# Shamir-Lab/Faucet

Hardware: AMD Instinct MI355X
Metric: canonical k-mers/s (load+scan) at k=31, 100bp reads; % HBM roofline (higher is better)
Workload: dtype u64

## Files before the change

### faucet_amd/csrc/api.hip

```cpp
#include <cstdio>
#include <algorithm>
#include <string>

#include <chrono>
#include <thread>

#include "fgpu_ctx.h"

int fgpu_scan_export_impl(fgpu_ctx* ctx, void* dev_entries, uint64_t cap_entries, uint64_t* d_stamps, uint64_t* n_entries);
int fgpu_scan_import_impl(fgpu_ctx* ctx, const void* dev_entries, uint64_t n);
int fgpu_scan_download_impl(fgpu_ctx* ctx, uint64_t* keys_host, fgpu_junction* recs_host, uint64_t cap, uint64_t* n_out);

static thread_local std::string g_create_error;

int g_fgpu_trace = getenv("FGPU_TRACE") && getenv("FGPU_TRACE")[0] == '1';

int fgpu_ensure(fgpu_ctx* ctx, DevBuf* b, uint64_t bytes) {
    if (b->bytes >= bytes && b->p) return FGPU_OK;
    if (b->p) {
        FGPU_HIP(fgpu_sync_stream(ctx, ctx->stream));
        FGPU_HIP(hipFree(b->p));
        b->p = nullptr;
        b->bytes = 0;
    } else {
// ... 228 lines not shown
    if (std::string(prop.gcnArchName).rfind("gfx950", 0) != 0) {
        g_create_error = std::string("device is ") + prop.gcnArchName + ", this library is built for gfx950 only";
        return FGPU_ERR_HIP;
    }
    if ((e = hipSetDevice(p->device)) != hipSuccess) { g_create_error = hipGetErrorString(e); return FGPU_ERR_HIP; }
    lap("device properties, hipSetDevice");

    fgpu_ctx* ctx = new fgpu_ctx();
    ctx->prm = *p;
    const int device = p->device;
    std::thread warm([device, ctx] {
        if (hipSetDevice(device) != hipSuccess) return;
        fgpu_touch_text();
        fgpu_touch_pack();
        fgpu_touch_load();
        fgpu_touch_load_slices();
        (void)fgpu_text_streams(ctx);
        (void)hipGetLastError();
    });
    struct Joiner { std::thread& t; ~Joiner() { if (t.joinable()) t.join(); } } joiner{warm};
    if (!ctx->prm.junction_capacity) {
        uint64_t c = p->tai / 32;
        if (c < (1ULL << 22)) c = 1ULL << 22;
        if (c > (1ULL << 28)) c = 1ULL << 28;
        ctx->prm.junction_capacity = c;
    }
    if (!ctx->prm.max_batch_bases) ctx->prm.max_batch_bases = 1ULL << 30;
    ctx->resident_budget = (p->flags & FGPU_FLAG_NO_RESIDENT) ? 0 : prop.totalGlobalMem / 8;
    ctx->journal_budget = prop.totalGlobalMem / 8;
    if (const char* e = getenv("FGPU_JOURNAL_MB")) ctx->journal_budget = (uint64_t)atoll(e) << 20;
    ctx->fd.k = p->k;
    ctx->fd.j = p->j;
    ctx->fd.n_hash = p->n_hash;
    ctx->fd.max_spacer = p->max_spacer_dist;
    ctx->fd.kmask = (1ULL << (2 * p->k)) - 1;
    ctx->fd.tai_mask = p->tai - 1;
    ctx->profile = (p->flags & FGPU_FLAG_PROFILE) != 0;
    ctx->record_stops = (p->flags & FGPU_FLAG_RECORD_STOPS) != 0;
    { const char* e = getenv("FGPU_PROFILE_WALK"); ctx->prof_walk_detail = e && e[0] == '1'; }
    ctx->bloom_bytes = p->tai / 8;
    ctx->max_span = std::min<uint64_t>(std::max<uint64_t>(p->tai >> 4, FGPU_MAX_SPAN), 1ULL << 28);
    if (const char* e = getenv("FGPU_MAX_SPAN_LOG2")) {
        int l = atoi(e);
        if (l >= 12 && l <= 28) ctx->max_span = 1ULL << l;
    }
    memset(&ctx->load_stats, 0, sizeof(ctx->load_stats));
    memset(&ctx->scan_stats, 0, sizeof(ctx->scan_stats));
    int rc = FGPU_OK;
    auto fail = [&](const char* what, hipError_t he) {
        g_create_error = std::string(what) + ": " + hipGetErrorString(he);
        rc = FGPU_ERR_HIP;
    };
    if (p->stream) {
        ctx->stream = (hipStream_t)p->stream;
    } else {
        if ((e = hipStreamCreateWithFlags(&ctx->stream, hipStreamNonBlocking)) != hipSuccess) fail("hipStreamCreate", e);
        ctx->own_stream = true;
    }
    ctx->launch_stream = ctx->stream;
    if (!rc) {
        ctx->bg = new std::thread([device, ctx] {
            auto bad = [ctx](const char* what, hipError_t he) {
                ctx->bg_err = std::string(what) + ": " + hipGetErrorString(he);
                ctx->bg_rc = FGPU_ERR_HIP;
            };
            hipError_t he;
            if ((he = hipSetDevice(device)) != hipSuccess) return bad("hipSetDevice", he);
            int lo = 0, hi = 0;
            hipDeviceGetStreamPriorityRange(&lo, &hi);
            if ((he = hipStreamCreateWithPriority(&ctx->wstream, hipStreamNonBlocking, hi)) != hipSuccess) return bad("hipStreamCreate (walk)", he);
            if ((he = hipStreamCreateWithPriority(&ctx->cstream, hipStreamNonBlocking, hi)) != hipSuccess) return bad("hipStreamCreate (clean)", he);
            if ((he = hipStreamCreateWithPriority(&ctx->ostream, hipStreamNonBlocking, hi)) != hipSuccess) return bad("hipStreamCreate (optimistic walk)", he);
            if ((he = hipEventCreateWithFlags(&ctx->ev_walked, hipEventDisableTiming)) != hipSuccess) return bad("hipEventCreate", he);
            if ((he = hipEventCreateWithFlags(&ctx->ev_listed, hipEventDisableTiming)) != hipSuccess) return bad("hipEventCreate", he);
            if ((he = hipEventCreateWithFlags(&ctx->ev_settled, hipEventDisableTiming)) != hipSuccess) return bad("hipEventCreate", he);
            for (int q = 0; q < 2; q++)
                if ((he = hipEventCreateWithFlags(&ctx->ev_uf_reset[q], hipEventDisableTiming)) != hipSuccess) return bad("hipEventCreate", he);
            fgpu_touch_scan_pure();
            fgpu_touch_scan_walk();
            fgpu_touch_scan_table();
            fgpu_touch_scan_harvest();
            (void)hipGetLastError();
        });
    }
    lap("main stream");
    if (!rc && getenv("FGPU_DEBUG_ALLOC_FIRST") && hipMalloc(&ctx->first, p->tai * 4) != hipSuccess) { (void)hipGetLastError(); ctx->first = nullptr; }
    if (!rc && (e = hipMalloc(&ctx->bloo1, ctx->bloom_bytes)) != hipSuccess) fail("hipMalloc bloo1", e);
    if (!rc && (e = hipMalloc(&ctx->bloo2, ctx->bloom_bytes)) != hipSuccess) fail("hipMalloc bloo2", e);
    if (!rc && (e = hipMalloc(&ctx->counters, sizeof(DevCounters))) != hipSuccess) fail("hipMalloc counters", e);
    if (!rc && (e = hipHostMalloc(&ctx->counters_host, sizeof(DevCounters))) != hipSuccess) fail("hipHostMalloc", e);
    if (!rc && (e = hipHostMalloc(&ctx->fb_host, 64)) != hipSuccess) fail("hipHostMalloc", e);
    if (!rc) {
        memset(ctx->counters_host, 0, sizeof(DevCounters));
        hipMemsetAsync(ctx->bloo1, 0, ctx->bloom_bytes, ctx->stream);
        hipMemsetAsync(ctx->bloo2, 0, ctx->bloom_bytes, ctx->stream);
        hipMemsetAsync(ctx->counters, 0, sizeof(DevCounters), ctx->stream);
        if ((e = hipStreamSynchronize(ctx->stream)) != hipSuccess) fail("initial memset", e);
    }
    lap("filters allocated and cleared");
    warm.join();
    lap("pass-1 code objects, text stream");
    if (rc) {
        fgpu_destroy(ctx);
        return rc;
    }
    *out = ctx;
    return FGPU_OK;
}

void fgpu_destroy(fgpu_ctx* ctx) {
    if (!ctx) return;
    (void)hipSetDevice(ctx->prm.device);
    (void)fgpu_bg_join(ctx);
    if (ctx->ostream) hipStreamSynchronize(ctx->ostream);
    if (ctx->cstream) hipStreamSynchronize(ctx->cstream);
    if (ctx->copy_stream) { hipStreamSynchronize(ctx->copy_stream); hipStreamDestroy(ctx->copy_stream); hipEventDestroy(ctx->copy_after); }
    if (ctx->tstream) {
        hipStreamSynchronize(ctx->tstream);
        hipStreamDestroy(ctx->tstream);
    }
    for (int i = 0; i < FGPU_TEXT_SETS; i++) if (ctx->ev_text_mark[i]) hipEventDestroy(ctx->ev_text_mark[i]);
    for (int i = 0; i < 2; i++) if (ctx->ev_stage_free[i]) hipEventDestroy(ctx->ev_stage_free[i]);
    if (ctx->ev_text_done) hipEventDestroy(ctx->ev_text_done);
    if (ctx->wstream) hipStreamSynchronize(ctx->wstream);
    if (ctx->stream) hipStreamSynchronize(ctx->stream);
    for (PendingEvent& pe : ctx->pending_events) { hipEventDestroy(pe.a); hipEventDestroy(pe.b); }
    for (DevBuf* b : ctx->owned) if (b->p) hipFree(b->p);
    if (ctx->lp.flips_host) hipHostFree(ctx->lp.flips_host);
    if (ctx->lp.ev_open) hipEventDestroy(ctx->lp.ev_open);
    void* ptrs[] = {ctx->lp.bits, ctx->lp.first, ctx->short_pf, ctx->bloo1, ctx->bloo2, ctx->first, ctx->pair, ctx->rec, ctx->slice_first, ctx->slice_pair, ctx->jkeys, ctx->jrecs, ctx->jstamps, ctx->jfilter, ctx->wkeys,
                    ctx->wbits, ctx->uf_parent, ctx->cl_count, ctx->cl_offset, ctx->cl_fill, ctx->cl_fail, ctx->ko_hk, ctx->ko_occ, ctx->ko_piece, ctx->cl_members, ctx->cl_roots, ctx->counters,
                    ctx->wdesc};
    for (void* p : ptrs) if (p) hipFree(p);
    stop_queue_recycle(ctx);
    for (StopBatch& f : ctx->stop_pool) hipHostFree(f.data);
    ctx->stop_pool.clear();
    if (ctx->counters_host) hipHostFree(ctx->counters_host);
    if (ctx->fb_host) hipHostFree(ctx->fb_host);
    if (ctx->wstream) { hipStreamSynchronize(ctx->wstream); hipStreamDestroy(ctx->wstream); }
    if (ctx->cstream) { hipStreamSynchronize(ctx->cstream); hipStreamDestroy(ctx->cstream); }
    if (ctx->ostream) { hipStreamSynchronize(ctx->ostream); hipStreamDestroy(ctx->ostream); }
    if (ctx->ev_walked) hipEventDestroy(ctx->ev_walked);
    if (ctx->ev_listed) hipEventDestroy(ctx->ev_listed);
    if (ctx->ev_settled) hipEventDestroy(ctx->ev_settled);
    for (int q = 0; q < 2; q++) if (ctx->ev_uf_reset[q]) hipEventDestroy(ctx->ev_uf_reset[q]);
    if (ctx->own_stream && ctx->stream) hipStreamDestroy(ctx->stream);
    for (ResidentBatch* r : ctx->resident) delete r;
    for (PackedBlock* b : ctx->packed) delete b;
    for (JournalBatch* j : ctx->journal) delete j;
    for (JournalBatch* j : ctx->journal_pool) delete j;
    for (BatchBufs* b : ctx->all_batches) {
        if (b->pure_done) hipEventDestroy(b->pure_done);
        if (b->walk_done) hipEventDestroy(b->walk_done);
        delete b;
    }
    delete ctx;
}

int fgpu_synchronize(fgpu_ctx* ctx) {
    if (!ctx) return FGPU_ERR_ARG;
    return sync_all(ctx);
}

int fgpu_load_begin(fgpu_ctx* ctx, int keep_carry) {
    if (!ctx) return FGPU_ERR_ARG;
    if (ctx->phase != 0) { ctx->err = "load_begin while another pass is open"; return FGPU_ERR_STATE; }
    FGPU_HIP(hipSetDevice(ctx->prm.device));
    if (int rc = fgpu_bloom_download_wait(ctx)) return rc;
    static const char* layout_env = getenv("FGPU_LOAD_LAYOUT");
    bool want_rec = layout_env && layout_env[0] == 'r';
    if (want_rec && !ctx->rec) {
        if (hipMalloc(&ctx->rec, ctx->prm.tai / 32 * 256) != hipSuccess) {
            (void)hipGetLastError();
            ctx->rec = nullptr;
            want_rec = false;
        }
    }
    ctx->rec_layout = want_rec;
    if (!ctx->rec_layout && !ctx->first) {
        hipError_t e = hipMalloc(&ctx->first, ctx->prm.tai * 4);
        if (e != hipSuccess) {
            ctx->err = std::string("hipMalloc of the first-set-time array (4 bytes per Bloom bit) failed: ") + hipGetErrorString(e);
            ctx->first = nullptr;
            return FGPU_ERR_NOMEM;
        }
    }
    if (!ctx->rec_layout && !ctx->pair) {
        hipError_t e = hipMalloc(&ctx->pair, ctx->bloom_bytes * 2);
        if (e != hipSuccess) {
            ctx->err = std::string("hipMalloc of the interleaved filter pair failed: ") + hipGetErrorString(e);
            ctx->pair = nullptr;
            return FGPU_ERR_NOMEM;
        }
        if (int rc = fgpu_place_pair(ctx)) return rc;
    }
    ctx->shard_times = (keep_carry & FGPU_LOAD_SHARD_TIMES) != 0;
    ctx->shard_planes = (keep_carry & FGPU_LOAD_SHARD_PLANES) != 0 && !ctx->shard_times && ctx->prm.n_hash <= 4;
    ctx->fixup_ready = false;
    ctx->scan_resident_base = 0;
    ctx->pass_positions = ctx->pass_batches = 0;
    ctx->pass_empty_carry = !(keep_carry & FGPU_LOAD_KEEP_CARRY);
    keep_carry &= FGPU_LOAD_KEEP_CARRY;
    fgpu_load_pass_policy(ctx);
    if (!ctx->rec_layout) FGPU_HIP(hipMemsetAsync(ctx->first, 0xFF, ctx->prm.tai * 4, ctx->stream));
    fgpu_resident_reset(ctx, true);
    if (!keep_carry) FGPU_HIP(hipMemsetAsync(ctx->bloo1, 0, ctx->bloom_bytes, ctx->stream));
    FGPU_HIP(hipMemsetAsync(ctx->bloo2, 0, ctx->bloom_bytes, ctx->stream));
    int rc = fgpu_load_pair_begin(ctx);
    if (rc) return rc;
    if ((rc = fgpu_load_pass_counters(ctx))) return rc;
    ctx->phase = 1;
    return FGPU_OK;
}

int fgpu_load_batch(fgpu_ctx* ctx, const fgpu_reads* reads) {
    if (!ctx) return FGPU_ERR_ARG;
    if (ctx->phase != 1) { ctx->err = "load_batch outside load_begin/load_end"; return FGPU_ERR_STATE; }
    int rc = fgpu_check_reads(ctx, reads);
    if (rc) return rc;
    FGPU_HIP(hipSetDevice(ctx->prm.device));
    if ((rc = fgpu_stage_pack(ctx, reads))) return rc;
    if ((rc = fgpu_stage_load(ctx))) return rc;
    if (ctx->cur->T) ctx->pass_batches++;
    ctx->load_stats.reads_processed += reads->n_reads;
    return fgpu_host_batch_done(ctx, reads);
}

int fgpu_presence_batch(fgpu_ctx* ctx, const fgpu_reads* reads) {
    if (!ctx) return FGPU_ERR_ARG;
    if (ctx->phase != 0) { ctx->err = "presence_batch while a pass is open"; return FGPU_ERR_STATE; }
    int rc = fgpu_check_reads(ctx, reads);
    if (rc) return rc;
    FGPU_HIP(hipSetDevice(ctx->prm.device));
    if ((rc = fgpu_stage_pack(ctx, reads))) return rc;
    if ((rc = fgpu_stage_presence(ctx))) return rc;
    return fgpu_host_batch_done(ctx, reads);
}

int fgpu_load_end(fgpu_ctx* ctx, fgpu_load_stats* stats) {
    if (!ctx) return FGPU_ERR_ARG;
    if (ctx->phase != 1) { ctx->err = "load_end without load_begin"; return FGPU_ERR_STATE; }
    return fgpu_load_pass_end(ctx, stats);
}

int fgpu_load_fixup_state(fgpu_ctx* ctx, int* ready, uint64_t* resident_budget_bytes) {
    if (!ctx) return FGPU_ERR_ARG;
    if (ready) *ready = ctx->phase == 0 && ctx->fixup_ready ? 1 : 0;
    if (resident_budget_bytes) *resident_budget_bytes = ctx->resident_budget;
    return FGPU_OK;
}

int fgpu_load_fixup(fgpu_ctx* ctx, const void* prefix_dev, fgpu_load_stats* stats) {
    if (!ctx || !prefix_dev) return FGPU_ERR_ARG;
    if (ctx->phase != 0) { ctx->err = "load_fixup while a pass is open"; return FGPU_ERR_STATE; }
    if (!ctx->fixup_ready) {
        ctx->err = "load_fixup needs a finished load pass begun with FGPU_LOAD_SHARD_TIMES and an empty carry (or FGPU_LOAD_SHARD_PLANES and at most 4 hash functions), every batch kept resident, no --mercy";
        return FGPU_ERR_STATE;
    }
    FGPU_HIP(hipSetDevice(ctx->prm.device));
    if (int rc = fgpu_bloom_download_wait(ctx)) return rc;
    int rc = fgpu_stage_fixup(ctx, (const uint32_t*)prefix_dev);
    if (!rc) rc = fgpu_util_or(ctx, ctx->bloo1, prefix_dev, ctx->bloom_bytes);
    if (!rc) rc = fgpu_pull_counters(ctx);
    if (rc) return rc;
    ctx->fixup_ready = false;
    ctx->load_stats.to_bloo2 = ctx->counters_host->to_bloo2;
    if (stats) *stats = ctx->load_stats;
    return FGPU_OK;
}

static uint32_t* bloom_ptr(fgpu_ctx* ctx, int which) { return which == FGPU_BLOO1 ? ctx->bloo1 : which == FGPU_BLOO2 ? ctx->bloo2 : nullptr; }

int fgpu_bloom_download(fgpu_ctx* ctx, int which, uint8_t* host_out, uint64_t nbytes) {
    if (!ctx || !host_out || !bloom_ptr(ctx, which) || nbytes != ctx->bloom_bytes) return FGPU_ERR_ARG;
    if (ctx->phase == 1 || ctx->phase == 3) { ctx->err = "bloom_download inside a load pass: the filters are interleaved until load_end"; return FGPU_ERR_STATE; }
    FGPU_HIP(hipMemcpyAsync(host_out, bloom_ptr(ctx, which), nbytes, hipMemcpyDeviceToHost, ctx->stream));
    FGPU_HIP(fgpu_sync_stream(ctx, ctx->stream));
    return FGPU_OK;
}

int fgpu_bloom_download_wait(fgpu_ctx* ctx) {
    if (!ctx) return FGPU_ERR_ARG;
    if (!ctx->copy_pending) return FGPU_OK;
    ctx->copy_pending = false;
    FGPU_HIP(fgpu_sync_stream(ctx, ctx->copy_stream));
    return FGPU_OK;
}

int fgpu_bloom_download_begin(fgpu_ctx* ctx, int which, uint8_t* host_out, uint64_t nbytes) {
    if (!ctx || !host_out || !bloom_ptr(ctx, which) || nbytes != ctx->bloom_bytes) return FGPU_ERR_ARG;
    if (ctx->phase == 1 || ctx->phase == 3) { ctx->err = "bloom_download_begin inside a load pass: the filters are interleaved until load_end"; return FGPU_ERR_STATE; }
    if (int rc = fgpu_bloom_download_wait(ctx)) return rc;
    FGPU_HIP(hipSetDevice(ctx->prm.device));
    if (!ctx->copy_stream) {
        FGPU_HIP(hipStreamCreateWithFlags(&ctx->copy_stream, hipStreamNonBlocking));
        FGPU_HIP(hipEventCreateWithFlags(&ctx->copy_after, hipEventDisableTiming));
    }
    FGPU_HIP(hipEventRecord(ctx->copy_after, ctx->stream));
    FGPU_HIP(hipStreamWaitEvent(ctx->copy_stream, ctx->copy_after, 0));
    FGPU_HIP(hipMemcpyAsync(host_out, bloom_ptr(ctx, which), nbytes, hipMemcpyDeviceToHost, ctx->copy_stream));
    ctx->copy_pending = true;
    return FGPU_OK;
}

int fgpu_bloom_upload(fgpu_ctx* ctx, int which, const uint8_t* host_in, uint64_t nbytes) {
    if (!ctx || !host_in || !bloom_ptr(ctx, which) || nbytes != ctx->bloom_bytes) return FGPU_ERR_ARG;
    if (ctx->phase != 0) { ctx->err = "bloom_upload while a pass is open (a load pass would overwrite it at load_end, a scan is reading bloo2)"; return FGPU_ERR_STATE; }
    if (int rc = fgpu_bloom_download_wait(ctx)) return rc;
    if (which == FGPU_BLOO2) fgpu_resident_reset(ctx, false);
    FGPU_HIP(hipMemcpyAsync(bloom_ptr(ctx, which), host_in, nbytes, hipMemcpyHostToDevice, ctx->stream));
    FGPU_HIP(fgpu_sync_stream(ctx, ctx->stream));
    return FGPU_OK;
}

int fgpu_bloom_weight(fgpu_ctx* ctx, int which, float* weight) {
    if (!ctx || !weight || !bloom_ptr(ctx, which)) return FGPU_ERR_ARG;
    if (ctx->phase == 1 || ctx->phase == 3) { ctx->err = "bloom_weight inside a load pass: the filters are interleaved until load_end"; return FGPU_ERR_STATE; }
    FGPU_HIP(hipMemsetAsync(&ctx->counters->pad, 0, 8, ctx->stream));
    int rc = fgpu_util_popcount(ctx, bloom_ptr(ctx, which), ctx->bloom_bytes, &ctx->counters->pad);
    if (rc) return rc;
    FGPU_HIP(hipMemcpyAsync(&ctx->counters_host->pad, &ctx->counters->pad, 8, hipMemcpyDeviceToHost, ctx->stream));
    FGPU_HIP(fgpu_sync_stream(ctx, ctx->stream));
    *weight = (float)(long)ctx->counters_host->pad / (float)ctx->prm.tai;
    return FGPU_OK;
}

int fgpu_bloom_devptr(fgpu_ctx* ctx, int which, void** dptr, uint64_t* nbytes) {
    if (!ctx || !dptr || !bloom_ptr(ctx, which)) return FGPU_ERR_ARG;
    *dptr = bloom_ptr(ctx, which);
    if (nbytes) *nbytes = ctx->bloom_bytes;
    return FGPU_OK;
}

int fgpu_bitmap_or(fgpu_ctx* ctx, void* dst_dev, const void* src_dev, uint64_t nbytes) {
    if (!ctx || !dst_dev || !src_dev || (nbytes & 15)) return FGPU_ERR_ARG;
    return fgpu_util_or(ctx, dst_dev, src_dev, nbytes);
}

int fgpu_scan_resident_base(fgpu_ctx* ctx, uint64_t first_batch) {
    if (!ctx) return FGPU_ERR_ARG;
    if (ctx->phase != 0) { ctx->err = "scan_resident_base while a pass is open: between the load pass and fgpu_scan_begin"; return FGPU_ERR_STATE; }
    ctx->scan_resident_base = first_batch;
    return FGPU_OK;
}

int fgpu_scan_begin(fgpu_ctx* ctx) {
    if (!ctx) return FGPU_ERR_ARG;
    if (ctx->phase != 0) { ctx->err = "scan_begin while another pass is open"; return FGPU_ERR_STATE; }
    FGPU_HIP(hipSetDevice(ctx->prm.device));
    int rc = fgpu_bg_join(ctx);
    if (rc) return rc;
    if ((rc = fgpu_scan_alloc(ctx))) return rc;
    if ((rc = fgpu_scan_reset(ctx))) return rc;
    ctx->fixup_ready = false;
    FGPU_HIP(hipMemsetAsync(ctx->counters, 0, sizeof(DevCounters), ctx->stream));
    memset(&ctx->scan_stats, 0, sizeof(ctx->scan_stats));
    memset(ctx->counters_host, 0, sizeof(DevCounters));
    ctx->scan_windows = 0;
    ctx->scan_pieces_seen = 0;
    ctx->scan_piece_base = 0;
    ctx->scan_imported = 0;
    ctx->delta_next = 0;
    journal_recycle(ctx);
    ctx->journal_on = !(ctx->prm.flags & FGPU_FLAG_EAGER_FLAGS) && !ctx->eager_runtime;
    ctx->eager_scan = ctx->lazy_failed = ctx->capacity_failed = false;
    ctx->dl_keys_n = 0;
    ctx->late_acc[0] = ctx->late_acc[1] = ctx->late_acc[2] = 0;
    ctx->stops_delivered = 0;
    ctx->lp_applied_seq = 0;
    ctx->host_waits = 0;
    ctx->host_wait_ms = 0;
    ctx->wait_sites.clear();
    if (ctx->short_pf) FGPU_HIP(hipMemsetAsync(ctx->short_pf, 0, ctx->short_pf_tai / 8, ctx->stream));
    if ((rc = fgpu_long_pairs_reset(ctx))) return rc;
    ctx->have_import = false;
    ctx->journal_max_read_len = 0;
    ctx->hint_in_table = false;
    ctx->hint_gen = 0;
    ctx->hint_n = ctx->hint_max_seq = 0;
    ctx->delta_ready = false;
    ctx->delta_keys = ctx->refresh_full = ctx->refresh_delta = ctx->refresh_mismatch = 0;
    ctx->sparse_links = ctx->full_links = 0;
    ctx->dbg_stall_us = getenv("FGPU_DEBUG_WALK_STALL_US") ? std::min(100000, std::max(0, atoi(getenv("FGPU_DEBUG_WALK_STALL_US")))) : 0;
    ctx->dbg_delta_check = getenv("FGPU_DEBUG_DELTA_CHECK") != nullptr;
    ctx->no_sparse_link = getenv("FGPU_NO_SPARSE_LINK") != nullptr;
    const uint64_t start_span = std::max<uint64_t>(1ULL << 18, ctx->settled_span / 4);
    ctx->window_span = ctx->prm.walk_window_span ? std::min<uint64_t>(std::max<uint64_t>(ctx->prm.walk_window_span, 64), ctx->max_span)
                                                 : std::min<uint64_t>(start_span, ctx->max_span);
    ctx->calib_left = 16;
    ctx->calib_f = ctx->calib_p = 0;
    ctx->adapt_followers = 0;
    ctx->adapt_pieces = 0;
    ctx->adapt_overflows = 0;
    ctx->adapt_vote = 0;
    ctx->calib_ovf = 0;
    ctx->span_ceiling = ~0ULL;
    ctx->repeats_seen_before = false;
    ctx->walked_pieces = 0;
    ctx->scan_batch_index = 0;
    ctx->scan_batch_seq = 0;
    for (BatchBufs* b : ctx->to_harvest) b->stops_pending = false;
    ctx->to_harvest.clear();
    stop_queue_recycle(ctx);
    for (BatchBufs* b : ctx->prepared) ctx->pool.push_back(b);
    ctx->prepared.clear();
    ctx->cur = &ctx->bb_default;
    ctx->phase = 2;
    return FGPU_OK;
}

static void adapt_window(fgpu_ctx* ctx) {
    static const bool dbg_span = getenv("FGPU_DEBUG_SPAN") != nullptr;
    const uint64_t f = ctx->counters_host->followers_seen - ctx->adapt_followers;
    const uint64_t p = ctx->counters_host->walked_pieces - ctx->adapt_pieces;
    if (p == 0 || ctx->prm.walk_window_span) return;
    {
        const uint64_t usual = std::min<uint64_t>(std::min<uint64_t>(ctx->max_span, FGPU_USUAL_SPAN), ctx->span_ceiling);
        int want = 0;
        bool clear = false;
        if (f * 2 > p) { want = -1; clear = f * 5 > p * 4; }
        else if (f * 3 < p) { want = 1; clear = f * 20 < p * 3; }
        const bool act = want < 0 || (want > 0 && (clear || ctx->adapt_vote > 0));
        ctx->adapt_vote = act ? 0 : want;
        if (want >= 0) ctx->proven_span = std::max(ctx->proven_span, ctx->window_span);
        if (ctx->counters_host->ko_overflows > ctx->adapt_overflows && ctx->window_span > 4096) {
            ctx->window_span = std::max<uint64_t>(4096, ctx->window_span / 4);
            ctx->proven_span = std::min(ctx->proven_span, ctx->window_span);
            ctx->span_ceiling = std::min(ctx->span_ceiling, ctx->window_span * 2);
            ctx->calib_ovf = ctx->counters_host->ko_overflows;
            ctx->calib_left = 0;
        }
        else if (act && want < 0 && ctx->window_span > 4096) {
            ctx->window_span /= 2;
            if (clear || ctx->window_span > ctx->proven_span) ctx->calib_left = 8;
            ctx->proven_span = std::min(ctx->proven_span, ctx->window_span);
        }
        else if (act && want > 0 && ctx->window_span < usual) {
            ctx->window_span = std::min<uint64_t>(ctx->window_span * 2, usual);
            if (ctx->window_span > ctx->proven_span) ctx->calib_left = std::max(ctx->calib_left, 2);
        }
        else if (f * 16 < p && ctx->window_span < std::min<uint64_t>(ctx->max_span, ctx->span_ceiling)) ctx->window_span *= 2;
    }
    if (dbg_span) fprintf(stderr, "[span] batch: followers %llu of %llu pieces -> span %llu, looks %d, vote %d\n", (unsigned long long)f, (unsigned long long)p,
                          (unsigned long long)ctx->window_span, ctx->calib_left, ctx->adapt_vote);
    ctx->adapt_followers = ctx->counters_host->followers_seen;
    ctx->adapt_pieces = ctx->counters_host->walked_pieces;
    ctx->adapt_overflows = ctx->counters_host->ko_overflows;
}

static BatchBufs* acquire_batch(fgpu_ctx* ctx) {
    BatchBufs* b;
    static const size_t depth = getenv("FGPU_SCAN_BUFFERS") ? (size_t)std::min(FGPU_DELTA_RING, std::max(2, atoi(getenv("FGPU_SCAN_BUFFERS")))) : 2;
    if (ctx->pool.size() >= depth) {
        const size_t at = ctx->pool.size() - depth;
        b = ctx->pool[at];
        ctx->pool.erase(ctx->pool.begin() + at);
    } else {
        b = new BatchBufs();
        ctx->all_batches.push_back(b);
        hipEventCreateWithFlags(&b->pure_done, hipEventDisableTiming);
        hipEventCreateWithFlags(&b->walk_done, hipEventDisableTiming);
    }
    return b;
}

static void note_walked(fgpu_ctx* ctx, BatchBufs* b) {
    if (!ctx->record_stops) return;
    b->stops_pending = true;
    ctx->to_harvest.push_back(b);
}

static int scan_pure_into(fgpu_ctx* ctx, BatchBufs* b, const fgpu_reads* reads) {
    if (b->stops_pending) {
        int hrc = fgpu_scan_harvest(ctx, b);
        if (hrc) return hrc;
    }
    b->seq = ctx->scan_batch_seq++;
    ctx->cur = b;
    const double t_a = fgpu_host_now();
    if (b->walk_pending) {
        FGPU_HIP(fgpu_sync_event(ctx, b->walk_done));
        b->walk_pending = false;
    }
    const double t_b = fgpu_host_now();
    ctx->host_ms[0] += t_b - t_a;
    int rc = fgpu_stage_pack(ctx, reads);
    ctx->host_ms[1] += fgpu_host_now() - t_b;
    if (!rc) rc = journal_add(ctx, b, reads);
    uint64_t n_pieces = 0;
    if (!rc) rc = fgpu_stage_scan_pure(ctx, &n_pieces);
    if (!rc) ctx->journal_max_read_len = std::max<uint64_t>(ctx->journal_max_read_len, ctx->counters_host->max_read_len);
    if (!rc) rc = check_errors(ctx);
    if (!rc) ctx->scan_stats.reads_processed += reads->n_reads;
    if (!rc && b->pure_done) FGPU_HIP(hipEventRecord(b->pure_done, ctx->stream));
    if (!rc) rc = fgpu_host_batch_done(ctx, reads);
    return rc;
}

static void journal_recycle(fgpu_ctx* ctx) {
    for (JournalBatch* j : ctx->journal) ctx->journal_pool.push_back(j);
    ctx->journal.clear();
    ctx->journal_bytes = 0;
}

static int journal_add(fgpu_ctx* ctx, BatchBufs* b, const fgpu_reads* reads) {
    if (!ctx->journal_on || ctx->in_replay) return FGPU_OK;
    const uint64_t cb = 2 * (b->n_words + FGPU_PADW) * 8, bbytes = (b->n_words + FGPU_PADW) * 8, ob = ctx->record_stops ? (b->n_reads + 1) * 8 : 0;
    if (ctx->journal_bytes + cb + bbytes + ob > ctx->journal_budget) {
        int rc = fgpu_pull_counters(ctx);
        if (rc) return rc;
        BatchBufs* const cur = ctx->cur;
        ctx->journal_max_read_len = std::max<uint64_t>(ctx->journal_max_read_len, ctx->counters_host->max_read_len);
        if (ctx->lazy_failed && (rc = scan_replay(ctx))) return rc;
        ctx->cur = cur;
        ctx->journal_on = false;
        ctx->eager_scan = true;
        journal_recycle(ctx);
        return FGPU_OK;
    }
    JournalBatch* j;
    if (!ctx->journal_pool.empty()) { j = ctx->journal_pool.back(); ctx->journal_pool.pop_back(); }
    else j = new JournalBatch();
    int rc;
    if ((rc = fgpu_ensure_b(ctx, &j->codes, cb)) || (rc = fgpu_ensure_b(ctx, &j->bad, bbytes)) || (ob && (rc = fgpu_ensure_b(ctx, &j->offs, ob)))) {
        ctx->journal_pool.push_back(j);
        return rc;
    }
    if (b->T) {
        FGPU_HIP(hipMemcpyAsync(j->codes.p, b->codes.p, cb, hipMemcpyDeviceToDevice, ctx->stream));
        FGPU_HIP(hipMemcpyAsync(j->bad.p, b->bad.p, bbytes, hipMemcpyDeviceToDevice, ctx->stream));
        if (ob) FGPU_HIP(hipMemcpyAsync(j->offs.p, b->d_offs, ob, hipMemcpyDeviceToDevice, ctx->stream));
    }
    j->T = b->T; j->n_words = b->n_words; j->n_reads = b->n_reads; j->seq = b->seq;
    ctx->journal.push_back(j);
    ctx->journal_bytes += cb + bbytes + ob;
    (void)reads;
    return FGPU_OK;
}

static int scan_replay_once(fgpu_ctx* ctx);
static int scan_replay(fgpu_ctx* ctx) {
    for (int attempt = 0;; attempt++) {
        const bool for_room = ctx->capacity_failed;
        ctx->capacity_failed = false;
        if (for_room) {
            int rc = sync_all(ctx);
            if (!rc) rc = fgpu_scan_regrow_empty(ctx, ctx->jcap * 4);
            if (rc) { ctx->lazy_failed = false; return rc; }
            ctx->capacity_replays++;
        }
        int rc = scan_replay_once(ctx);
        if (rc == FGPU_ERR_CAPACITY && (ctx->counters_host->error_flags & 1ULL) && ctx->jcap < (1ULL << 31) && attempt < 6) {
            ctx->capacity_failed = true;
            continue;
        }
        if (!rc && for_room) ctx->journal_on = true;
        return rc;
    }
}

static int scan_replay_once(fgpu_ctx* ctx) {
    ctx->in_replay = true;
    ctx->journal_on = false;
    ctx->eager_scan = true;
    ctx->lazy_failed = false;
    int rc = sync_all(ctx);
    for (BatchBufs* b : ctx->prepared) ctx->pool.push_back(b);
    ctx->prepared.clear();
    for (BatchBufs* b : ctx->to_harvest) b->stops_pending = false;
    ctx->to_harvest.clear();
    stop_queue_recycle(ctx);
    if (!rc) rc = fgpu_scan_reset(ctx);
    if (rc) { ctx->in_replay = false; return rc; }
    {
        unsigned long long ln[3] = {0, 0, 0};
        if (hipMemcpy(ln, ctx->counters->late_n, sizeof(ln), hipMemcpyDeviceToHost) == hipSuccess)
            for (int i = 0; i < 3; i++) ctx->late_acc[i] += ln[i];
    }
    FGPU_HIP(hipMemsetAsync(ctx->counters, 0, sizeof(DevCounters), ctx->stream));
    FGPU_HIP(hipMemcpyAsync(&ctx->counters->max_read_len, &ctx->journal_max_read_len, 8, hipMemcpyHostToDevice, ctx->stream));
    FGPU_HIP(fgpu_sync_stream(ctx, ctx->stream));
    const uint64_t reads_processed = ctx->scan_stats.reads_processed;
    memset(&ctx->scan_stats, 0, sizeof(ctx->scan_stats));
    ctx->scan_stats.reads_processed = reads_processed;
    memset(ctx->counters_host, 0, sizeof(DevCounters));
    ctx->scan_windows = 0;
    ctx->scan_pieces_seen = 0;
    ctx->scan_piece_base = 0;
    ctx->scan_imported = 0;
    ctx->delta_next = 0;
    ctx->hint_in_table = false;
    ctx->delta_ready = false;
    ctx->window_span = ctx->prm.walk_window_span ? std::min<uint64_t>(std::max<uint64_t>(ctx->prm.walk_window_span, 64), ctx->max_span)
                                                 : std::min<uint64_t>(std::max<uint64_t>(1ULL << 18, ctx->settled_span / 4), ctx->max_span);
    ctx->calib_left = 16;
    ctx->calib_f = ctx->calib_p = 0;
    ctx->adapt_followers = ctx->adapt_pieces = ctx->adapt_overflows = 0;
    ctx->adapt_vote = 0;
    ctx->calib_ovf = 0;
    ctx->span_ceiling = ~0ULL;
    ctx->repeats_seen_before = false;
    ctx->walked_pieces = 0;
    ctx->scan_batch_index = 0;
    memset(&ctx->carried, 0, sizeof(ctx->carried));
    if (ctx->have_import) {
        if ((rc = fgpu_scan_reserve(ctx, ctx->import_n)) || (rc = fgpu_scan_import_impl(ctx, ctx->import_copy.p, ctx->import_n))) { ctx->in_replay = false; return rc; }
        FGPU_HIP(fgpu_sync_stream(ctx, ctx->stream));
        ctx->scan_imported = ctx->import_n;
        if (ctx->import_has_carried) {
            ctx->carried = ctx->import_carried;
            ctx->scan_piece_base = ctx->import_carried.reads_no_errors;
        }
    }
    for (size_t i = 0; i < ctx->journal.size() && !rc; i++) {
        JournalBatch* j = ctx->journal[i];
        BatchBufs* b = acquire_batch(ctx);
        if (b->stops_pending && (rc = fgpu_scan_harvest(ctx, b))) {
            ctx->pool.push_back(b);
            break;
        }
        if (b->walk_pending) {
            FGPU_HIP(fgpu_sync_event(ctx, b->walk_done));
            b->walk_pending = false;
        }
        b->seq = j->seq;
        ctx->cur = b;
        b->T = j->T; b->n_words = j->n_words; b->n_reads = j->n_reads;
        b->d_offs = (const uint64_t*)j->offs.p;
        if (b->T) {
            const uint64_t cb = 2 * (b->n_words + FGPU_PADW) * 8, bbytes = (b->n_words + FGPU_PADW) * 8;
            if ((rc = fgpu_ensure_b(ctx, &b->codes, cb)) || (rc = fgpu_ensure_b(ctx, &b->bad, bbytes))) break;
            FGPU_HIP(hipMemcpyAsync(b->codes.p, j->codes.p, cb, hipMemcpyDeviceToDevice, ctx->stream));
            FGPU_HIP(hipMemcpyAsync(b->bad.p, j->bad.p, bbytes, hipMemcpyDeviceToDevice, ctx->stream));
        }
        uint64_t n_pieces = 0;
        rc = fgpu_stage_scan_pure(ctx, &n_pieces);
        if (!rc) rc = check_errors(ctx);
        if (!rc && b->pure_done) FGPU_HIP(hipEventRecord(b->pure_done, ctx->stream));
        if (!rc) rc = fgpu_scan_reserve(ctx, ctx->counters_host->n_junctions + ctx->scan_imported);
        if (!rc) {
            adapt_window(ctx);
            rc = fgpu_stage_scan_walk(ctx, b->n_pieces);
            ctx->walked_pieces += b->n_pieces;
            if (!rc) note_walked(ctx, b);
        }
        ctx->pool.push_back(b);
    }
    ctx->cur = &ctx->bb_default;
    if (!rc) rc = fgpu_pull_counters(ctx);
    ctx->in_replay = false;
    ctx->scan_replays++;
    return rc;
}

int fgpu_scan_batch(fgpu_ctx* ctx, const fgpu_reads* reads) {
    if (!ctx) return FGPU_ERR_ARG;
    if (ctx->phase != 2) { ctx->err = "scan_batch outside scan_begin/scan_end"; return FGPU_ERR_STATE; }
    if (!ctx->prepared.empty()) { ctx->err = "scan_batch while prepared batches are waiting: call fgpu_scan_walk_prepared first"; return FGPU_ERR_STATE; }
    if (ctx->hint_in_table) { ctx->err = "the junction table holds a preview (fgpu_scan_import_hint): import the real table before walking"; return FGPU_ERR_STATE; }
    int rc = fgpu_check_reads(ctx, reads);
    if (rc) return rc;
    FGPU_HIP(hipSetDevice(ctx->prm.device));
    if (ctx->lazy_failed && (rc = scan_replay(ctx))) return rc;
    BatchBufs* b = acquire_batch(ctx);
    rc = scan_pure_into(ctx, b, reads);
    if (rc == FGPU_INTERNAL_REPLAY) {
        ctx->cur = &ctx->bb_default;
        ctx->pool.insert(ctx->pool.begin(), b);
        if ((rc = scan_replay(ctx))) return rc;
        b = acquire_batch(ctx);
        rc = scan_pure_into(ctx, b, reads);
    }
    if (!rc && ctx->lazy_failed) {
        ctx->cur = &ctx->bb_default;
        ctx->pool.push_back(b);
        return scan_replay(ctx);
    }
    if (!rc) rc = fgpu_scan_reserve(ctx, ctx->counters_host->n_junctions + ctx->scan_imported);
    if (!rc) {
        adapt_window(ctx);
        const double t_w = fgpu_host_now();
        rc = fgpu_stage_scan_walk(ctx, b->n_pieces);
        ctx->host_ms[5] += fgpu_host_now() - t_w;
        ctx->walked_pieces += b->n_pieces;
        if (!rc) note_walked(ctx, b);
    }
    ctx->cur = &ctx->bb_default;
    ctx->pool.push_back(b);
    return rc;
}

int fgpu_scan_prepare(fgpu_ctx* ctx, const fgpu_reads* reads) {
    if (!ctx) return FGPU_ERR_ARG;
    if (ctx->phase != 2) { ctx->err = "scan_prepare outside scan_begin/scan_end"; return FGPU_ERR_STATE; }
    int rc = fgpu_check_reads(ctx, reads);
    if (rc) return rc;
    FGPU_HIP(hipSetDevice(ctx->prm.device));
    BatchBufs* b;
    if (!ctx->pool.empty()) { b = ctx->pool.front(); ctx->pool.erase(ctx->pool.begin()); }
    else {
        b = new BatchBufs();
        ctx->all_batches.push_back(b);
        hipEventCreateWithFlags(&b->pure_done, hipEventDisableTiming);
        hipEventCreateWithFlags(&b->walk_done, hipEventDisableTiming);
    }
    rc = scan_pure_into(ctx, b, reads);
    ctx->cur = &ctx->bb_default;
    if (rc == FGPU_INTERNAL_REPLAY) {
        ctx->pool.insert(ctx->pool.begin(), b);
        if ((rc = scan_replay(ctx))) return rc;
        return fgpu_scan_prepare(ctx, reads);
    }
    if (rc) { ctx->pool.push_back(b); return rc; }
    b->planes_gen = ctx->hint_in_table ? ctx->hint_gen : 0;
    b->cand_gen = 0;
    ctx->prepared.push_back(b);
    return FGPU_OK;
}

int fgpu_scan_refresh_prepared(fgpu_ctx* ctx) {
    if (!ctx) return FGPU_ERR_ARG;
    if (ctx->phase != 2) { ctx->err = "scan_refresh_prepared outside scan_begin/scan_end"; return FGPU_ERR_STATE; }
    if (!ctx->hint_in_table) { ctx->err = "scan_refresh_prepared without a preview in the table (fgpu_scan_import_hint)"; return FGPU_ERR_STATE; }
    FGPU_HIP(hipSetDevice(ctx->prm.device));
    const bool no_sparse = ctx->no_sparse_link;
    for (BatchBufs* b : ctx->prepared) {
        if (b->planes_gen != ctx->hint_gen) {
            if (int rc = fgpu_scan_refresh_planes(ctx, b)) return rc;
            b->planes_gen = ctx->hint_gen;
            b->cand_gen = 0;
        }
        if (!no_sparse && b->cand_gen != ctx->hint_gen)
            if (int rc = fgpu_scan_build_cand(ctx, b)) return rc;
    }
    ctx->launch_stream = ctx->stream;
    FGPU_HIP(fgpu_sync_stream(ctx, ctx->stream));
    return FGPU_OK;
}

int fgpu_scan_walk_prepared(fgpu_ctx* ctx) {
    if (!ctx) return FGPU_ERR_ARG;
    if (ctx->phase != 2) { ctx->err = "scan_walk_prepared outside scan_begin/scan_end"; return FGPU_ERR_STATE; }
    if (ctx->hint_in_table) { ctx->err = "the junction table holds a preview (fgpu_scan_import_hint): import the real table before walking"; return FGPU_ERR_STATE; }
    FGPU_HIP(hipSetDevice(ctx->prm.device));
    int rc = FGPU_OK;
    if (ctx->lazy_failed) return scan_replay(ctx);
    static const bool serial_refresh = !(getenv("FGPU_PREPARED_REFRESH") && getenv("FGPU_PREPARED_REFRESH")[0] == 'o');
    if (!serial_refresh && !ctx->prepared.empty()) rc = fgpu_scan_refresh_planes(ctx, ctx->prepared[0]);
    for (size_t i = 0; i < ctx->prepared.size() && !rc; i++) {
        BatchBufs* b = ctx->prepared[i];
        if (i > 0) {
            if ((rc = fgpu_pull_counters(ctx))) break;
            if (ctx->lazy_failed) { ctx->cur = &ctx->bb_default; return scan_replay(ctx); }
            if (!ctx->prm.walk_window_span) adapt_window(ctx);
            if ((rc = fgpu_scan_reserve(ctx, ctx->counters_host->n_junctions + ctx->scan_imported))) break;
        }
        if (!serial_refresh && i + 1 < ctx->prepared.size() && (rc = fgpu_scan_refresh_planes(ctx, ctx->prepared[i + 1]))) break;
        ctx->cur = b;
        ctx->refresh_snapshot = serial_refresh;
        rc = fgpu_stage_scan_walk(ctx, b->n_pieces);
        ctx->refresh_snapshot = false;
        ctx->walked_pieces += b->n_pieces;
        if (!rc) note_walked(ctx, b);
    }
    ctx->cur = &ctx->bb_default;
    for (BatchBufs* b : ctx->prepared) ctx->pool.push_back(b);
    ctx->prepared.clear();
    return rc;
}

int fgpu_scan_set_eager(fgpu_ctx* ctx, int on) {
    if (!ctx) return FGPU_ERR_ARG;
    if (ctx->phase != 0) { ctx->err = "fgpu_scan_set_eager while a pass is open"; return FGPU_ERR_STATE; }
    ctx->eager_runtime = on != 0;
    return FGPU_OK;
}

int fgpu_scan_short_pairs(fgpu_ctx* ctx, uint64_t tai, int32_t n_hash, int32_t lists_to_host) {
    if (!ctx) return FGPU_ERR_ARG;
    if (ctx->phase != 0) { ctx->err = "fgpu_scan_short_pairs while a pass is open"; return FGPU_ERR_STATE; }
    FGPU_HIP(hipSetDevice(ctx->prm.device));
    if (ctx->short_pf) {
        FGPU_HIP(fgpu_sync_stream(ctx, ctx->stream));
        FGPU_HIP(hipFree(ctx->short_pf));
        ctx->short_pf = nullptr;
        ctx->short_pf_tai = 0;
    }
    if (!tai) return FGPU_OK;
    if (!ctx->record_stops) { ctx->err = "fgpu_scan_short_pairs needs FGPU_FLAG_RECORD_STOPS"; return FGPU_ERR_STATE; }
    if (!is_pow2(tai) || tai < 128 || n_hash < 1 || n_hash > 32) { ctx->err = "fgpu_scan_short_pairs: tai must be a power of two >= 128, n_hash 1..32"; return FGPU_ERR_ARG; }
    FGPU_HIP(hipMalloc(&ctx->short_pf, tai / 8));
    FGPU_HIP(hipMemsetAsync(ctx->short_pf, 0, tai / 8, ctx->stream));
    ctx->short_pf_tai = tai;
    ctx->short_pf_hashes = n_hash;
    ctx->short_pf_lists_to_host = lists_to_host != 0;
    return FGPU_OK;
}

int fgpu_scan_short_pairs_download(fgpu_ctx* ctx, uint8_t* out, uint64_t n_bytes) {
    if (!ctx || !out) return FGPU_ERR_ARG;
    if (!ctx->short_pf) { ctx->err = "fgpu_scan_short_pairs_download without fgpu_scan_short_pairs"; return FGPU_ERR_STATE; }
    if (ctx->phase != 0) { ctx->err = "fgpu_scan_short_pairs_download while a pass is open"; return FGPU_ERR_STATE; }
    if (n_bytes != ctx->short_pf_tai / 8) { ctx->err = "fgpu_scan_short_pairs_download: the filter has tai / 8 bytes"; return FGPU_ERR_ARG; }
    FGPU_HIP(hipSetDevice(ctx->prm.device));
    FGPU_HIP(hipMemcpyAsync(out, ctx->short_pf, n_bytes, hipMemcpyDeviceToHost, ctx->stream));
    FGPU_HIP(fgpu_sync_stream(ctx, ctx->stream));
    return FGPU_OK;
}

int fgpu_scan_take_stops(fgpu_ctx* ctx, fgpu_stop* out, uint64_t cap, uint64_t* n_out, int64_t* batch_seq) {
    if (!ctx || !n_out || !batch_seq) return FGPU_ERR_ARG;
    if (!ctx->record_stops) { ctx->err = "fgpu_scan_take_stops needs FGPU_FLAG_RECORD_STOPS"; return FGPU_ERR_STATE; }
    *n_out = 0;
    *batch_seq = -1;
    if (ctx->phase == 2 && ctx->lazy_failed) {
        if (int rc = scan_replay(ctx)) return rc;
    }
    if (ctx->stop_queue.empty() && !ctx->to_harvest.empty()) {
        FGPU_HIP(hipSetDevice(ctx->prm.device));
        int rc = fgpu_scan_harvest(ctx, ctx->to_harvest.front());
        if (rc == FGPU_INTERNAL_REPLAY && ctx->phase == 2) {
            if ((rc = scan_replay(ctx))) return rc;
            if (!ctx->to_harvest.empty()) rc = fgpu_scan_harvest(ctx, ctx->to_harvest.front());
        }
        if (rc) return rc;
    }
    if (ctx->stop_queue.empty()) return FGPU_OK;
    StopBatch& sb = ctx->stop_queue.front();
    *n_out = sb.n;
    *batch_seq = (int64_t)sb.seq;
    if (sb.n > cap || (sb.n && !out)) return FGPU_ERR_CAPACITY;
    if (sb.n) memcpy(out, sb.data, sb.n * sizeof(fgpu_stop));
    ctx->stops_delivered = sb.seq + 1;
    if (sb.data) { StopBatch f; f.data = sb.data; f.cap = sb.cap; ctx->stop_pool.push_back(f); }
    ctx->stop_queue.pop_front();
    return FGPU_OK;
}

int fgpu_scan_end(fgpu_ctx* ctx, fgpu_scan_stats* stats) {
    if (!ctx) return FGPU_ERR_ARG;
    if (ctx->phase != 2) { ctx->err = "scan_end without scan_begin"; return FGPU_ERR_STATE; }
    static const bool dbg_host = getenv("FGPU_DEBUG_HOST") != nullptr;
    static const bool dbg_waits = getenv("FGPU_DEBUG_WAITS") != nullptr;
    struct TellWaits {
        fgpu_ctx* c;
        bool on;
        ~TellWaits() {
            if (!on) return;
            for (const WaitSite& w : c->wait_sites) {
                const char* f = strrchr(w.file, '/');
                fprintf(stderr, "[waits] %-14s:%-5d %6llu times %9.2f ms\n", f ? f + 1 : w.file, w.line, (unsigned long long)w.n, w.ms);
            }
        }
    } tell_waits{ctx, dbg_waits};
    if (dbg_host) {
        fprintf(stderr, "[host] scan: wait for the buffers' last walk %.2f ms, pack issue %.2f, pure stage issue (first half) %.2f, wait for the piece count %.2f, "
                        "pure stage issue (second half) %.2f, walk issue %.2f\n", ctx->host_ms[0], ctx->host_ms[1], ctx->host_ms[2], ctx->host_ms[3], ctx->host_ms[4], ctx->host_ms[5]);
        for (double& v : ctx->host_ms) v = 0;
    }
// ... 310 lines not shown
```

### faucet_amd/csrc/fgpu_ctx.h

```cpp
#pragma once
#include <chrono>
#include <hip/hip_runtime.h>
#include <stdint.h>
#include <stdio.h>
#include <string.h>

#include <string>
#include <thread>
#include <vector>

#include "../../include/faucet_gpu.h"
#include <deque>

#include "fgpu_device.h"

#define FGPU_PADW 8
#define FGPU_USUAL_SPAN (1ULL << 26)
#define FGPU_MAX_SPAN (1ULL << 26)

struct DevBuf {
    void*    p = nullptr;
    uint64_t bytes = 0;
};

struct BatchBufs {
    DevBuf codes, bad;
    DevBuf readflag;
    DevBuf pending;
    DevBuf sure;
    DevBuf fail;
    DevBuf same;
    DevBuf valid, pm, ps, ff, fb, cf0, cf1, cb0, cb1, inF, inB;
    DevBuf lk;
    DevBuf cand;
    uint32_t cand_gen = 0;
    DevBuf nF, nB, need;
    DevBuf kh;
    DevBuf cr;
    DevBuf ps_prefix;
    DevBuf pieces;
    DevBuf sF, sB;
    DevBuf piece_read;
    DevBuf stop_off, stop_out;
    const uint64_t* d_offs = nullptr;
    uint64_t seq = 0;
    bool stops_pending = false;
    uint64_t T = 0;
    uint64_t n_words = 0;
    uint64_t n_reads = 0;
    uint64_t n_pieces = 0;
    uint64_t max_piece_span = 0;
    hipEvent_t pure_done = nullptr;
    hipEvent_t walk_done = nullptr;
    bool walk_pending = false;
    uint32_t planes_gen = 0;
};

struct ResidentBatch {
    DevBuf codes, bad, sure;
    DevBuf fail;
    DevBuf miss;
    uint64_t T = 0, n_words = 0;
    uint32_t tb = 0;
    void *packed_codes = nullptr, *packed_bad = nullptr;
    const void* codes_p() const { return packed_codes ? packed_codes : codes.p; }
    const void* bad_p() const { return packed_bad ? packed_bad : bad.p; }
};

struct PackedBlock {
    DevBuf buf;
    uint64_t T = 0, n_words = 0, n_reads = 0;
    int state = 0;
};
static inline uint64_t fgpu_packed_bytes(uint64_t n_words) { return 3 * (n_words + FGPU_PADW) * 8 + 16; }

struct DeltaList {
    DevBuf list, count;
};
#define FGPU_DELTA_RING 4

struct JournalBatch {
    DevBuf codes, bad, offs;
    uint64_t T = 0, n_words = 0, n_reads = 0, seq = 0;
};
#define FGPU_INTERNAL_REPLAY 1000

struct StopBatch {
    uint64_t seq = 0;
    fgpu_stop* data = nullptr;
    size_t n = 0, cap = 0;
};

struct LongPairs {
    int mode = 0;
    bool sparse = false;
    uint64_t tai = 0;
    int n_hash = 0;
    uint32_t* bits = nullptr;
    uint32_t* first = nullptr;
    DevBuf table;
    uint64_t table_high = 0;
    DevBuf canon, h0, h1, vread, rs, state, dev;
    DevBuf kept_set[2];
    int kept_cur = 0;
    uint32_t* flips_host = nullptr;
    bool pending_first = false;
    uint64_t n_kept = 0;
    uint64_t empty_host = 0;
    uint64_t rounds = 0, max_rounds = 0, batches = 0;
    bool open = false, open_odd = false, open_filter = false;
    uint32_t open_elems = 0, open_vreads = 0;
    hipEvent_t ev_open = nullptr;
};

struct WaitSite {
    const char* file;
    int line;
    uint64_t n;
    double ms;
};

struct KernelStat {
    std::string name;
    uint64_t launches = 0;
    double total_ms = 0;
};

struct PendingEvent {
    int stat;
    hipEvent_t a, b;
};

constexpr unsigned FGPU_LATE_CAP = 256;
struct DevCounters {
    unsigned long long kmers;
    unsigned long long to_bloo2;
    unsigned long long segments;
    unsigned long long pieces;
    unsigned long long nb_jcheck;
    unsigned long long nb_no_juncs;
    unsigned long long nb_processed;
    unsigned long long nb_skipped;
    unsigned long long n_junctions;
    unsigned long long table_slots_used;
    unsigned long long followers;
    unsigned long long max_cluster;
    unsigned long long error_flags;
    unsigned long long max_read_len;
    unsigned long long wt_used;
    unsigned long long pad;
    unsigned long long wt_used_b;
    unsigned long long pad2;
    unsigned long long flag_positions;
    unsigned long long piece_positions;
    unsigned long long valid_reused;
    unsigned long long flags_filled;
    unsigned long long walked_pieces;
    unsigned long long followers_seen;
    unsigned long long mark_hits;
    unsigned long long mark_pending;
    unsigned long long walk_parallel;
    unsigned long long par_probe[4];
    unsigned long long ko_time[8];
    unsigned long long ko_overflows;
    unsigned long long ovw_kept;
    unsigned long long ovw[4];
    unsigned long long ovw_fill;
    unsigned long long late_n[3];
    unsigned long long late[2 * FGPU_LATE_CAP];
    unsigned long long slice_mercy[6];
};

constexpr int FGPU_TEXT_SETS = 3;
struct TextSet { DevBuf buf, nl, rank, tmp, rec; };

static inline double fgpu_host_now() { return std::chrono::duration<double, std::milli>(std::chrono::steady_clock::now().time_since_epoch()).count(); }

struct fgpu_ctx {
    fgpu_params prm;
    FdParams fd;
    hipStream_t stream = nullptr;
    hipStream_t wstream = nullptr;
    hipStream_t cstream = nullptr;
    hipEvent_t ev_walked = nullptr, ev_uf_reset[2] = {nullptr, nullptr};
    hipStream_t ostream = nullptr;
    hipEvent_t ev_listed = nullptr, ev_settled = nullptr;
    hipStream_t launch_stream = nullptr;
    bool own_stream = false;
    std::string err;
    std::thread* bg = nullptr;
    int bg_rc = 0;
    std::string bg_err;

    uint32_t* bloo1 = nullptr;
    uint64_t epoch_positions = 0;
    uint64_t swept_positions = 0;
    bool shard_times = false;
    bool shard_planes = false;
    bool fixup_ready = false;
    uint64_t pass_positions = 0;
    uint32_t cur_tb = 0;
    bool pass_empty_carry = true;
    uint64_t pass_batches = 0;
    uint64_t sweep_min = 0;
    uint32_t sweep_num = 1, sweep_den = 1;
    bool carry_by_set = false;
    uint32_t* bloo2 = nullptr;
    uint32_t* first = nullptr;
    uint2* pair = nullptr;
    uint32_t* rec = nullptr;
    bool rec_layout = false;
    uint64_t bloom_bytes = 0;
    int phase = 0;
    uint64_t slice_lo = 0, slice_n = 0;
    uint32_t* slice_first = nullptr;
    uint2* slice_pair = nullptr;
    uint64_t slice_first_bytes = 0, slice_pair_bytes = 0;
    bool slice_committed = false;
    bool slice_mercy = false;
    bool slice_probe_owed = false;
    uint64_t slice_owed_span = 0;
    uint64_t slice_mercy_diag[6] = {0, 0, 0, 0, 0, 0};
    std::vector<ResidentBatch*> resident;
    uint64_t resident_count = 0;
    uint64_t resident_bytes = 0, resident_budget = 0;
    bool resident_open = false;
    uint64_t scan_batch_index = 0;
    uint64_t scan_resident_base = 0;
    std::vector<PackedBlock*> packed;
    DevBuf packed_digest;

    uint64_t jcap = 0;
    uint64_t* jkeys = nullptr;
    uint8_t* jrecs = nullptr;
    uint64_t* jstamps = nullptr;
    uint32_t* jfilter = nullptr;
    uint64_t wcap = 0;
    uint64_t* wkeys = nullptr;
    uint32_t* wbits = nullptr;
    int wbits_log2 = 24;
    DeltaList delta_ring[FGPU_DELTA_RING];
    bool refresh_snapshot = false;
    uint64_t delta_hist[FGPU_DELTA_RING] = {0, 0, 0, 0};
    uint64_t delta_ring_keys = 0, delta_batch_base = 0;
    uint64_t delta_next = 0;
    uint32_t wt_epoch = 0;
    uint32_t wmax = 0;
    uint32_t* uf_parent = nullptr;
    uint32_t* cl_count = nullptr;
    uint32_t* cl_offset = nullptr;
    uint32_t* cl_fill = nullptr;
    uint32_t* ko_hk = nullptr;
    uint32_t* ko_occ = nullptr;
    uint32_t* ko_piece = nullptr;
    DevBuf ovw_ev, ovw_filt, ovw_log, ovw_res, ovw_list, ovw_state, ovw_longp, ovw_marks;
    uint32_t ovw_epoch = 0;
    int ovw_ev_log2 = 23;
    int ovw_ev_log2_alloc = 0;
    int ovw_rounds = 12;
    uint32_t ko_hk_cap = 0, ko_occ_cap = 0;
    uint32_t walk_ko = 64;
    uint32_t walk_ko_weight = 0;
    bool walk_ko_always = false;
    uint32_t* cl_fail = nullptr;
    uint32_t walk_heavy = 0;
    uint32_t* cl_members = nullptr;
    uint32_t* cl_roots = nullptr;
    void* wdesc = nullptr;
    uint64_t window_span = 1ULL << 17;
    uint64_t max_span = FGPU_MAX_SPAN;
    uint64_t settled_span = 0;
    uint64_t scan_piece_base = 0;
    uint64_t scan_imported = 0;
    bool hint_in_table = false;
    uint32_t hint_gen = 0;
    uint64_t hint_n = 0, hint_max_seq = 0;
    uint64_t hint_digest[2] = {0, 0};
    DevBuf delta_filter;
    uint64_t delta_filter_bits = 0;
    bool delta_ready = false;
    uint64_t delta_keys = 0;
    uint64_t refresh_full = 0, refresh_delta = 0, refresh_mismatch = 0;
    DevBuf cand_filter;
    uint64_t sparse_links = 0, full_links = 0;
    int dbg_stall_us = 0;
    bool dbg_delta_check = false;
    bool no_sparse_link = false;
    DevBuf import_probe;
    uint64_t scan_grown = 0;

    DevCounters* counters = nullptr;
    DevCounters* counters_host = nullptr;

    fgpu_load_stats load_stats;
    uint64_t load_mark_hits = 0, load_mark_pending = 0;
    fgpu_scan_stats scan_stats;
    uint64_t scan_windows = 0;
    uint64_t scan_pieces_seen = 0;

    uint64_t adapt_followers = 0, adapt_pieces = 0;
    double host_ms[8] = {0, 0, 0, 0, 0, 0, 0, 0};
    bool repeats_seen_before = false;
    uint64_t calib_ovf = 0;
    uint64_t span_ceiling = ~0ULL;
    int adapt_vote = 0;
    uint64_t proven_span = 0;
    uint64_t adapt_overflows = 0;
    int calib_left = 0;
    uint64_t calib_f = 0, calib_p = 0;
    unsigned long long* fb_host = nullptr;
    fgpu_scan_stats carried = {};

    BatchBufs bb_default;
    BatchBufs* cur = &bb_default;
    std::vector<BatchBufs*> prepared;
    std::vector<BatchBufs*> pool;
    std::vector<BatchBufs*> all_batches;
    std::vector<JournalBatch*> journal, journal_pool;
    uint64_t journal_bytes = 0, journal_budget = 0;
    bool journal_on = false;
    bool eager_scan = false;
    bool lazy_failed = false;
    bool in_replay = false;
    bool capacity_failed = false;
    uint64_t capacity_replays = 0;
    uint32_t* short_pf = nullptr;
    uint64_t short_pf_tai = 0;
    int short_pf_hashes = 0;
    bool short_pf_lists_to_host = true;
    LongPairs lp;
    uint64_t stops_delivered = 0;
    uint64_t lp_applied_seq = 0;
    uint64_t scan_replays = 0;
    uint64_t host_waits = 0;
    double host_wait_ms = 0;
    std::vector<WaitSite> wait_sites;
    uint64_t late_acc[3] = {0, 0, 0};
    uint64_t journal_max_read_len = 0;
    DevBuf import_copy;
    uint64_t import_n = 0;
    fgpu_scan_stats import_carried = {};
    bool have_import = false, import_has_carried = false;
    bool record_stops = false;
    bool eager_runtime = false;
    std::vector<BatchBufs*> to_harvest;
    std::deque<StopBatch> stop_queue;
    std::vector<StopBatch> stop_pool;
    uint64_t scan_batch_seq = 0;
    uint64_t walked_pieces = 0;
    DevBuf probe_buf, export_stamps;
    DevBuf ko_trace;
    DevBuf s3_keys, s3_dist, s3_in;
    uint64_t s3_mask = 0, s3_count = 0;
    bool s3_ready = false;
    DevBuf dl_entries, dl_stamps, dl_stamps_sorted, dl_idx, dl_idx_sorted, dl_keys, dl_recs, dl_tmp;
    uint64_t dl_keys_n = 0;
    hipStream_t copy_stream = nullptr;
    hipEvent_t copy_after = nullptr;
    bool copy_pending = false;
    TextSet text[FGPU_TEXT_SETS];
    uint64_t text_calls = 0;
    uint64_t text_reserve = 0;
    uint64_t text_last_bytes = 0;
    double ensure_scale = 1.0;
    hipStream_t tstream = nullptr;
    hipEvent_t ev_text_mark[FGPU_TEXT_SETS] = {nullptr, nullptr, nullptr};
    hipEvent_t ev_text_done = nullptr;
    DevBuf host_stage[4];
    hipEvent_t ev_stage_free[2] = {nullptr, nullptr};
    bool host_stage_used[2] = {false, false};
    uint64_t host_turn = 0;
    int host_set = -1;
    const uint64_t* split_offsets = nullptr;
    uint64_t split_n = 0, split_total = 0;
    std::vector<DevBuf*> owned;

    bool profile = false;
    bool prof_suppress = false;
    bool prof_walk_detail = false;
    std::vector<KernelStat> kstats;
    std::vector<PendingEvent> pending_events;
};

#define FGPU_HIP(call)                                                                               \
    do {                                                                                             \
        hipError_t e__ = (call);                                                                     \
        if (e__ != hipSuccess) {                                                                     \
            char b__[512];                                                                           \
            snprintf(b__, sizeof(b__), "%s failed: %s (%s:%d)", #call, hipGetErrorString(e__), __FILE__, __LINE__); \
            ctx->err = b__;                                                                          \
            return FGPU_ERR_HIP;                                                                     \
        }                                                                                            \
    } while (0)

static inline void fgpu_note_wait(fgpu_ctx* ctx, double ms, const char* file, int line) {
    ctx->host_waits++;
    ctx->host_wait_ms += ms;
    for (WaitSite& w : ctx->wait_sites)
        if (w.line == line && w.file == file) { w.n++; w.ms += ms; return; }
    ctx->wait_sites.push_back(WaitSite{file, line, 1, ms});
}
static inline hipError_t fgpu_sync_stream_at(fgpu_ctx* ctx, hipStream_t st, const char* file, int line) {
    const double t0 = fgpu_host_now();
    const hipError_t e = hipStreamSynchronize(st);
    fgpu_note_wait(ctx, fgpu_host_now() - t0, file, line);
    return e;
}
static inline hipError_t fgpu_sync_event_at(fgpu_ctx* ctx, hipEvent_t ev, const char* file, int line) {
    const double t0 = fgpu_host_now();
    const hipError_t e = hipEventSynchronize(ev);
    fgpu_note_wait(ctx, fgpu_host_now() - t0, file, line);
    return e;
}
#define fgpu_sync_stream(ctx, st) fgpu_sync_stream_at(ctx, st, __FILE__, __LINE__)
#define fgpu_sync_event(ctx, ev) fgpu_sync_event_at(ctx, ev, __FILE__, __LINE__)

int fgpu_ensure(fgpu_ctx* ctx, DevBuf* b, uint64_t bytes);
int fgpu_ensure_b(fgpu_ctx* ctx, DevBuf* b, uint64_t bytes);
int fgpu_bg_join(fgpu_ctx* ctx);
int fgpu_prof_begin(fgpu_ctx* ctx, const char* name);
void fgpu_prof_end(fgpu_ctx* ctx, int token);
int fgpu_prof_collect(fgpu_ctx* ctx);

extern int g_fgpu_trace;
#define FGPU_LAUNCH(name, kernel, grid, block, ...)                                        \
    do {                                                                                   \
        int tok__ = fgpu_prof_begin(ctx, name);                                            \
        if (g_fgpu_trace) { fprintf(stderr, "[fgpu] %s grid %u x %u ...", name, (unsigned)(grid), (unsigned)(block)); fflush(stderr); } \
        hipLaunchKernelGGL(kernel, dim3(grid), dim3(block), 0, ctx->launch_stream, __VA_ARGS__);  \
        fgpu_prof_end(ctx, tok__);                                                         \
        FGPU_HIP(hipGetLastError());                                                       \
        if (g_fgpu_trace) { FGPU_HIP(hipStreamSynchronize(ctx->launch_stream)); fprintf(stderr, " done\n"); fflush(stderr); } \
    } while (0)

static inline unsigned fgpu_blocks(uint64_t n, unsigned per_block) { return (unsigned)((n + per_block - 1) / per_block); }
#define FGPU_GRID_BLOCKS 4096u
static inline unsigned fgpu_grid(uint64_t n, unsigned per_block) {
    uint64_t b = (n + per_block - 1) / per_block;
    return (unsigned)(b < FGPU_GRID_BLOCKS ? (b ? b : 1) : FGPU_GRID_BLOCKS);
}

static inline bool fgpu_overflow_absorbable(const fgpu_ctx* ctx) {
    return ctx->journal_on && ctx->phase == 2 && !ctx->in_replay && ctx->jcap < (1ULL << 31);
}
#define FGPU_TABLE_FULL_MSG "junction table full: raise fgpu_params.junction_capacity"

int fgpu_text_streams(fgpu_ctx* ctx);
void fgpu_touch_load();
void fgpu_touch_load_slices();
void fgpu_touch_pack();
void fgpu_touch_text();
void fgpu_touch_scan_pure();
void fgpu_touch_scan_walk();
void fgpu_touch_scan_table();
void fgpu_touch_scan_harvest();
int fgpu_stage_pack(fgpu_ctx* ctx, const fgpu_reads* reads);
int fgpu_stage_pack_block(fgpu_ctx* ctx, const fgpu_reads* reads, PackedBlock** out);
int fgpu_packed_acquire(fgpu_ctx* ctx, uint64_t T, uint64_t n_reads, int state, const char* who, PackedBlock** out);
int fgpu_packed_digest(fgpu_ctx* ctx, const PackedBlock* b, bool verify);
int fgpu_host_batch_done(fgpu_ctx* ctx, const fgpu_reads* reads);
int fgpu_stage_load(fgpu_ctx* ctx);
int fgpu_load_sweep(fgpu_ctx* ctx);
int fgpu_stage_fixup(fgpu_ctx* ctx, const uint32_t* prefix);
int fgpu_stage_presence(fgpu_ctx* ctx);
int fgpu_epoch_before_batch(fgpu_ctx* ctx, uint64_t span);
int fgpu_epoch_after_batch(fgpu_ctx* ctx, uint64_t span);
enum { FGPU_TAKE_OK = 0, FGPU_TAKE_NO_BUDGET, FGPU_TAKE_NO_MEMORY };
int fgpu_resident_take(fgpu_ctx* ctx, const uint64_t (&parts)[5], bool budgeted, ResidentBatch** out, uint64_t* total);
int fgpu_pull_counters(fgpu_ctx* ctx);
int fgpu_check_reads(fgpu_ctx* ctx, const fgpu_reads* r);
void fgpu_load_pass_policy(fgpu_ctx* ctx);
int fgpu_load_pass_counters(fgpu_ctx* ctx);
int fgpu_load_pass_end(fgpu_ctx* ctx, fgpu_load_stats* stats);
int fgpu_load_pair_begin(fgpu_ctx* ctx);
int fgpu_load_pair_end(fgpu_ctx* ctx);
void fgpu_resident_reset(fgpu_ctx* ctx, bool keep_going);
int fgpu_stage_scan_pure(fgpu_ctx* ctx, uint64_t* n_pieces);
int fgpu_stage_scan_walk(fgpu_ctx* ctx, uint64_t n_pieces);
int fgpu_stage_scan_need(fgpu_ctx* ctx);
int fgpu_scan_refresh_planes(fgpu_ctx* ctx, BatchBufs* b);
int fgpu_scan_build_cand(fgpu_ctx* ctx, BatchBufs* b);
int fgpu_scan_import_probe(fgpu_ctx* ctx, const void* dev_entries, uint64_t n, uint64_t after_seq, uint32_t* dfilter, uint64_t dfilter_bits,
                           uint64_t* max_seq, uint64_t* n_newer, uint64_t digest[2]);
int fgpu_stage_scan_debug_drop(fgpu_ctx* ctx);
int fgpu_util_count_segments(fgpu_ctx* ctx, const void* bad, uint64_t n_words, int minlen);
int fgpu_util_popcount(fgpu_ctx* ctx, const void* dev, uint64_t nbytes, unsigned long long* dev_out);
int fgpu_util_or(fgpu_ctx* ctx, void* dst, const void* src, uint64_t nbytes);
int fgpu_util_probe_hash(fgpu_ctx* ctx, const uint64_t* d_kmers, uint64_t n, uint64_t* d_canon, uint64_t* d_hA, uint64_t* d_hB);
int fgpu_util_probe_contains(fgpu_ctx* ctx, const uint32_t* bloom, const uint64_t* d_canon, uint64_t n, unsigned char* d_out);
int fgpu_util_probe_stage3(fgpu_ctx* ctx, const uint64_t* d_kmers, uint64_t n, int mode, signed char* d_out);
int fgpu_scan_alloc(fgpu_ctx* ctx);
int fgpu_scan_harvest(fgpu_ctx* ctx, BatchBufs* b);
int fgpu_long_pairs_batch(fgpu_ctx* ctx, const fgpu_stop* d_stops, uint64_t n_stops, uint64_t n_reads);
int fgpu_long_pairs_reset(fgpu_ctx* ctx);
int fgpu_long_pairs_close(fgpu_ctx* ctx);
int fgpu_place_pair(fgpu_ctx* ctx);
int fgpu_scan_reset(fgpu_ctx* ctx);
int fgpu_scan_grow(fgpu_ctx* ctx, uint64_t new_cap);
int fgpu_scan_reserve(fgpu_ctx* ctx, uint64_t records);
int fgpu_scan_clear_table(fgpu_ctx* ctx);
int fgpu_scan_dump_order_impl(fgpu_ctx* ctx, const uint64_t* d_keys, const uint64_t* counts, const uint64_t* buckets, uint64_t n_phases, uint64_t n, uint32_t* order_host);
int fgpu_scan_regrow_empty(fgpu_ctx* ctx, uint64_t new_cap);
```

### faucet_amd/csrc/scan_pure.hip

```cpp
#include <algorithm>

#include "fgpu_ctx.h"
#include "fgpu_flags.h"

namespace {

__global__ void __launch_bounds__(256) k_scan_same(const uint64_t* __restrict__ codes, const uint64_t* __restrict__ kept_codes, uint64_t n_code_words,
                                                   const uint64_t* __restrict__ bad, const uint64_t* __restrict__ kept_bad, uint64_t n_words,
                                                   uint32_t* same) {
    bool differ = false;
    for (uint64_t i = (uint64_t)blockIdx.x * blockDim.x + threadIdx.x; i < n_code_words; i += (uint64_t)gridDim.x * blockDim.x) {
        differ |= codes[i] != kept_codes[i];
        if (i < n_words) differ |= bad[i] != kept_bad[i];
    }
    if (__ballot(differ) && fd_lane() == 0) *same = 0;
}

__global__ void __launch_bounds__(256) k_scan_valid(const uint64_t* __restrict__ codes, const uint64_t* __restrict__ bad,
                                                    uint64_t T, uint64_t n_words, FdParams fp, const uint32_t* __restrict__ bloom,
                                                    const uint64_t* __restrict__ sure, const uint32_t* __restrict__ same,
                                                    uint64_t* __restrict__ valid, DevCounters* cnt) {
    unsigned long long n_ok = 0, n_reused = 0;
    const uint64_t total = n_words * 64;
    const bool reuse = sure && *same != 0;
    for (uint64_t p = (uint64_t)blockIdx.x * blockDim.x + threadIdx.x; p < total; p += (uint64_t)gridDim.x * blockDim.x) {
        bool ok = p < T && fd_window_ok(bad, p, fp.k);
        bool v = false;
        if (ok) {
            n_ok++;
            if (reuse && ((sure[p >> 6] >> (p & 63)) & 1ULL)) {
                v = true;
                n_reused++;
            } else {
                v = fd_bloom_contains_canon(bloom, fd_canon(fd_kmer_at(codes, p, fp.k), fp.k), fp.tai_mask, fp.n_hash);
            }
        }
        uint64_t vm = __ballot(v);
        if (fd_lane() == 0) valid[p >> 6] = vm;
    }
    block_add(&cnt->kmers, n_ok);
    block_add(&cnt->valid_reused, n_reused);
}

__global__ void __launch_bounds__(256) k_scan_pieces(const uint64_t* __restrict__ valid, const uint64_t* __restrict__ bad,
                                                     uint64_t n_words, FdParams fp, int check_segment,
                                                     unsigned long long* pm, uint64_t* __restrict__ ps, DevCounters* cnt) {
    unsigned long long n_pieces = 0;
    for (uint64_t w = (uint64_t)blockIdx.x * blockDim.x + threadIdx.x; w < n_words; w += (uint64_t)gridDim.x * blockDim.x) {
        uint64_t vw = valid[w];
        uint64_t prev = w ? valid[w - 1] >> 63 : 0;
        uint64_t starts = vw & ~((vw << 1) | prev);
        uint64_t psw = 0;
        while (starts) {
            const int sbit = __builtin_ctzll(starts);
            starts &= starts - 1;
            const uint64_t p = w * 64 + sbit;
            uint64_t q = p, len = 0;
            for (;;) {
                uint64_t bits = ~fd_bits_at(valid, q);
                if (bits) { len += __builtin_ctzll(bits); break; }
                len += 64;
                q += 64;
            }
            bool piece = len >= (uint64_t)fp.k;
            if (piece && check_segment) {
                uint64_t b = p;
                while (b > 0 && !((bad[(b - 1) >> 6] >> ((b - 1) & 63)) & 1ULL)) b--;
                uint64_t e = p;
                for (;;) {
                    uint64_t bits = fd_bits_at(bad, e);
                    if (bits) { e += __builtin_ctzll(bits); break; }
                    e += 64;
                }
                piece = (e - b) >= (uint64_t)(fp.k + 2 * fp.j + 1);
            }
            if (piece) {
                psw |= 1ULL << sbit;
                n_pieces++;
                uint64_t a = p, z = p + len;
                while (a < z) {
                    uint64_t wi = a >> 6;
                    uint64_t hi = (wi + 1) << 6;
                    uint64_t upto = z < hi ? z : hi;
                    int lo_b = (int)(a & 63), n_b = (int)(upto - a);
                    unsigned long long m = (n_b == 64 ? ~0ULL : ((1ULL << n_b) - 1)) << lo_b;
                    atomicOr(&pm[wi], m);
                    a = upto;
                }
            }
        }
        ps[w] = psw;
    }
    block_add(&cnt->pieces, n_pieces);
}

constexpr int SCAN_BLOCK = 1024;
__global__ void __launch_bounds__(SCAN_BLOCK) k_prefix_block(const uint64_t* __restrict__ ps, uint64_t n_words,
                                                             uint32_t* __restrict__ prefix, uint32_t* __restrict__ block_sums) {
    __shared__ uint32_t sh[SCAN_BLOCK];
    uint64_t w = (uint64_t)blockIdx.x * SCAN_BLOCK + threadIdx.x;
    uint32_t c = w < n_words ? (uint32_t)__popcll(ps[w]) : 0;
    sh[threadIdx.x] = c;
    __syncthreads();
    for (int o = 1; o < SCAN_BLOCK; o <<= 1) {
        uint32_t t = threadIdx.x >= (unsigned)o ? sh[threadIdx.x - o] : 0;
        __syncthreads();
        sh[threadIdx.x] += t;
        __syncthreads();
    }
    if (w < n_words) prefix[w] = sh[threadIdx.x] - c;
    if (threadIdx.x == SCAN_BLOCK - 1) block_sums[blockIdx.x] = sh[threadIdx.x];
}

__global__ void __launch_bounds__(SCAN_BLOCK) k_prefix_sums(uint32_t* block_sums, uint32_t n_blocks) {
    __shared__ uint32_t sh[SCAN_BLOCK];
    __shared__ uint32_t carry;
    if (threadIdx.x == 0) carry = 0;
    __syncthreads();
    for (uint32_t base = 0; base < n_blocks; base += SCAN_BLOCK) {
        uint32_t i = base + threadIdx.x;
        uint32_t c = i < n_blocks ? block_sums[i] : 0;
        sh[threadIdx.x] = c;
        __syncthreads();
        for (int o = 1; o < SCAN_BLOCK; o <<= 1) {
            uint32_t t = threadIdx.x >= (unsigned)o ? sh[threadIdx.x - o] : 0;
            __syncthreads();
            sh[threadIdx.x] += t;
            __syncthreads();
        }
        if (i < n_blocks) block_sums[i] = carry + sh[threadIdx.x] - c;
        __syncthreads();
        if (threadIdx.x == SCAN_BLOCK - 1) carry += sh[threadIdx.x];
        __syncthreads();
    }
}

__global__ void __launch_bounds__(256) k_prefix_apply(uint32_t* __restrict__ prefix, const uint32_t* __restrict__ block_sums,
                                                      uint64_t n_words) {
    uint64_t w = (uint64_t)blockIdx.x * blockDim.x + threadIdx.x;
    if (w < n_words) prefix[w] += block_sums[w / SCAN_BLOCK];
}

__global__ void __launch_bounds__(256) k_scan_piece_list(const uint64_t* __restrict__ ps, const uint64_t* __restrict__ pm,
                                                         const uint32_t* __restrict__ prefix, uint64_t n_words, uint2* __restrict__ pieces) {
    for (uint64_t w = (uint64_t)blockIdx.x * blockDim.x + threadIdx.x; w < n_words; w += (uint64_t)gridDim.x * blockDim.x) {
        uint64_t word = ps[w];
        uint32_t rank = prefix[w];
        while (word) {
            const int sbit = __builtin_ctzll(word);
            word &= word - 1;
            const uint64_t p = w * 64 + sbit;
            uint64_t q = p, len = 0;
            for (;;) {
                uint64_t bits = ~fd_bits_at(pm, q);
                if (bits) { len += __builtin_ctzll(bits); break; }
                len += 64;
                q += 64;
            }
            pieces[rank++] = make_uint2((uint32_t)p, (uint32_t)len);
        }
    }
}

__global__ void __launch_bounds__(256) k_scan_piece_read(const uint2* __restrict__ pieces, uint64_t n_pieces, const uint64_t* __restrict__ offs,
                                                         uint64_t n_reads, uint32_t* __restrict__ piece_read) {
    const uint64_t i = (uint64_t)blockIdx.x * blockDim.x + threadIdx.x;
    if (i >= n_pieces) return;
    const uint64_t off0 = offs[0], s0 = pieces[i].x;
    uint64_t lo = 0, hi = n_reads - 1;
    while (lo < hi) {
        const uint64_t mid = (lo + hi + 1) >> 1;
        if ((offs[mid] - off0) + mid <= s0) lo = mid; else hi = mid - 1;
    }
    piece_read[i] = (uint32_t)lo;
}

__global__ void __launch_bounds__(256) k_scan_flags(const uint64_t* __restrict__ codes, const uint64_t* __restrict__ pm,
                                                    const uint64_t* __restrict__ need, uint64_t T, uint64_t n_words, FdParams fp, const uint32_t* __restrict__ bloom,
                                                    unsigned long long* ff, unsigned long long* fb, unsigned long long* cf0,
                                                    unsigned long long* cf1, unsigned long long* cb0, unsigned long long* cb1,
                                                    DevCounters* cnt) {
    const int lane = fd_lane();
    const uint64_t n_waves = ((uint64_t)gridDim.x * blockDim.x) >> 6;
    const uint64_t n_chunks = (n_words + 3) / 4;
    unsigned long long n_eval = 0, n_piece = 0;
    for (uint64_t chunk = ((uint64_t)blockIdx.x * blockDim.x + threadIdx.x) >> 6; chunk < n_chunks; chunk += n_waves) {
        uint64_t mine = 0;
        if (lane < 8) {
            const uint64_t w = chunk * 4 + (lane & 3);
            if (w < n_words) {
                const uint64_t tmask = (w + 1) * 64 <= T ? ~0ULL : (T > w * 64 ? (1ULL << (T - w * 64)) - 1 : 0ULL);
                const uint64_t pmw = pm[w] & tmask, nd = need[w] & tmask;
                if (lane < 4) {
                    mine = nd & pmw & ((pmw >> 1) | (pm[w + 1] << 63));
                    n_eval += __popcll(nd);
                    n_piece += __popcll(pmw);
                } else {
                    mine = nd & pmw & ((pmw << 1) | (w ? pm[w - 1] >> 63 : 0ULL));
                }
            }
        }
        uint64_t m[8];
        int cum[9];
        cum[0] = 0;
#pragma unroll
        for (int q = 0; q < 8; q++) {
            m[q] = __shfl(mine, q, 64);
            cum[q + 1] = cum[q] + __popcll(m[q]);
        }
        for (int t = lane; t < cum[8]; t += 64) {
            int q = 0;
            uint64_t mq = m[0];
            int before = 0;
#pragma unroll
            for (int c = 1; c < 8; c++)
                if (t >= cum[c]) { q = c; mq = m[c]; before = cum[c]; }
            const int bit = select_bit(mq, t - before);
            const uint64_t w = chunk * 4 + (q & 3);
            const uint64_t pos = w * 64 + bit;
            const uint64_t km = fd_kmer_at(codes, pos, fp.k);
            bool flag;
            int njc;
            const unsigned long long bm = 1ULL << bit;
            if (q < 4) {
                test_for_junction(km, fd_base_at(codes, pos + fp.k), fp, bloom, flag, njc);
                if (flag) atomicOr(&ff[w], bm);
                if (njc & 1) atomicOr(&cf0[w], bm);
                if (njc & 2) atomicOr(&cf1[w], bm);
            } else {
                test_for_junction(fd_revcomp(km, fp.k), fd_base_at(codes, pos - 1) ^ 2, fp, bloom, flag, njc);
                if (flag) atomicOr(&fb[w], bm);
                if (njc & 1) atomicOr(&cb0[w], bm);
                if (njc & 2) atomicOr(&cb1[w], bm);
            }
        }
    }
    block_add(&cnt->flag_positions, n_eval);
    block_add(&cnt->piece_positions, n_piece);
}

struct FlagPool {
    unsigned long long mf[64], mb[64];
    int excl[64];
};

struct FlagChain {
    uint64_t key;
    uint64_t hA, hB;
    uint32_t w;
    uint32_t st;
};
#define FC_ACTIVE 1u
#define FC_FRESH 2u
#define FC_BACKWARD 4u
#define FC_GET(st, sh, bits) (((st) >> (sh)) & ((1u << (bits)) - 1))
#define FC_SET(st, sh, bits, v) ((st) = ((st) & ~(((1u << (bits)) - 1) << (sh))) | ((uint32_t)(v) << (sh)))

template <int S>
__global__ void __launch_bounds__(256) k_scan_flags_sm(const uint64_t* __restrict__ codes, const uint64_t* __restrict__ pm,
                                                       const uint64_t* __restrict__ need, uint64_t T, uint64_t n_words, FdParams fp,
                                                       const uint32_t* __restrict__ bloom, unsigned long long* ff, unsigned long long* fb,
                                                       unsigned long long* cf0, unsigned long long* cf1, unsigned long long* cb0,
                                                       unsigned long long* cb1, DevCounters* cnt) {
    __shared__ FlagPool pools[4];
    const int wid = (int)(threadIdx.x >> 6);
    const int lane = fd_lane();
    const uint64_t lt_mask = (1ULL << lane) - 1;
    const uint64_t n_waves = ((uint64_t)gridDim.x * blockDim.x) >> 6;
    const uint64_t wv = ((uint64_t)blockIdx.x * blockDim.x + threadIdx.x) >> 6;
    const uint64_t n_groups = (n_words + 63) / 64;
    uint64_t grp = wv * n_groups / n_waves;
    const uint64_t grp_end = (wv + 1) * n_groups / n_waves;
    unsigned long long n_eval = 0, n_piece = 0;
    int next = 0, total = 0;
    uint64_t pool_word0 = 0;
    FlagChain ch[S];
#pragma unroll
    for (int q = 0; q < S; q++) ch[q].st = 0;

    for (;;) {
        uint64_t idle[S];
        uint64_t any_idle = 0;
#pragma unroll
        for (int q = 0; q < S; q++) { idle[q] = __ballot(!(ch[q].st & FC_ACTIVE)); any_idle |= idle[q]; }
        while (any_idle && (next < total || grp < grp_end)) {
            if (next == total) {
                const uint64_t w = grp * 64 + lane;
                uint64_t f = 0, b = 0;
                if (w < n_words) {
                    const uint64_t tmask = (w + 1) * 64 <= T ? ~0ULL : (T > w * 64 ? (1ULL << (T - w * 64)) - 1 : 0ULL);
                    const uint64_t pmw = pm[w] & tmask, nd = need[w] & tmask;
                    f = nd & pmw & ((pmw >> 1) | (pm[w + 1] << 63));
                    b = nd & pmw & ((pmw << 1) | (w ? pm[w - 1] >> 63 : 0ULL));
                    n_eval += __popcll(nd);
                    n_piece += __popcll(pmw);
                }
                const int c = __popcll(f) + __popcll(b);
                int incl = c;
#pragma unroll
                for (int d = 1; d < 64; d <<= 1) {
                    const int o = __shfl_up(incl, d, 64);
                    if (lane >= d) incl += o;
                }
                pools[wid].mf[lane] = f;
                pools[wid].mb[lane] = b;
                pools[wid].excl[lane] = incl - c;
                total = __builtin_amdgcn_readlane(incl, 63);
                next = 0;
                pool_word0 = grp * 64;
                grp++;
                __builtin_amdgcn_fence(__ATOMIC_RELEASE, "wavefront");
                __builtin_amdgcn_wave_barrier();
                __builtin_amdgcn_fence(__ATOMIC_ACQUIRE, "wavefront");
                continue;
            }
#pragma unroll
            for (int q = 0; q < S; q++) {
                const int r = __popcll(idle[q] & lt_mask);
                const int avail = total - next;
                if (!(ch[q].st & FC_ACTIVE) && r < avail) {
                    const int t = next + r;
                    int sl = 0;
#pragma unroll
                    for (int step = 32; step > 0; step >>= 1)
                        if (pools[wid].excl[sl + step] <= t) sl += step;
                    const uint64_t f = pools[wid].mf[sl], b = pools[wid].mb[sl];
                    const int within = t - pools[wid].excl[sl], cf = __popcll(f);
                    const bool backward = within >= cf;
                    const int bit = backward ? select_bit(b, within - cf) : select_bit(f, within);
                    const uint64_t iw = pool_word0 + sl;
                    const uint64_t pos = iw * 64 + bit;
                    const uint64_t km = fd_kmer_at(codes, pos, fp.k);
                    int real;
                    if (!backward) {
                        ch[q].key = km;
                        real = fd_base_at(codes, pos + fp.k);
                    } else {
                        ch[q].key = fd_revcomp(km, fp.k);
                        real = fd_base_at(codes, pos - 1) ^ 2;
                    }
                    ch[q].w = (uint32_t)iw;
                    uint32_t st = FC_ACTIVE | FC_FRESH | (backward ? FC_BACKWARD : 0u);
                    FC_SET(st, 3, 2, real);
                    FC_SET(st, 5, 3, real == 0 ? 1 : 0);
                    FC_SET(st, 17, 6, bit);
                    ch[q].st = st;
                }
                next += min(__popcll(idle[q]), avail > 0 ? avail : 0);
            }
            any_idle = 0;
#pragma unroll
            for (int q = 0; q < S; q++) { idle[q] = __ballot(!(ch[q].st & FC_ACTIVE)); any_idle |= idle[q]; }
        }
        bool mine = false;
#pragma unroll
        for (int q = 0; q < S; q++) mine |= (ch[q].st & FC_ACTIVE) != 0;
        if (!__ballot(mine)) break;
        uint32_t word[S];
        uint32_t sh[S];
#pragma unroll
        for (int q = 0; q < S; q++) {
            word[q] = 0;
            sh[q] = 0;
            if (ch[q].st & FC_ACTIVE) {
                if (ch[q].st & FC_FRESH) {
                    const uint32_t jn = FC_GET(ch[q].st, 8, 3);
                    const uint64_t alt = ((ch[q].key << 2) | (uint64_t)FC_GET(ch[q].st, 5, 3)) & fp.kmask;
                    const uint64_t e = jn == 0 ? alt : ((alt << 2) | (uint64_t)(jn - 1)) & fp.kmask;
                    fd_hash_pair(fd_canon(e, fp.k), fp.tai_mask, ch[q].hA, ch[q].hB);
                    FC_SET(ch[q].st, 11, 4, 0);
                    ch[q].st &= ~FC_FRESH;
                }
                const uint64_t p = (ch[q].hA + (uint64_t)FC_GET(ch[q].st, 11, 4) * ch[q].hB) & fp.tai_mask;
                word[q] = bloom[p >> 5];
                sh[q] = (uint32_t)(p & 31);
            }
        }
#pragma unroll
        for (int q = 0; q < S; q++) {
            uint32_t st = ch[q].st;
            if (st & FC_ACTIVE) {
            const bool bit = (word[q] >> sh[q]) & 1u;
            const uint32_t real = FC_GET(st, 3, 2);
            uint32_t jn = FC_GET(st, 8, 3), h = FC_GET(st, 11, 4), njc = FC_GET(st, 15, 2), nt = FC_GET(st, 5, 3);
            bool done = false, flag = false;
            if (bit && h + 1 < (uint32_t)fp.n_hash) {
                h++;
            } else if (bit) {
                if (jn == 0) {
                    njc++;
                    if (fp.j == 0) { done = true; flag = true; }
                    else { jn = 1; st |= FC_FRESH; }
                } else {
                    done = true;
                    flag = true;
                }
            } else {
                if (jn >= 1 && jn < 4) {
                    jn++;
                    st |= FC_FRESH;
                } else {
                    nt++;
                    if (nt == real) nt++;
                    if (nt > 3) done = true;
                    else { jn = 0; st |= FC_FRESH; }
                }
            }
            FC_SET(st, 8, 3, jn);
            FC_SET(st, 11, 4, h);
            FC_SET(st, 15, 2, njc);
            FC_SET(st, 5, 3, nt & 7);
            if (done) {
                const unsigned long long bm = 1ULL << FC_GET(st, 17, 6);
                const uint32_t iw = ch[q].w;
                if (!(st & FC_BACKWARD)) {
                    if (flag) atomicOr(&ff[iw], bm);
                    if (njc & 1) atomicOr(&cf0[iw], bm);
                    if (njc & 2) atomicOr(&cf1[iw], bm);
                } else {
                    if (flag) atomicOr(&fb[iw], bm);
                    if (njc & 1) atomicOr(&cb0[iw], bm);
                    if (njc & 2) atomicOr(&cb1[iw], bm);
                }
                st &= ~FC_ACTIVE;
            }
            ch[q].st = st;
            }
        }
    }
    block_add(&cnt->flag_positions, n_eval);
    block_add(&cnt->piece_positions, n_piece);
}

__global__ void __launch_bounds__(256) k_probe_stage3(const uint64_t* __restrict__ kmers, uint64_t n, int mode, FdParams fp,
                                                      const uint32_t* __restrict__ bloom, signed char* __restrict__ out) {
    const uint64_t i = (uint64_t)blockIdx.x * blockDim.x + threadIdx.x;
    if (i >= n) return;
    const uint64_t km = kmers[i] & fp.kmask;
    int r;
    if (mode == 0) {
        r = jcheck_dfs(km, fp, bloom) ? 1 : 0;
    } else if (mode == 1) {
        r = -1;
        for (int nt = 0; nt < 4; nt++) {
            const uint64_t e = ((km << 2) | (uint64_t)nt) & fp.kmask;
            if (fd_bloom_contains_canon(bloom, fd_canon(e, fp.k), fp.tai_mask, fp.n_hash) && jcheck_dfs(e, fp, bloom)) {
                if (r != -1) { r = -2; break; }
                r = nt;
            }
        }
    } else {
        int paths = 0;
        for (int nt = 0; nt < 4; nt++) paths += jcheck_dfs(((km << 2) | (uint64_t)nt) & fp.kmask, fp, bloom) ? 1 : 0;
        r = paths > 1 ? 1 : 0;
    }
    out[i] = (signed char)r;
}

}

void fgpu_touch_scan_pure() {
    hipFuncAttributes attr;
    (void)hipFuncGetAttributes(&attr, (const void*)k_scan_same);
}

int fgpu_util_probe_stage3(fgpu_ctx* ctx, const uint64_t* d_kmers, uint64_t n, int mode, signed char* d_out) {
    FGPU_LAUNCH("probe_stage3", k_probe_stage3, fgpu_blocks(n, 256), 256, d_kmers, n, mode, ctx->fd, (const uint32_t*)ctx->bloo2, d_out);
    return FGPU_OK;
}

int fgpu_stage_scan_pure(fgpu_ctx* ctx, uint64_t* n_pieces) {
    BatchBufs& bb = *ctx->cur;
    *n_pieces = 0;
    bb.n_pieces = 0;
    if (bb.T == 0) return FGPU_OK;
    const uint64_t wb = (bb.n_words + FGPU_PADW) * 8;
    int rc;
    DevBuf* planes[] = {&bb.valid, &bb.pm, &bb.ps, &bb.ff, &bb.fb, &bb.cf0, &bb.cf1, &bb.cb0, &bb.cb1, &bb.inF, &bb.inB, &bb.lk, &bb.nF, &bb.nB, &bb.need};
    for (DevBuf* b : planes)
        if ((rc = fgpu_ensure_b(ctx, b, wb))) return rc;
    if ((rc = fgpu_ensure_b(ctx, &bb.ps_prefix, (bb.n_words + FGPU_PADW + bb.n_words / SCAN_BLOCK + 2) * 4))) return rc;
    const double t_a = fgpu_host_now();
    FGPU_HIP(hipMemsetAsync(bb.valid.p, 0, wb, ctx->stream));
    FGPU_HIP(hipMemsetAsync(bb.pm.p, 0, wb, ctx->stream));
    FGPU_HIP(hipMemsetAsync(bb.ps.p, 0, wb, ctx->stream));

    const unsigned grid = fgpu_grid(bb.n_words * 64, 256);
    const unsigned wgrid = fgpu_grid(bb.n_words, 256);
    if ((rc = fgpu_util_count_segments(ctx, ctx->cur->bad.p, ctx->cur->n_words, ctx->fd.k + 2 * ctx->fd.j + 1))) return rc;
    const uint64_t kept_index = ctx->scan_resident_base + ctx->scan_batch_index;
    const ResidentBatch* kept = kept_index < ctx->resident_count ? ctx->resident[kept_index] : nullptr;
    ctx->scan_batch_index++;
    if (kept && (kept->T != bb.T || kept->n_words != bb.n_words)) kept = nullptr;
    if (kept) {
        if ((rc = fgpu_ensure_b(ctx, &bb.same, 64))) return rc;
        FGPU_HIP(hipMemsetAsync(bb.same.p, 0x01, 4, ctx->stream));
        const uint64_t ncw = 2 * bb.n_words;
        FGPU_LAUNCH("scan_same", k_scan_same, fgpu_grid(ncw, 256), 256, (const uint64_t*)bb.codes.p, (const uint64_t*)kept->codes_p(), ncw,
                    (const uint64_t*)bb.bad.p, (const uint64_t*)kept->bad_p(), bb.n_words, (uint32_t*)bb.same.p);
    }
    FGPU_LAUNCH("scan_valid", k_scan_valid, grid, 256, (const uint64_t*)bb.codes.p, (const uint64_t*)bb.bad.p, bb.T, bb.n_words, ctx->fd,
                (const uint32_t*)ctx->bloo2, kept ? (const uint64_t*)kept->sure.p : (const uint64_t*)nullptr,
                kept ? (const uint32_t*)bb.same.p : (const uint32_t*)nullptr, (uint64_t*)bb.valid.p, ctx->counters);
    const int check_segment = ctx->fd.k < 2 * ctx->fd.j + 2;
    FGPU_LAUNCH("scan_pieces", k_scan_pieces, wgrid, 256, (const uint64_t*)bb.valid.p, (const uint64_t*)bb.bad.p, bb.n_words, ctx->fd,
                check_segment, (unsigned long long*)bb.pm.p, (uint64_t*)bb.ps.p, ctx->counters);
    uint32_t* prefix = (uint32_t*)bb.ps_prefix.p;
    uint32_t* block_sums = prefix + bb.n_words + FGPU_PADW;
    const uint32_t nblk = fgpu_blocks(bb.n_words + 1, SCAN_BLOCK);
    const uint64_t nw1 = bb.n_words + 1;
    FGPU_LAUNCH("prefix_block", k_prefix_block, nblk, SCAN_BLOCK, (const uint64_t*)bb.ps.p, nw1, prefix, block_sums);
    FGPU_LAUNCH("prefix_sums", k_prefix_sums, 1, SCAN_BLOCK, block_sums, nblk);
    FGPU_LAUNCH("prefix_apply", k_prefix_apply, fgpu_blocks(nw1, 256), 256, prefix, (const uint32_t*)block_sums, nw1);
    FGPU_HIP(hipMemcpyAsync(ctx->counters_host, ctx->counters, sizeof(DevCounters), hipMemcpyDeviceToHost, ctx->stream));
    const double t_b = fgpu_host_now();
    FGPU_HIP(fgpu_sync_stream(ctx, ctx->stream));
    const double t_c = fgpu_host_now();
    ctx->host_ms[2] += t_b - t_a;
    ctx->host_ms[3] += t_c - t_b;
    bb.max_piece_span = ctx->counters_host->max_read_len + 64;
    const uint64_t np = ctx->counters_host->pieces - ctx->scan_pieces_seen;
    ctx->scan_pieces_seen = ctx->counters_host->pieces;
    *n_pieces = np;
    bb.n_pieces = np;
    if ((rc = fgpu_ensure_b(ctx, &bb.pieces, (np + 1) * sizeof(uint2)))) return rc;
    if (np) {
        FGPU_LAUNCH("piece_list", k_scan_piece_list, wgrid, 256, (const uint64_t*)bb.ps.p, (const uint64_t*)bb.pm.p,
                    (const uint32_t*)prefix, bb.n_words, (uint2*)bb.pieces.p);
        if (ctx->record_stops) {
            if ((rc = fgpu_ensure_b(ctx, &bb.piece_read, np * 4))) return rc;
            FGPU_LAUNCH("piece_read", k_scan_piece_read, fgpu_blocks(np, 256), 256, (const uint2*)bb.pieces.p, np, bb.d_offs, bb.n_reads,
                        (uint32_t*)bb.piece_read.p);
        }
        if ((rc = fgpu_stage_scan_need(ctx))) return rc;
        DevBuf* outs[] = {&bb.ff, &bb.fb, &bb.cf0, &bb.cf1, &bb.cb0, &bb.cb1};
        for (DevBuf* o : outs) FGPU_HIP(hipMemsetAsync(o->p, 0, wb, ctx->stream));
        const unsigned flags_grid = (unsigned)std::min<uint64_t>(std::max<uint64_t>(bb.n_words / 16, 1), 2 * FGPU_GRID_BLOCKS);
        static const int sm_blocks = getenv("FGPU_FLAGS_SM_BLOCKS") ? atoi(getenv("FGPU_FLAGS_SM_BLOCKS")) : 4096;
        if (ctx->fd.j <= 1 && sm_blocks > 0) {
            const unsigned sm_grid = (unsigned)std::min<uint64_t>(std::max<uint64_t>((bb.n_words + 255) / 256, 1), (uint64_t)sm_blocks);
            static const int sm_slots = getenv("FGPU_FLAGS_SM_SLOTS") ? atoi(getenv("FGPU_FLAGS_SM_SLOTS")) : 1;
#define FGPU_FLAGS_SM(SLOTS)                                                                                                        \
    FGPU_LAUNCH("scan_flags", k_scan_flags_sm<SLOTS>, sm_grid, 256, (const uint64_t*)bb.codes.p, (const uint64_t*)bb.pm.p,           \
                (const uint64_t*)bb.need.p, bb.T, bb.n_words, ctx->fd, (const uint32_t*)ctx->bloo2, (unsigned long long*)bb.ff.p,    \
                (unsigned long long*)bb.fb.p, (unsigned long long*)bb.cf0.p, (unsigned long long*)bb.cf1.p,                         \
                (unsigned long long*)bb.cb0.p, (unsigned long long*)bb.cb1.p, ctx->counters)
            if (sm_slots <= 1) FGPU_FLAGS_SM(1);
            else if (sm_slots == 2) FGPU_FLAGS_SM(2);
            else if (sm_slots == 3) FGPU_FLAGS_SM(3);
            else FGPU_FLAGS_SM(4);
#undef FGPU_FLAGS_SM
        } else
        FGPU_LAUNCH("scan_flags", k_scan_flags, flags_grid, 256, (const uint64_t*)bb.codes.p, (const uint64_t*)bb.pm.p,
                    (const uint64_t*)bb.need.p, bb.T, bb.n_words, ctx->fd, (const uint32_t*)ctx->bloo2, (unsigned long long*)bb.ff.p,
                    (unsigned long long*)bb.fb.p, (unsigned long long*)bb.cf0.p, (unsigned long long*)bb.cf1.p,
                    (unsigned long long*)bb.cb0.p, (unsigned long long*)bb.cb1.p, ctx->counters);
        if ((rc = fgpu_stage_scan_debug_drop(ctx))) return rc;
    }
    ctx->host_ms[4] += fgpu_host_now() - t_c;
    return FGPU_OK;
}
```

### faucet_amd/csrc/scan_walk.hip

```cpp
#include <cstring>
#include <algorithm>

#include "fgpu_flags.h"
#include "walk_tables.h"

namespace {

__device__ __forceinline__ uint32_t uf_find(uint32_t* parent, uint32_t x) {
    uint32_t p = ld_agent(&parent[x]);
    while (p != x) {
        uint32_t gp = ld_agent(&parent[p]);
        if (gp != p) atomicMin(&parent[x], gp);
        x = p;
        p = gp;
    }
    return x;
}

__device__ __forceinline__ void uf_union(uint32_t* parent, uint32_t a, uint32_t b) {
    for (;;) {
        a = uf_find(parent, a);
        b = uf_find(parent, b);
        if (a == b) return;
        if (a < b) { uint32_t t = a; a = b; b = t; }
// ... 1881 lines not shown
        for (int o = 32; o > 0; o >>= 1) { n0 += __shfl_down(n0, o, 64); n1 += __shfl_down(n1, o, 64); }
        if (fd_lane() == 0) {
            if (n0) atomicAdd(&ot.state[6], n0);
            if (n1) atomicAdd(&ot.state[7], n1);
            __threadfence();
            if (atomicAdd(&ot.state[5], 1u) + 1u == gridDim.x * (blockDim.x / 64)) {
                const unsigned a = atomicAdd(&ot.state[6], 0u), b = atomicAdd(&ot.state[7], 0u);
                atomicMax(&cnt->ovw_fill, (unsigned long long)(a > b ? a : b));
            }
        }
    }
    const int settled = ovw_settled_round(ot.state, rounds);
    unsigned long long v[8] = {0, 0, 0, 0, 0, 0, 0, 0};
    if (settled >= 0) {
        const uint4* log = ot.log;
        const uint32_t* res_all = ot.res;
        const uint32_t n = ot.state[0] < ot.list_cap ? ot.state[0] : ot.list_cap;
        if (blockIdx.x == 0 && threadIdx.x == 0 && n) v[7] = (unsigned long long)settled + 1;
        const WinDesc wd = *wdp;
        for (uint32_t idx = blockIdx.x * blockDim.x + threadIdx.x; idx < n; idx += gridDim.x * blockDim.x) {
            const uint32_t li = ot.list[idx];
            const uint32_t r = root[li];
            if (!ot.longp[r] && !kt.bad[r]) {
                if (r == li) {
                    if (count_followers) atomicAdd(&cnt->followers, (unsigned long long)count[r]);
                    atomicMax(&cnt->max_cluster, (unsigned long long)count[r] + 1);
                }
                const uint2 pc = pl.pieces[wd.first_piece + li];
                const uint32_t* res = res_all + 8 * idx;
                const uint4* lg = log + 2ULL * kt.piece_base[li];
                const uint64_t seq = piece_seq_base + wd.first_piece + li;
                for (uint32_t i = 0; i < res[0]; i++) {
                    const uint4 e = lg[i];
                    const uint32_t tn = e.y & 0xFFFF, flags = (e.y >> 16) & 0xFF;
                    const uint64_t pos = pc.x + (tn >> 1);
                    if (flags & OVW_F_CREATED) {
                        const uint64_t slot = e.x >> 1;
                        jt.stamps[e.x] = (seq << STAMP_SHIFT) | ((flags & OVW_F_FAKE) ? STAMP_FAKE : (uint64_t)tn);
                        atomicOr((unsigned long long*)&jt.keys[slot], 1ULL << (62 + (e.x & 1)));
                        const uint64_t hb = jt_filter_bit(jt, ld_agent(&jt.keys[slot]) & J_KEYMASK);
                        atomicOr(&jt.filter[hb >> 5], 1u << (hb & 31));
                        atomicOr(&pl.cr[pos >> 6], 1ULL << (pos & 63));
                        v[4]++;
                    }
                    if (pl.sF && !(flags & OVW_F_FAKE)) atomicOr(&((tn & 1) ? pl.sF : pl.sB)[pos >> 6], 1ULL << (pos & 63));
                    ovw_apply((uint64_t*)(jt.recs + (uint64_t)e.x * 16), tn, flags, e.y >> 24, e.z & 0xFF);
                }
                v[0] += res[1]; v[1] += res[2]; v[2] += res[3]; v[3] += res[4]; v[5] += res[5]; v[6] += 1;
                if (res[6]) atomicOr(&cnt->error_flags, 4ULL);
            }
        }
    }
    walk_counters_flush(cnt, v[0], v[1], v[2], v[3]);
    wave_add(&cnt->n_junctions, v[4]);
    wave_add(&cnt->flags_filled, v[5]);
    v[6] = wave_sum(v[6]);
    v[7] = wave_sum(v[7]);
    if (fd_lane() == 0) {
        if (v[6]) { atomicAdd(&cnt->walk_parallel, v[6]); atomicAdd(&cnt->ovw[0], v[6]); }
        if (v[7]) { atomicAdd(&cnt->ovw[1], v[7]); atomicAdd(&cnt->ovw[2], 1ULL); }
        if (blockIdx.x == 0 && settled < 0 && kt.state[3]) atomicAdd(&cnt->ovw[3], 1ULL);
        if (blockIdx.x == 0 && settled < 0 && kt.state[3] && ot.state[1]) atomicAdd(&cnt->ko_overflows, 1ULL);
    }
}

__global__ void __launch_bounds__(256) k_delta_collect(unsigned long long* __restrict__ cr, const uint32_t* __restrict__ kh, uint64_t w_first, uint64_t n_words,
                                                       uint32_t* __restrict__ list, unsigned long long* __restrict__ count, Planes pl,
                                                       const WinDesc* __restrict__ wdp, DevCounters* cnt, uint32_t win_seq) {
    __shared__ unsigned s_wave[4];
    __shared__ unsigned long long s_base;
    __shared__ uint32_t s_late_h[FGPU_LATE_CAP];
    __shared__ uint64_t s_late_p[FGPU_LATE_CAP];
    __shared__ uint32_t s_late_n;
    if (threadIdx.x == 0) s_late_n = 0;
    if (blockIdx.x == 0 && threadIdx.x == 0) { cnt->walked_pieces += wdp->n; cnt->followers_seen = ld_agent((const uint64_t*)&cnt->followers); }
    __syncthreads();
    const unsigned long long n_noted = cnt->late_n[0] < FGPU_LATE_CAP ? cnt->late_n[0] : FGPU_LATE_CAP;
    if (n_noted) {
        if (threadIdx.x < n_noted && cnt->late[2 * threadIdx.x + 1] == win_seq) {
            const uint32_t at = atomicAdd(&s_late_n, 1u);
            s_late_p[at] = cnt->late[2 * threadIdx.x];
            s_late_h[at] = kh[cnt->late[2 * threadIdx.x]];
        }
        __syncthreads();
    }
    const uint32_t n_late = s_late_n;
    const int wave = (int)(threadIdx.x >> 6);
    for (uint64_t w0 = w_first + (uint64_t)blockIdx.x * 256; w0 < n_words; w0 += (uint64_t)gridDim.x * 256) {
        const uint64_t w = w0 + threadIdx.x;
        if (n_late && w < n_words) {
            const WinDesc wd = *wdp;
            uint64_t inside = pl.pm[w];
            while (inside) {
                const uint64_t pos = w * 64 + (uint64_t)__builtin_ctzll(inside);
                inside &= inside - 1;
                const uint32_t h = kh[pos];
                for (uint32_t e = 0; e < n_late; e++) {
                    uint32_t li;
                    uint2 pc;
                    if (h == s_late_h[e] && piece_in_window(pl, wd, pos, li, pc)) {
                        if (pos == s_late_p[e]) {
                            atomicAdd(&cnt->late_n[2], 1ULL);
                        } else {
                            atomicOr(&cnt->error_flags, 4ULL);
                            atomicAdd(&cnt->late_n[1], 1ULL);
                        }
                    }
                }
            }
        }
        unsigned long long m = w < n_words ? cr[w] : 0ULL;
        if (m) cr[w] = 0;
        unsigned mine = (unsigned)__popcll(m), incl = mine;
        for (int o = 1; o < 64; o <<= 1) { const unsigned t = __shfl_up(incl, o, 64); if (fd_lane() >= o) incl += t; }
        if (fd_lane() == 63) s_wave[wave] = incl;
        __syncthreads();
        if (threadIdx.x == 0) {
            const unsigned total = s_wave[0] + s_wave[1] + s_wave[2] + s_wave[3];
            s_base = total ? atomicAdd(count, (unsigned long long)total) : 0ULL;
        }
        __syncthreads();
        unsigned long long at = s_base + (incl - mine);
        for (int q = 0; q < wave; q++) at += s_wave[q];
        while (m) {
            const int b = __builtin_ctzll(m);
            m &= m - 1;
            list[at++] = kh[w * 64 + (uint64_t)b];
        }
        __syncthreads();
    }
}

__global__ void __launch_bounds__(256) k_walk_reset_uf(uint32_t* parent, uint32_t* count, uint32_t* head, uint32_t* par_fail, uint32_t n, uint4* wbits,
                                                       uint32_t wbits_vec) {
    for (uint32_t a = blockIdx.x * blockDim.x + threadIdx.x; a < n; a += gridDim.x * blockDim.x) {
        parent[a] = a;
        count[a] = 0;
        head[a] = U_INF;
        par_fail[a] = 0;
    }
    for (uint32_t a = blockIdx.x * blockDim.x + threadIdx.x; a < wbits_vec; a += gridDim.x * blockDim.x) wbits[a] = make_uint4(0, 0, 0, 0);
}

__global__ void __launch_bounds__(256) k_fill_u64(uint64_t* p, uint64_t n, uint64_t v) {
    uint64_t i = (uint64_t)blockIdx.x * blockDim.x + threadIdx.x;
    uint64_t stride = (uint64_t)gridDim.x * blockDim.x;
    for (; i < n; i += stride) p[i] = v;
}
__global__ void k_debug_stall(unsigned long long ticks) {
    const unsigned long long t0 = wall_clock64();
    while (wall_clock64() - t0 < ticks) __builtin_amdgcn_s_sleep(32);
}

__global__ void __launch_bounds__(256) k_debug_need_drop(uint64_t n_words, uint64_t* __restrict__ ff, uint64_t* __restrict__ fb,
                                                         uint64_t* need, uint64_t* cf0, uint64_t* cf1, uint64_t* cb0, uint64_t* cb1, int mode,
                                                         const uint64_t* __restrict__ pm, const uint32_t* __restrict__ kh) {
    for (uint64_t w = (uint64_t)blockIdx.x * blockDim.x + threadIdx.x; w < n_words; w += (uint64_t)gridDim.x * blockDim.x) {
        uint64_t drop = need[w] & ~(ff[w] | fb[w]) & fd_mix(w * 0x9E3779B97F4A7C15ULL + 12345);
        if (mode == 2) {
            drop = 0;
            for (uint64_t m = need[w] & pm[w]; m; m &= m - 1) {
                const int b = __builtin_ctzll(m);
                if ((fd_mix((uint64_t)kh[w * 64 + (uint64_t)b] + 0x1234567ULL) & 15) == 0) drop |= 1ULL << b;
            }
        }
        need[w] &= ~drop;
        cf0[w] &= ~drop; cf1[w] &= ~drop; cb0[w] &= ~drop; cb1[w] &= ~drop;
        if (mode == 2) { ff[w] &= ~drop; fb[w] &= ~drop; }
    }
}

__global__ void __launch_bounds__(256) k_need_lookup(const uint64_t* __restrict__ codes, const uint64_t* __restrict__ pm, uint64_t n_words,
                                                     FdParams fp, JTable jt, uint64_t* __restrict__ nF, uint64_t* __restrict__ nB,
                                                     uint32_t* __restrict__ kh, uint64_t w_first) {
    const uint64_t total = n_words * 64;
    for (uint64_t p = w_first * 64 + (uint64_t)blockIdx.x * blockDim.x + threadIdx.x; p < total; p += (uint64_t)gridDim.x * blockDim.x) {
        bool inF = false, inB = false;
        if ((pm[p >> 6] >> (p & 63)) & 1ULL) {
            uint64_t km = fd_kmer_at(codes, p, fp.k);
            uint64_t rc = fd_revcomp(km, fp.k);
            uint64_t canon = km < rc ? km : rc;
            const uint32_t h32 = jt_h32(canon);
            kh[p] = h32;
            const uint64_t hb = jt_filter_bit_h(jt, h32);
            if ((jt.filter[hb >> 5] >> (hb & 31)) & 1u) {
                uint32_t present = jt_present_snapshot(jt, canon);
                inF = (present >> (km == canon ? 0 : 1)) & 1u;
                inB = (present >> (rc == canon ? 0 : 1)) & 1u;
            }
        }
        uint64_t mF = __ballot(inF), mB = __ballot(inB);
        if (fd_lane() == 0) { nF[p >> 6] = mF; nB[p >> 6] = mB; }
    }
}

__global__ void __launch_bounds__(256) k_refresh_lookup(const uint64_t* __restrict__ codes, const uint64_t* __restrict__ pm, uint64_t n_words,
                                                        FdParams fp, JTable jt, const uint32_t* __restrict__ filter, uint64_t filter_mask,
                                                        uint64_t* __restrict__ nF, uint64_t* __restrict__ nB, const uint32_t* __restrict__ kh, int merge,
                                                        uint64_t* __restrict__ cand) {
    const uint64_t total = n_words * 64;
    for (uint64_t p = (uint64_t)blockIdx.x * blockDim.x + threadIdx.x; p < total; p += (uint64_t)gridDim.x * blockDim.x) {
        bool inF = false, inB = false, hitC = false;
        if ((pm[p >> 6] >> (p & 63)) & 1ULL) {
            const uint32_t h32 = kh[p];
            const uint64_t hb = ((((uint64_t)(h32 * 0x9E3779B1u) << 16) ^ (uint64_t)(h32 >> 7)) & filter_mask);
            const bool maybe = merge ? (filter[hb >> 5] & delta_bits(h32)) == delta_bits(h32) : (((filter[hb >> 5] >> (hb & 31)) & 1u) != 0);
            if (maybe) {
                hitC = true;
                const uint64_t km = fd_kmer_at(codes, p, fp.k);
                const uint64_t rc = fd_revcomp(km, fp.k);
                const uint64_t canon = km < rc ? km : rc;
                const uint32_t present = jt_present_snapshot(jt, canon);
                inF = (present >> (km == canon ? 0 : 1)) & 1u;
                inB = (present >> (rc == canon ? 0 : 1)) & 1u;
            }
        }
        const uint64_t mF = __ballot(inF), mB = __ballot(inB);
        if (cand) {
            const uint64_t mC = __ballot(hitC);
            if (fd_lane() == 0 && mC) cand[p >> 6] |= mC;
        }
        if (fd_lane() == 0) {
            if (merge) { if (mF) nF[p >> 6] |= mF; if (mB) nB[p >> 6] |= mB; }
            else { nF[p >> 6] = mF; nB[p >> 6] = mB; }
        }
    }
}

__global__ void k_dbg_diff(const uint64_t* a, const uint64_t* b, uint64_t n, unsigned long long* out, int slot) {
    unsigned long long d = 0;
    for (uint64_t i = (uint64_t)blockIdx.x * blockDim.x + threadIdx.x; i < n; i += (uint64_t)gridDim.x * blockDim.x) d += a[i] != b[i];
    if (d) atomicAdd(&out[slot], d);
}
__device__ __forceinline__ void need_mark(unsigned long long* need, uint64_t a, uint64_t z) {
    while (a < z) {
        uint64_t wi = a >> 6;
        uint64_t hi = (wi + 1) << 6;
        uint64_t upto = z < hi ? z : hi;
        int lo_b = (int)(a & 63), n_b = (int)(upto - a);
        unsigned long long m = (n_b == 64 ? ~0ULL : ((1ULL << n_b) - 1)) << lo_b;
        atomicOr(&need[wi], m);
        a = upto;
    }
}

__global__ void __launch_bounds__(256) k_need_prewalk(const uint64_t* __restrict__ codes, const uint2* __restrict__ pieces, uint64_t n_pieces,
                                                      FdParams fp, JTable jt, const uint64_t* __restrict__ nF, const uint64_t* __restrict__ nB,
                                                      unsigned long long* need, int tight) {
    for (uint64_t i = (uint64_t)blockIdx.x * blockDim.x + threadIdx.x; i < n_pieces; i += (uint64_t)gridDim.x * blockDim.x) {
        const uint2 pc = pieces[i];
        const uint64_t p0 = pc.x;
        const uint32_t nwin = pc.y;
        const int k = fp.k, j = fp.j;
        const int tmax = 2 * (int)nwin - 2 - 2 * j;
        int t = 2 * j + 1;
        while (t <= tmax) {
            int t_ev = 0x7fffffff;
            const uint32_t q0 = (uint32_t)(t >> 1);
            for (uint32_t qc = q0; qc < nwin && 2 * (int)qc <= tmax; qc += 64) {
                uint64_t eF = fd_bits_at(nF, p0 + qc), eB = fd_bits_at(nB, p0 + qc);
                if (qc == q0 && (t & 1)) eB &= ~1ULL;
                const uint32_t rem = nwin - qc;
                if (rem < 64) { const uint64_t m = (1ULL << rem) - 1; eF &= m; eB &= m; }
                const int tb = eB ? 2 * (int)(qc + __builtin_ctzll(eB)) : 0x7fffffff;
                const int tf = eF ? 2 * (int)(qc + __builtin_ctzll(eF)) + 1 : 0x7fffffff;
                const int te = tb < tf ? tb : tf;
                if (te != 0x7fffffff) { t_ev = te; break; }
            }
            if (t_ev > tmax) {
                need_mark(need, p0 + (uint64_t)(t >> 1), p0 + (uint64_t)(tmax >> 1) + 1);
                break;
            }
            if (tight >= 1) { if (t < t_ev) need_mark(need, p0 + (uint64_t)(t >> 1), p0 + (uint64_t)((t_ev - 1) >> 1) + 1); }
            else need_mark(need, p0 + (uint64_t)(t >> 1), p0 + (uint64_t)(t_ev >> 1) + 1);
            const uint32_t q = (uint32_t)(t_ev >> 1);
            const bool fwd = t_ev & 1;
            const uint64_t km = fd_kmer_at(codes, p0 + q, k);
            const uint64_t rc = fd_revcomp(km, k);
            const uint64_t key = fwd ? km : rc;
            const uint64_t canon = km < rc ? km : rc;
            const int orient = key == canon ? 0 : 1;
            const int ext_fwd = fwd ? fd_base_at(codes, p0 + q + k) : 4;
            uint64_t s = fd_mix(canon) & jt.mask;
            int d = 1;
            for (uint64_t n = 0; n <= jt.mask; n++) {
                const uint64_t w = jt.keys[s];
                if (w == J_EMPTY) break;
                if ((w & J_KEYMASK) == canon) {
                    const uint8_t dv = jt.recs[(s * 2 + orient) * 16 + ext_fwd];
                    d = dv < 1 ? 1 : dv;
                    break;
                }
                s = (s + 1) & jt.mask;
            }
            const int land = t_ev + d;
            if (land > tmax) break;
            const uint32_t lq = (uint32_t)(land >> 1);
            const uint64_t lbits = (land & 1) ? fd_bits_at(nF, p0 + lq) : fd_bits_at(nB, p0 + lq);
            if (!(lbits & 1ULL) && tight < 2) {
                need_mark(need, p0 + lq, p0 + (uint64_t)(tmax >> 1) + 1);
                break;
            }
            t = land;
        }
    }
}

__global__ void __launch_bounds__(256) k_delta_filter_add(const uint32_t* __restrict__ list, const unsigned long long* __restrict__ count, uint32_t* dfilter,
                                                          uint64_t dmask) {
    const uint64_t n = *count;
    for (uint64_t i = (uint64_t)blockIdx.x * blockDim.x + threadIdx.x; i < n; i += (uint64_t)gridDim.x * blockDim.x) {
        const uint32_t h32 = list[i];
        atomicOr(&dfilter[delta_word(h32, dmask)], delta_bits(h32));
    }
}

}

void fgpu_touch_scan_walk() {
    hipFuncAttributes attr;
    (void)hipFuncGetAttributes(&attr, (const void*)k_iota_u32);
}

int fgpu_scan_alloc(fgpu_ctx* ctx) {
    if (ctx->jkeys) return FGPU_OK;
    ctx->jcap = ctx->prm.junction_capacity;
    if (const char* e = getenv("FGPU_WBITS_LOG2")) ctx->wbits_log2 = std::min(28, std::max(16, atoi(e)));
    if (const char* e = getenv("FGPU_WALK_KO")) ctx->walk_ko = (uint32_t)std::max(0, atoi(e));
    ctx->walk_ko_always = getenv("FGPU_WALK_KO_ALWAYS") != nullptr || (ctx->prm.flags & FGPU_FLAG_KEY_ORDER_FROM_START) != 0;
    if ((ctx->prm.flags & FGPU_FLAG_KEY_ORDER_FROM_START) && !getenv("FGPU_WALK_KO")) ctx->walk_ko = 32;
    ctx->walk_ko_weight = (ctx->prm.flags & FGPU_FLAG_KEY_ORDER_FROM_START) ? 128u : 0u;
    if (const char* e = getenv("FGPU_WALK_KO_WEIGHT")) ctx->walk_ko_weight = (uint32_t)std::max(0, atoi(e));
    if (const char* e = getenv("FGPU_OVW_EV_LOG2")) ctx->ovw_ev_log2 = std::min(27, std::max(8, atoi(e)));
    if (const char* e = getenv("FGPU_OVW_ROUNDS")) ctx->ovw_rounds = std::max(0, atoi(e));
    ctx->ko_hk_cap = 1u << 22;
    ctx->ko_occ_cap = 1u << 24;
    if (const char* e = getenv("FGPU_WALK_HEAVY")) ctx->walk_heavy = (uint32_t)std::max(0, atoi(e));
    {
        size_t free_b = 0, total_b = 0;
        if (hipMemGetInfo(&free_b, &total_b) == hipSuccess)
            while (ctx->max_span > FGPU_MAX_SPAN && 40ULL * ctx->max_span > free_b / 4) ctx->max_span >>= 1;
        (void)hipGetLastError();
    }
    for (;;) {
        while (ctx->max_span / (uint64_t)(ctx->fd.k + 1) + 2 >= W_OWNER_MASK) ctx->max_span >>= 1;
        ctx->wcap = 4 * ctx->max_span;
        ctx->wmax = (uint32_t)(ctx->max_span / (uint64_t)(ctx->fd.k + 1) + 2);
        struct { void** p; uint64_t bytes; } want[] = {
            {(void**)&ctx->jkeys, ctx->jcap * 8}, {(void**)&ctx->jrecs, ctx->jcap * 32}, {(void**)&ctx->jstamps, ctx->jcap * 16}, {(void**)&ctx->jfilter, ctx->jcap * 2 / 8},
            {(void**)&ctx->wdesc, 64}, {(void**)&ctx->wkeys, ctx->wcap * 8},
            {(void**)&ctx->wbits, 2 * (1ULL << ctx->wbits_log2) / 8},
            {(void**)&ctx->uf_parent, 2ULL * ctx->wmax * 4},
            {(void**)&ctx->cl_count, 2ULL * ctx->wmax * 4}, {(void**)&ctx->cl_offset, 2ULL * ctx->wmax * 4}, {(void**)&ctx->cl_fill, (uint64_t)ctx->wmax * 4},
            {(void**)&ctx->cl_fail, 2ULL * ctx->wmax * 4}, {(void**)&ctx->ko_hk, (uint64_t)ctx->ko_hk_cap * 4 * 3},
            {(void**)&ctx->ko_occ, (uint64_t)ctx->ko_occ_cap * (4 * 3 + 8)}, {(void**)&ctx->ko_piece, (uint64_t)ctx->wmax * 4 * 2 + 64},
            {(void**)&ctx->cl_members, (uint64_t)ctx->wmax * 4 * 2}, {(void**)&ctx->cl_roots, (uint64_t)ctx->wmax * 4 + 64}};
        hipError_t err = hipSuccess;
        uint64_t failed_bytes = 0;
        for (auto& w : want) {
            *w.p = nullptr;
            if ((err = hipMalloc(w.p, w.bytes)) != hipSuccess) { *w.p = nullptr; failed_bytes = w.bytes; break; }
        }
        if (err == hipSuccess) return FGPU_OK;
        (void)hipGetLastError();
        for (auto& w : want) { if (*w.p) hipFree(*w.p); *w.p = nullptr; }
        if (ctx->max_span <= FGPU_MAX_SPAN) {
            ctx->err = std::string("the scan's tables do not fit the device (hipMalloc of ") + std::to_string(failed_bytes) + " bytes: " + hipGetErrorString(err) + ")";
            return FGPU_ERR_NOMEM;
        }
        ctx->max_span >>= 1;
    }
}

int fgpu_scan_reset(fgpu_ctx* ctx) {
    if (int rc = fgpu_scan_clear_table(ctx)) return rc;
    if (!ctx->wt_epoch) FGPU_HIP(hipMemsetAsync(ctx->wkeys, 0, ctx->wcap * 8, ctx->stream));
    FGPU_HIP(hipMemsetAsync(ctx->wbits, 0, 2 * (1ULL << ctx->wbits_log2) / 8, ctx->stream));
    FGPU_LAUNCH("iota", k_iota_u32, 64, 256, ctx->uf_parent, (uint64_t)ctx->wmax);
    FGPU_LAUNCH("iota", k_iota_u32, 64, 256, ctx->uf_parent + ctx->wmax, (uint64_t)ctx->wmax);
    FGPU_HIP(hipMemsetAsync(ctx->cl_count, 0, 2 * ctx->wmax * 4, ctx->stream));
    FGPU_HIP(hipMemsetAsync(ctx->cl_offset, 0xFF, 2 * ctx->wmax * 4, ctx->stream));
    FGPU_HIP(hipMemsetAsync(ctx->cl_fail, 0, 2 * ctx->wmax * 4, ctx->stream));
    FGPU_HIP(hipMemsetAsync(ctx->ko_hk, 0xFF, (size_t)ctx->ko_hk_cap * 4 * 2, ctx->stream));
    FGPU_HIP(hipMemsetAsync(ctx->ko_hk + 2 * (size_t)ctx->ko_hk_cap, 0, (size_t)ctx->ko_hk_cap * 4, ctx->stream));
    FGPU_HIP(hipMemsetAsync(ctx->ko_piece, 0, (size_t)ctx->wmax * 4 * 2 + 64, ctx->stream));
    return FGPU_OK;
}

int fgpu_stage_scan_need(fgpu_ctx* ctx) {
    BatchBufs& bb = *ctx->cur;
    const uint64_t wb = (bb.n_words + FGPU_PADW) * 8;
    const bool eager = (ctx->prm.flags & FGPU_FLAG_EAGER_FLAGS) || ctx->eager_runtime || ctx->eager_scan;
    FGPU_HIP(hipMemsetAsync(bb.need.p, eager ? 0xFF : 0, wb, ctx->stream));
    if (!bb.n_pieces) return FGPU_OK;
    if (int rc = fgpu_ensure_b(ctx, &bb.kh, (bb.n_words + FGPU_PADW) * 64 * 4)) return rc;

    static const int need_tight = getenv("FGPU_NEED_TIGHT") ? atoi(getenv("FGPU_NEED_TIGHT")) : 2;
    JTable jt = make_jt(ctx);
    FGPU_LAUNCH("need_lookup", k_need_lookup, fgpu_grid(bb.n_words * 64, 256), 256, (const uint64_t*)bb.codes.p, (const uint64_t*)bb.pm.p,
                bb.n_words, ctx->fd, jt, (uint64_t*)bb.nF.p, (uint64_t*)bb.nB.p, (uint32_t*)bb.kh.p, (uint64_t)0);
    if (eager) return FGPU_OK;
    FGPU_LAUNCH("need_prewalk", k_need_prewalk, fgpu_grid(bb.n_pieces, 256), 256, (const uint64_t*)bb.codes.p, (const uint2*)bb.pieces.p,
                bb.n_pieces, ctx->fd, jt, (const uint64_t*)bb.nF.p, (const uint64_t*)bb.nB.p, (unsigned long long*)bb.need.p, need_tight);
    return FGPU_OK;
}

int fgpu_scan_refresh_planes(fgpu_ctx* ctx, BatchBufs* b) {
    if (!b->n_pieces || !b->T) return FGPU_OK;
    JTable jt = make_jt(ctx);
    ctx->launch_stream = ctx->stream;
    FGPU_LAUNCH("need_lookup", k_refresh_lookup, fgpu_grid(b->n_words * 64, 256), 256, (const uint64_t*)b->codes.p, (const uint64_t*)b->pm.p, b->n_words,
                ctx->fd, jt, (const uint32_t*)jt.filter, jt.filter_mask, (uint64_t*)b->nF.p, (uint64_t*)b->nB.p, (const uint32_t*)b->kh.p, 0, (uint64_t*)nullptr);
    if (b->pure_done) FGPU_HIP(hipEventRecord(b->pure_done, ctx->stream));
    return FGPU_OK;
}

int fgpu_scan_build_cand(fgpu_ctx* ctx, BatchBufs* b) {
    b->cand_gen = 0;
    if (!b->n_pieces || !b->T) return FGPU_OK;
    int rc;
    const uint64_t wb = (b->n_words + FGPU_PADW) * 8;
    if ((rc = fgpu_ensure_b(ctx, &b->cand, wb)) || (rc = fgpu_ensure(ctx, &ctx->cand_filter, (1ULL << CAND_FILTER_LOG2) / 8))) return rc;
    ctx->launch_stream = ctx->stream;
    FGPU_HIP(hipMemsetAsync(ctx->cand_filter.p, 0, (1ULL << CAND_FILTER_LOG2) / 8, ctx->stream));
    FGPU_HIP(hipMemsetAsync(b->cand.p, 0, wb, ctx->stream));
    const unsigned word_blocks = std::min(fgpu_blocks(b->n_words, 256), 2048u), piece_blocks = std::min(fgpu_blocks(b->n_pieces, 256), 2048u);
    FGPU_LAUNCH("cand_plane", k_cand_mark, word_blocks + piece_blocks, 256, (const uint64_t*)b->pm.p, (const uint64_t*)b->nF.p, (const uint64_t*)b->nB.p,
                (const uint64_t*)b->ff.p, (const uint64_t*)b->fb.p, (const uint32_t*)b->kh.p, b->n_words, (const uint2*)b->pieces.p, b->n_pieces, ctx->fd,
                (uint32_t*)ctx->cand_filter.p, word_blocks);
    FGPU_LAUNCH("cand_plane", k_cand_probe, fgpu_grid(b->n_words * 64, 256), 256, (const uint64_t*)b->pm.p, (const uint32_t*)b->kh.p, b->n_words,
                (const uint32_t*)ctx->cand_filter.p, (uint64_t*)b->cand.p);
    if (b->pure_done) FGPU_HIP(hipEventRecord(b->pure_done, ctx->stream));
    b->cand_gen = ctx->hint_gen;
    return FGPU_OK;
}

int fgpu_stage_scan_debug_drop(fgpu_ctx* ctx) {
    static const int drop = getenv("FGPU_DEBUG_NEED_DROP") ? atoi(getenv("FGPU_DEBUG_NEED_DROP")) : 0;
    BatchBufs& bb = *ctx->cur;
    if (!drop || !bb.n_pieces) return FGPU_OK;
    if (drop == 2 && ((ctx->prm.flags & FGPU_FLAG_EAGER_FLAGS) || ctx->eager_runtime || ctx->eager_scan)) return FGPU_OK;
    FGPU_LAUNCH("debug_need_drop", k_debug_need_drop, fgpu_grid(bb.n_words, 256), 256, bb.n_words, (uint64_t*)bb.ff.p, (uint64_t*)bb.fb.p,
                (uint64_t*)bb.need.p, (uint64_t*)bb.cf0.p, (uint64_t*)bb.cf1.p, (uint64_t*)bb.cb0.p, (uint64_t*)bb.cb1.p, drop,
                (const uint64_t*)bb.pm.p, (const uint32_t*)bb.kh.p);
    return FGPU_OK;
}

static int env_int(const char* name, int absent) { const char* e = getenv(name); return e ? atoi(e) : absent; }
static bool env_is_one(const char* name) { const char* e = getenv(name); return e && e[0] == '1'; }
struct WalkKnobs {
    const int dbg_walk = env_int("FGPU_DEBUG_WALK", 0);
    const bool serial_clean = env_is_one("FGPU_SERIAL_CLEAN");
    const bool no_overlap = env_is_one("FGPU_NO_OVERLAP");
    const bool no_whole_batch = getenv("FGPU_NO_WHOLE_BATCH") != nullptr;
    const unsigned cluster_grid = (unsigned)std::max(1, env_int("FGPU_CLUSTER_GRID", 256));
    const uint64_t refresh_div = (uint64_t)std::max(1, env_int("FGPU_REFRESH_DIV", 4));
    const unsigned delta_per_block = (unsigned)std::max(1, env_int("FGPU_DELTA_PER_BLOCK", 1024));
    const int ko_avg = getenv("FGPU_WALK_KO_AVG") ? std::min(255, std::max(0, env_int("FGPU_WALK_KO_AVG", 0))) : -1;
    const int ko_avg_min = getenv("FGPU_WALK_KO_AVG_MIN") ? std::min(255, std::max(1, env_int("FGPU_WALK_KO_AVG_MIN", 0))) : -1;
    const uint32_t ko_ticket = (uint32_t)std::max(64, env_int("FGPU_KO_TICKET", 64) / 64 * 64);
    const int ovw_followers = env_int("FGPU_OVW_FOLLOWERS", 0);
    const bool ovw_beside = !env_is_one("FGPU_OVW_SERIAL");
    const unsigned walk_dyn_grid = (unsigned)std::max(1, env_int("FGPU_WALK_DYN_GRID", 1024));
    const bool dbg_span = getenv("FGPU_DEBUG_SPAN") != nullptr;
};
static const WalkKnobs& walk_knobs() { static const WalkKnobs knobs; return knobs; }

struct WalkBatch {
    BatchBufs& bb;
    Planes pl;
    JTable jt;
    uint64_t T, ext, seq_base;
    hipStream_t walk_stream, ovw_stream;
    bool cand_ok;
    DeltaList* created;
};

struct WalkWindow {
    uint64_t lo, hi, pos_end;
    int parity;
    uint64_t max_pieces;
    uint32_t *uf_parent, *cl_count, *cl_offset, *cl_fail;
    WTable wt;
    uint32_t *roots_state, *root_list;
};

struct LargeClusterRule {
    uint32_t ko_heavy;
    uint32_t ko_heavy_w;
    uint32_t heavy;
    int ovw_rounds;
    bool ovw_on;
};

constexpr int OVW_MARK_LOG2 = 22;

template <class FullPass>
static int walk_dbg_compare(fgpu_ctx* ctx, hipStream_t st, const uint64_t* plane0, const uint64_t* plane1, uint64_t n_words, FullPass full, const char* what,
                            uint64_t batch, uint64_t lo) {
    uint64_t* scratch = nullptr;
    unsigned long long* out = nullptr;
    FGPU_HIP(hipMalloc(&scratch, 2 * n_words * 8));
    FGPU_HIP(hipMalloc(&out, 32));
    FGPU_HIP(hipMemsetAsync(out, 0, 32, st));
    FGPU_HIP(full(scratch));
    hipLaunchKernelGGL(k_dbg_diff, dim3(64), dim3(256), 0, st, (const uint64_t*)scratch, plane0, n_words, out, 0);
    if (plane1) hipLaunchKernelGGL(k_dbg_diff, dim3(64), dim3(256), 0, st, (const uint64_t*)(scratch + n_words), plane1, n_words, out, 1);
    unsigned long long h[4] = {0, 0, 0, 0};
    FGPU_HIP(hipMemcpyAsync(h, out, 32, hipMemcpyDeviceToHost, st));
    FGPU_HIP(hipStreamSynchronize(st));
    ctx->refresh_mismatch += h[0] + h[1];
    if (h[0] + h[1]) fprintf(stderr, "[fgpu] %s: %llu + %llu words differ, batch %llu window at %llu\n", what, h[0], h[1], (unsigned long long)batch, (unsigned long long)lo);
    (void)hipFree(scratch); (void)hipFree(out);
    return FGPU_OK;
}

static int walk_refresh_prepared(fgpu_ctx* ctx, BatchBufs& bb, const JTable& jt, hipStream_t walk_stream, bool* cand_ok) {
    *cand_ok = false;
    if (!(ctx->delta_ready && bb.planes_gen == ctx->hint_gen)) {
        FGPU_LAUNCH("walk_lookup", k_refresh_lookup, fgpu_grid(bb.n_words * 64, 256), 256, (const uint64_t*)bb.codes.p, (const uint64_t*)bb.pm.p, bb.n_words,
                    ctx->fd, jt, (const uint32_t*)jt.filter, jt.filter_mask, (uint64_t*)bb.nF.p, (uint64_t*)bb.nB.p, (const uint32_t*)bb.kh.p, 0, (uint64_t*)nullptr);
        ctx->refresh_full++;
        return FGPU_OK;
    }
    *cand_ok = !ctx->no_sparse_link && bb.cand.p && bb.cand_gen == ctx->hint_gen;
    if (ctx->delta_keys || ctx->refresh_delta)
        FGPU_LAUNCH("walk_lookup", k_refresh_lookup, fgpu_grid(bb.n_words * 64, 256), 256, (const uint64_t*)bb.codes.p, (const uint64_t*)bb.pm.p, bb.n_words,
                    ctx->fd, jt, (const uint32_t*)ctx->delta_filter.p, ctx->delta_filter_bits - 1, (uint64_t*)bb.nF.p, (uint64_t*)bb.nB.p,
                    (const uint32_t*)bb.kh.p, 1, *cand_ok ? (uint64_t*)bb.cand.p : (uint64_t*)nullptr);
    ctx->refresh_delta++;
    if (!ctx->dbg_delta_check) return FGPU_OK;
    const auto full = [&](uint64_t* scratch) {
        hipLaunchKernelGGL(k_refresh_lookup, dim3(fgpu_grid(bb.n_words * 64, 256)), dim3(256), 0, walk_stream, (const uint64_t*)bb.codes.p, (const uint64_t*)bb.pm.p,
                           bb.n_words, ctx->fd, jt, (const uint32_t*)jt.filter, jt.filter_mask, scratch, scratch + bb.n_words, (const uint32_t*)bb.kh.p, 0,
                           (uint64_t*)nullptr);
        return hipSuccess;
    };
    return walk_dbg_compare(ctx, walk_stream, (const uint64_t*)bb.nF.p, (const uint64_t*)bb.nB.p, bb.n_words, full, "merged in-map planes against planes made again",
                            bb.seq, 0);
}

static int walk_window_begin(fgpu_ctx* ctx, const WalkBatch& wb, uint64_t lo, uint64_t hi, WalkWindow* w) {
    const int parity = (int)(ctx->scan_windows & 1);
    const uint64_t set = parity * (uint64_t)ctx->wmax;
    FGPU_HIP(hipStreamWaitEvent(wb.walk_stream, ctx->ev_uf_reset[parity], 0));
    if (++ctx->wt_epoch > 255) {
        FGPU_HIP(hipMemsetAsync(ctx->wkeys, 0, ctx->wcap * 8, wb.walk_stream));
        ctx->wt_epoch = 1;
    }
    const uint64_t max_pieces = std::min<uint64_t>((hi - lo) / (uint64_t)(ctx->fd.k + 1) + 2, ctx->wmax);
    *w = WalkWindow{lo, hi, std::min<uint64_t>(wb.T, hi + wb.ext), parity, max_pieces, ctx->uf_parent + set, ctx->cl_count + set, ctx->cl_offset + set, ctx->cl_fail + set,
                    make_wt(ctx, ctx->wt_epoch, parity),
                    ctx->cl_roots, ctx->cl_roots + 16};
    return FGPU_OK;
}

static int walk_register(fgpu_ctx* ctx, const WalkKnobs& kn, const WalkBatch& wb, const WalkWindow& w) {
    const BatchBufs& bb = wb.bb;
    DeltaSrc ds;
    memset(&ds, 0, sizeof(ds));
    const uint64_t delta_est = ctx->delta_ring_keys + (uint64_t)(3.0 * (double)bb.n_pieces * (double)w.lo / (double)wb.T);
    const bool refresh_window = !ctx->refresh_snapshot && delta_est > (w.pos_end - w.lo) / kn.refresh_div;
    if (refresh_window) {
        const uint64_t w_first = w.lo >> 6, w_last = std::min<uint64_t>(bb.n_words, (w.pos_end + 63) / 64);
        FGPU_LAUNCH("walk_lookup", k_need_lookup, fgpu_grid((w_last - w_first) * 64, 256), 256, (const uint64_t*)bb.codes.p, (const uint64_t*)bb.pm.p, w_last,
                    ctx->fd, wb.jt, (uint64_t*)bb.nF.p, (uint64_t*)bb.nB.p, (uint32_t*)bb.kh.p, w_first);
    } else {
        if (!ctx->refresh_snapshot)
            for (int r = 1; r < FGPU_DELTA_RING && (uint64_t)r <= ctx->delta_next; r++) {
                const DeltaList& dl = ctx->delta_ring[(ctx->delta_next - r) % FGPU_DELTA_RING];
                ds.list[r - 1] = (const uint32_t*)dl.list.p;
                ds.count[r - 1] = (const unsigned long long*)dl.count.p;
            }
        if (w.lo) {
            ds.list[FGPU_DELTA_RING - 1] = (const uint32_t*)wb.created->list.p;
            ds.count[FGPU_DELTA_RING - 1] = (const unsigned long long*)wb.created->count.p;
        }
    }
    const unsigned word_blocks = fgpu_blocks((w.pos_end - (w.lo & ~63ULL) + 63) / 64, 256);
    const unsigned piece_blocks = fgpu_blocks(w.max_pieces, 256);
    const unsigned delta_blocks = refresh_window ? 64u : (unsigned)std::min<uint64_t>(4096, std::max<uint64_t>(64, delta_est / kn.delta_per_block));
    FGPU_LAUNCH("walk_lookup", k_walk_register, word_blocks + piece_blocks + delta_blocks, 256, wb.pl, ctx->fd, w.wt, w.uf_parent, w.lo, w.hi, w.pos_end, ctx->counters,
                word_blocks, piece_blocks, ds);
    return FGPU_OK;
}

static int walk_link(fgpu_ctx* ctx, const WalkBatch& wb, const WalkWindow& w) {
    const BatchBufs& bb = wb.bb;
    const unsigned full_grid = std::min(fgpu_blocks(w.pos_end - (w.lo & ~63ULL), 1024), 4096u);
    if (!(wb.cand_ok && w.lo == 0)) {
        FGPU_LAUNCH("walk_link", k_walk_link, full_grid, 256, wb.pl, ctx->fd, w.wt, w.uf_parent, w.lo, w.hi, w.pos_end, w.roots_state);
        if (ctx->refresh_snapshot) ctx->full_links++;
        return FGPU_OK;
    }
    const uint64_t link_words = ((w.pos_end + 63) >> 6) - (w.lo >> 6);
    uint64_t* const lk = (uint64_t*)bb.lk.p + (w.lo >> 6);
    FGPU_LAUNCH("walk_link", k_walk_link_sparse, std::min(fgpu_blocks(link_words, 256), 4096u), 256, wb.pl, ctx->fd, w.wt, w.uf_parent, w.lo, w.hi, w.pos_end,
                w.roots_state, (const uint64_t*)bb.cand.p, (uint64_t*)bb.lk.p);
    ctx->sparse_links++;
    if (!ctx->dbg_delta_check) return FGPU_OK;
    const auto full = [&](uint64_t* scratch) {
        const hipError_t e = hipMemcpyAsync(scratch, lk, link_words * 8, hipMemcpyDeviceToDevice, wb.walk_stream);
        hipLaunchKernelGGL(k_walk_link, dim3(full_grid), dim3(256), 0, wb.walk_stream, wb.pl, ctx->fd, w.wt, w.uf_parent, w.lo, w.hi, w.pos_end, (uint32_t*)nullptr);
        return e;
    };
    return walk_dbg_compare(ctx, wb.walk_stream, (const uint64_t*)lk, (const uint64_t*)nullptr, link_words, full, "sparse link pass: lk plane against the full pass's",
                            bb.seq, w.lo);
}

static LargeClusterRule large_cluster_rule(fgpu_ctx* ctx, const WalkKnobs& kn) {
    const DevCounters& seen = *ctx->counters_host;
    LargeClusterRule r;
    r.ko_heavy = (kn.dbg_walk || !ctx->walk_ko || !(ctx->walk_ko_always || seen.max_cluster >= ctx->walk_ko)) ? 0u : ctx->walk_ko;
    const bool repeats_seen = seen.walk_parallel * 50 > seen.walked_pieces ||
                              (ctx->walk_ko_always && seen.walked_pieces < (1ULL << 17) && ctx->delta_next >= 2 && ctx->repeats_seen_before);
    if (repeats_seen) ctx->repeats_seen_before = true;
    const uint32_t ko_total = std::min<uint32_t>(ctx->walk_ko_weight, 0xFFFFu);
    const uint32_t ko_avg = kn.ko_avg >= 0 ? (uint32_t)kn.ko_avg : repeats_seen ? 8u : 12u;
    const uint32_t ko_total_rep = kn.ko_avg_min > 0 ? (uint32_t)kn.ko_avg_min : repeats_seen ? 16u : std::min<uint32_t>(255u, 3 * ko_total / 8);
    r.ko_heavy_w = (r.ko_heavy && ko_total) ? (ko_total | (ko_avg << 16) | (ko_total_rep << 24)) : 0u;
    r.heavy = (kn.dbg_walk || r.ko_heavy) ? 0u : ctx->walk_heavy;
    r.ovw_rounds = !r.ko_heavy ? 0 : std::min(ctx->ovw_rounds, OVW_MAX_ROUNDS);
    const bool ovw_seen_enough = seen.walked_pieces >= (1ULL << 17);
    r.ovw_on = r.ovw_rounds > 0 && ((ctx->walk_ko_always && (ctx->delta_next < 2 || !ovw_seen_enough)) || seen.walk_parallel * 256 > seen.walked_pieces);
    return r;
}

static int walk_large_tables(fgpu_ctx* ctx, const WalkBatch& wb, const LargeClusterRule& rule, KoTables& kt, OvwTables& ot) {
    kt.hk_key = ctx->ko_hk;
    kt.hk_head = ctx->ko_hk + ctx->ko_hk_cap;
    kt.hk_turn = ctx->ko_hk + 2 * (size_t)ctx->ko_hk_cap;
    kt.hk_mask = ctx->ko_hk_cap - 1;
    kt.occ_id = (uint64_t*)ctx->ko_occ;
    kt.occ_entry = (uint32_t*)(kt.occ_id + ctx->ko_occ_cap);
    kt.occ_rank = kt.occ_entry + ctx->ko_occ_cap;
    kt.occ_next = kt.occ_rank + ctx->ko_occ_cap;
    kt.occ_cap = ctx->ko_occ_cap;
    kt.trace = nullptr;
#ifdef FGPU_KO_TRACE
    if (!ctx->ko_trace.p) {
        if (int trc = fgpu_ensure(ctx, &ctx->ko_trace, ((1ULL << 23) + 4096 * 1024) * 8)) return trc;
        FGPU_HIP(hipMemsetAsync(ctx->ko_trace.p, 0, 32, ctx->stream));
    }
    kt.trace = (unsigned long long*)ctx->ko_trace.p;
#endif
    kt.state = ctx->ko_piece;
    kt.piece_base = ctx->ko_piece + 16;
    kt.bad = kt.piece_base + ctx->wmax;
    memset(&ot, 0, sizeof(ot));
    {
        const uint64_t fill = ctx->counters_host->ovw_fill;
        int want = ctx->ovw_ev_log2;
        while (want < 27 && fill * 4 > (1ULL << want)) want++;
        if (want != ctx->ovw_ev_log2) {
            while (want < 27 && fill * 8 > (1ULL << want)) want++;
            if (ctx->ovw_ev.p) {
                FGPU_HIP(fgpu_sync_stream(ctx, wb.walk_stream));
                if (ctx->ostream) FGPU_HIP(fgpu_sync_stream(ctx, ctx->ostream));
            }
            ctx->ovw_ev_log2 = want;
        }
    }
    if (!rule.ovw_on) return FGPU_OK;
    int rc;
    const int ev_log2 = ctx->ovw_ev_log2;
    const uint32_t filt_words = 1u << (ev_log2 + 1 - 5), list_cap = (uint32_t)std::min<uint64_t>(ctx->wmax, 1u << 20);
    const bool fresh = !ctx->ovw_ev.p || ctx->ovw_ev_log2_alloc != ev_log2;
    ctx->ovw_ev_log2_alloc = ev_log2;
    if ((rc = fgpu_ensure(ctx, &ctx->ovw_ev, 4ULL * 8 * (1ULL << ev_log2))) || (rc = fgpu_ensure(ctx, &ctx->ovw_filt, 3ULL * 4 * filt_words)) ||
        (rc = fgpu_ensure(ctx, &ctx->ovw_log, 2ULL * ctx->ko_occ_cap * sizeof(uint4))) || (rc = fgpu_ensure(ctx, &ctx->ovw_res, 32ULL * list_cap)) ||
        (rc = fgpu_ensure(ctx, &ctx->ovw_marks, 3ULL * 4 * (1ULL << OVW_MARK_LOG2))) ||
        (rc = fgpu_ensure(ctx, &ctx->ovw_list, 4ULL * list_cap)) || (rc = fgpu_ensure(ctx, &ctx->ovw_state, 4ULL * (8 + OVW_MAX_ROUNDS) + 64)) ||
        (rc = fgpu_ensure(ctx, &ctx->ovw_longp, 4ULL * ctx->wmax)))
        return rc;
    if (fresh || ctx->ovw_epoch + (uint32_t)rule.ovw_rounds > 255) {
        FGPU_HIP(hipMemsetAsync(ctx->ovw_ev.p, 0, 4ULL * 8 * (1ULL << ev_log2), wb.walk_stream));
        ctx->ovw_epoch = 0;
    }
    ot.list = (uint32_t*)ctx->ovw_list.p;
    ot.list_cap = list_cap;
    ot.state = (uint32_t*)ctx->ovw_state.p;
    ot.longp = (uint32_t*)ctx->ovw_longp.p;
    ot.filt_words = filt_words;
    return FGPU_OK;
}

static int walk_large_first(fgpu_ctx* ctx, const WalkKnobs& kn, const WalkBatch& wb, const WalkWindow& w, const LargeClusterRule& rule, const KoTables& kt,
                            OvwTables& ot) {
    const int ev_log2 = ctx->ovw_ev_log2;
    const uint32_t filt_words = ot.filt_words;
    uint32_t* const ovw_filt = rule.ovw_on ? (uint32_t*)ctx->ovw_filt.p : nullptr;
    if (rule.ko_heavy) {
        FGPU_LAUNCH("walk_ko_prepare", k_ko_reset, 256, 256, kt, (uint32_t)ctx->wmax, (uint32_t)w.parity);
        if (rule.ovw_on) FGPU_LAUNCH("walk_ko_prepare", k_ovw_reset, 64, 256, ot.state, ovw_filt, 3 * filt_words, ot.longp, (uint32_t)w.max_pieces,
                                     (uint32_t*)ctx->ovw_marks.p, 3u << OVW_MARK_LOG2);
        FGPU_LAUNCH("walk_ko_prepare", k_ko_prepare, fgpu_blocks(w.max_pieces, 256), 256, wb.pl, (const uint32_t*)ctx->cl_fill, (const uint32_t*)w.cl_count,
                    (const WinDesc*)ctx->wdesc, kt, rule.ko_heavy, (uint32_t)w.parity, (const uint32_t*)w.cl_fail, rule.ko_heavy_w, ot);
// ... 4 lines not shown
        FGPU_HIP(hipStreamWaitEvent(wb.ovw_stream, ctx->ev_listed, 0));
        ctx->launch_stream = wb.ovw_stream;
    }
    unsigned long long* const evb = (unsigned long long*)ctx->ovw_ev.p;
    uint32_t* const marks = (uint32_t*)ctx->ovw_marks.p;
    ot.log = (uint4*)ctx->ovw_log.p;
    ot.res = (uint32_t*)ctx->ovw_res.p;
    ot.mark_mask = (1u << OVW_MARK_LOG2) - 1;
    const unsigned ovw_grid = (unsigned)std::min<uint64_t>(fgpu_blocks(std::min<uint64_t>(w.max_pieces, ot.list_cap), 64), 2048);
    const auto table = [&](int r, uint64_t epoch) {
        OvwEv ev;
        ev.key = evb + (uint64_t)(r & 1) * 2 * (1ULL << ev_log2);
        ev.val = ev.key + (1ULL << ev_log2);
        ev.bits = ovw_filt + (uint64_t)(r % 3) * filt_words;
        ev.mask = (1ULL << ev_log2) - 1;
        ev.epoch = epoch << 56;
        ev.fshift = 32 - (ev_log2 + 1);
        return ev;
    };
    const uint64_t epoch_first = (uint64_t)ctx->ovw_epoch + 1;
    for (int r = 0; r < rule.ovw_rounds; r++) {
        ctx->ovw_epoch++;
        ot.cur = table(r, ctx->ovw_epoch);
        ot.prev = table(r + 1, ctx->ovw_epoch - 1);
        ot.prev.bits = ovw_filt + (uint64_t)((r + 2) % 3) * filt_words;
        ot.filt_next = ovw_filt + (uint64_t)((r + 1) % 3) * filt_words;
        ot.mark_cur = marks + ((uint64_t)(r % 3) << OVW_MARK_LOG2);
        ot.mark_prev = marks + ((uint64_t)((r + 2) % 3) << OVW_MARK_LOG2);
        ot.mark_next = marks + ((uint64_t)((r + 1) % 3) << OVW_MARK_LOG2);
        FGPU_LAUNCH("walk_ovw", k_ovw_round, ovw_grid, 64, wb.pl, ctx->fd, wb.jt, (const uint32_t*)ctx->cl_fill, (const WinDesc*)ctx->wdesc, kt, ot, (uint32_t)r,
                    (const uint32_t*)ctx->bloo2, ctx->counters);
    }
    FGPU_LAUNCH("walk_ovw", k_ovw_commit, ovw_grid, 64, wb.pl, ctx->fd, wb.jt, (const uint32_t*)ctx->cl_fill, (const uint32_t*)w.cl_count, (const WinDesc*)ctx->wdesc,
                wb.seq_base, kt, ot, rule.ovw_rounds, ctx->counters, kn.ovw_followers, (const unsigned long long*)evb, (uint64_t)1 << ev_log2, epoch_first);
    if (wb.ovw_stream != wb.walk_stream) {
        FGPU_HIP(hipEventRecord(ctx->ev_settled, wb.ovw_stream));
        ctx->launch_stream = wb.walk_stream;
    }
    return FGPU_OK;
}

static int walk_clusters(fgpu_ctx* ctx, const WalkKnobs& kn, const WalkBatch& wb, const WalkWindow& w, const LargeClusterRule& rule, const KoTables& kt,
                         const OvwTables& ot) {
    const unsigned walk_grid_w = fgpu_blocks(w.max_pieces, 64);
#ifdef FGPU_KO_ONE_XCD
    const unsigned ko_grid = 4096;
#else
    const unsigned ko_grid = 512;
#endif
    if (rule.heavy)
        FGPU_LAUNCH("walk_probe", k_walk_par<WALK_PROBE>, walk_grid_w, 64, wb.pl, ctx->fd, wb.jt, (const uint32_t*)ctx->cl_fill, (const uint32_t*)w.cl_count, w.cl_fail,
                    (const WinDesc*)ctx->wdesc, (const uint32_t*)ctx->bloo2, ctx->counters, rule.heavy);
    FGPU_LAUNCH("walk", k_walk_dyn, std::min(walk_grid_w, kn.walk_dyn_grid), 64, wb.pl, ctx->fd, wb.jt, (const uint32_t*)w.root_list, w.roots_state,
                (const uint32_t*)w.cl_count, (const uint32_t*)w.cl_offset, (const uint32_t*)ctx->cl_members, ctx->cl_members + ctx->wmax, (const WinDesc*)ctx->wdesc,
                wb.seq_base, (const uint32_t*)ctx->bloo2, ctx->counters, kn.dbg_walk, (const uint32_t*)w.cl_fail, rule.heavy, (const uint32_t*)kt.bad,
                (const uint32_t*)kt.state, rule.ko_heavy, (uint32_t)ctx->scan_windows, rule.ko_heavy_w);
    if (rule.ovw_on && wb.ovw_stream != wb.walk_stream) FGPU_HIP(hipStreamWaitEvent(wb.walk_stream, ctx->ev_settled, 0));
    if (rule.ko_heavy) {
        FGPU_LAUNCH("walk_ko_prepare", k_ko_rank, 256, 256, kt, (const uint32_t*)ot.state, rule.ovw_rounds);
        FGPU_LAUNCH("walk_ko", k_walk_ko, ko_grid, 64, wb.pl, ctx->fd, wb.jt, (const uint32_t*)ctx->cl_fill, (const uint32_t*)w.cl_count, (const WinDesc*)ctx->wdesc,
                    wb.seq_base, (const uint32_t*)ctx->bloo2, ctx->counters, kt, rule.ko_heavy, kn.ko_ticket, (const uint32_t*)w.cl_fail, rule.ko_heavy_w,
                    (const uint32_t*)ot.state, (const uint32_t*)ot.longp, rule.ovw_rounds);
    }
    if (rule.heavy)
        FGPU_LAUNCH("walk_commit", k_walk_par<WALK_COMMIT>, walk_grid_w, 64, wb.pl, ctx->fd, wb.jt, (const uint32_t*)ctx->cl_fill, (const uint32_t*)w.cl_count, w.cl_fail,
                    (const WinDesc*)ctx->wdesc, (const uint32_t*)ctx->bloo2, ctx->counters, rule.heavy);
    return FGPU_OK;
}

static int walk_collect_and_reset(fgpu_ctx* ctx, const WalkKnobs& kn, const WalkBatch& wb, const WalkWindow& w) {
    const BatchBufs& bb = wb.bb;
    const uint64_t w_first = w.lo >> 6, w_last = std::min<uint64_t>(bb.n_words, (w.pos_end + 63) / 64);
    FGPU_LAUNCH("walk_delta", k_delta_collect, (unsigned)std::min<uint64_t>(fgpu_blocks(w_last - w_first, 256), 256), 256, (unsigned long long*)bb.cr.p,
                (const uint32_t*)bb.kh.p, w_first, w_last, (uint32_t*)wb.created->list.p, (unsigned long long*)wb.created->count.p, wb.pl,
                (const WinDesc*)ctx->wdesc, ctx->counters, (uint32_t)ctx->scan_windows);
    FGPU_HIP(hipEventRecord(ctx->ev_walked, wb.walk_stream));
    FGPU_HIP(hipStreamWaitEvent(ctx->cstream, ctx->ev_walked, 0));
    ctx->launch_stream = ctx->cstream;
    FGPU_LAUNCH("walk_clean", k_walk_reset_uf, std::min(256u, fgpu_blocks(w.max_pieces, 256)), 256, w.uf_parent, w.cl_count, w.cl_offset, w.cl_fail, (uint32_t)w.max_pieces,
                (uint4*)w.wt.bits, (uint32_t)((1u << ctx->wbits_log2) / 128));
    ctx->launch_stream = wb.walk_stream;
    FGPU_HIP(hipEventRecord(ctx->ev_uf_reset[w.parity], ctx->cstream));
    if (kn.serial_clean) FGPU_HIP(hipStreamWaitEvent(wb.walk_stream, ctx->ev_uf_reset[w.parity], 0));
    return FGPU_OK;
}

static int walk_span_look(fgpu_ctx* ctx, const WalkKnobs& kn, hipStream_t walk_stream, uint64_t* span_now) {
    if (ctx->calib_left <= 0 || ctx->prm.walk_window_span) return FGPU_OK;
    FGPU_HIP(hipMemcpyAsync(ctx->fb_host, &ctx->counters->followers, 8, hipMemcpyDeviceToHost, walk_stream));
    FGPU_HIP(hipMemcpyAsync(ctx->fb_host + 1, &ctx->counters->walked_pieces, 8, hipMemcpyDeviceToHost, walk_stream));
    FGPU_HIP(hipMemcpyAsync(ctx->fb_host + 2, &ctx->counters->ko_overflows, 8, hipMemcpyDeviceToHost, walk_stream));
    FGPU_HIP(fgpu_sync_stream(ctx, walk_stream));
    uint64_t span = *span_now;
    const uint64_t f = ctx->fb_host[0] - ctx->calib_f, p = ctx->fb_host[1] - ctx->calib_p;
    if (ctx->fb_host[2] > ctx->calib_ovf && span > 4096) {
        ctx->calib_ovf = ctx->fb_host[2];
        ctx->calib_f = ctx->fb_host[0];
        ctx->calib_p = ctx->fb_host[1];
        span = std::max<uint64_t>(4096, span / 4);
        ctx->proven_span = std::min(ctx->proven_span, span);
        ctx->calib_left = std::max(ctx->calib_left, 4);
        ctx->span_ceiling = std::min(ctx->span_ceiling, span * 2);
        if (kn.dbg_span) fprintf(stderr, "[span] look: the large-cluster walks' tables overflowed -> span %llu, looks left %d\n", (unsigned long long)span, ctx->calib_left);
    } else if (p >= 64) {
        ctx->calib_f = ctx->fb_host[0];
        ctx->calib_p = ctx->fb_host[1];
        bool shrunk = false;
        const uint64_t ceiling = std::min<uint64_t>(ctx->max_span, ctx->span_ceiling), usual = std::min<uint64_t>(ceiling, FGPU_USUAL_SPAN);
        if (f * 2 > p && span > 4096) { span /= 2; shrunk = true; }
        else if (f * 3 < p && span < usual) span = std::min<uint64_t>(span * 4, usual);
        else if (f * 16 < p && span < ceiling) span = std::min<uint64_t>(span * 4, ceiling);
        else ctx->calib_left = 1;
        ctx->calib_left--;
        if (!shrunk && span >= (1ULL << 22)) ctx->calib_left = 0;
        if (kn.dbg_span) fprintf(stderr, "[span] look: followers %llu of %llu pieces -> span %llu, looks left %d\n", (unsigned long long)f, (unsigned long long)p,
                                 (unsigned long long)span, ctx->calib_left);
    }
    *span_now = span;
    return FGPU_OK;
}

int fgpu_stage_scan_walk(fgpu_ctx* ctx, uint64_t n_pieces) {
    if (!n_pieces) return FGPU_OK;
    const WalkKnobs& kn = walk_knobs();
    BatchBufs& bb = *ctx->cur;
    int rc;
    const uint64_t wbytes = (bb.n_words + FGPU_PADW) * 8;
    Planes pl{(const uint64_t*)bb.codes.p, (const uint64_t*)bb.pm.p, (const uint64_t*)bb.ps.p, (const uint32_t*)bb.ps_prefix.p,
              (const uint64_t*)bb.ff.p, (const uint64_t*)bb.fb.p, (const uint64_t*)bb.cf0.p, (const uint64_t*)bb.cf1.p,
              (const uint64_t*)bb.cb0.p, (const uint64_t*)bb.cb1.p, (uint64_t*)bb.nF.p, (uint64_t*)bb.nB.p, (const uint2*)bb.pieces.p,
              (uint64_t*)bb.lk.p, (const uint64_t*)bb.need.p, nullptr, nullptr, (const uint32_t*)bb.kh.p, nullptr};
    if ((rc = fgpu_ensure_b(ctx, &bb.cr, wbytes))) return rc;
    pl.cr = (unsigned long long*)bb.cr.p;
    if (ctx->record_stops) {
        if ((rc = fgpu_ensure_b(ctx, &bb.sF, wbytes)) || (rc = fgpu_ensure_b(ctx, &bb.sB, wbytes))) return rc;
        pl.sF = (unsigned long long*)bb.sF.p;
        pl.sB = (unsigned long long*)bb.sB.p;
    }
    const uint64_t span = ctx->window_span;
    const uint64_t ext = bb.max_piece_span;
    if (ctx->max_span + ext + 64 > ctx->wcap) {
        ctx->err = "a read of " + std::to_string(ext) + " bases is longer than the walk's window tables allow";
        return FGPU_ERR_CAPACITY;
    }
    if (ext >= (1ULL << (STAMP_SHIFT - 1)) - 64) {
        ctx->err = "a read of " + std::to_string(ext) + " bases is longer than the junction creation stamps allow (2^19 windows)";
        return FGPU_ERR_CAPACITY;
    }
    hipStream_t walk_stream = kn.no_overlap ? ctx->stream : ctx->wstream;
    hipStream_t ovw_stream = (kn.ovw_beside && !kn.no_overlap && ctx->ostream) ? ctx->ostream : walk_stream;
    WalkBatch wb{bb, pl, make_jt(ctx), bb.T, ext, ctx->scan_piece_base, walk_stream, ovw_stream, false, &ctx->delta_ring[ctx->delta_next % FGPU_DELTA_RING]};
    const uint64_t T = wb.T;
    ctx->launch_stream = walk_stream;
    if (bb.pure_done) FGPU_HIP(hipStreamWaitEvent(walk_stream, bb.pure_done, 0));
    if (ctx->dbg_stall_us) FGPU_LAUNCH("debug_stall", k_debug_stall, 1, 1, (unsigned long long)ctx->dbg_stall_us * 100ULL);
    if (ctx->refresh_snapshot && (rc = walk_refresh_prepared(ctx, bb, wb.jt, walk_stream, &wb.cand_ok))) return rc;
    if (ctx->record_stops) {
        FGPU_HIP(hipMemsetAsync(bb.sF.p, 0, wbytes, walk_stream));
        FGPU_HIP(hipMemsetAsync(bb.sB.p, 0, wbytes, walk_stream));
    }
    FGPU_HIP(hipMemsetAsync(bb.cr.p, 0, wbytes, walk_stream));
    {
        const uint64_t now = ctx->counters_host->n_junctions;
        ctx->delta_hist[ctx->delta_next % FGPU_DELTA_RING] = now;
        const uint64_t back = ctx->delta_next >= (uint64_t)(FGPU_DELTA_RING - 1) ? ctx->delta_hist[(ctx->delta_next - (FGPU_DELTA_RING - 1)) % FGPU_DELTA_RING] : 0;
        ctx->delta_ring_keys = now > back ? now - back : 0;
        ctx->delta_batch_base = now;
    }
    if ((rc = fgpu_ensure_b(ctx, &wb.created->list, (bb.n_words + FGPU_PADW) * 64 * 4)) || (rc = fgpu_ensure(ctx, &wb.created->count, 64))) return rc;
    FGPU_HIP(hipMemsetAsync(wb.created->count.p, 0, 8, walk_stream));
    const int stage_tok = fgpu_prof_begin(ctx, "walk_stage");
    ctx->prof_suppress = !ctx->prof_walk_detail;
    uint64_t span_now = span;
    const bool whole_batch = wb.cand_ok && !kn.no_whole_batch && !ctx->prm.walk_window_span && ctx->calib_left <= 0 && span * 2 >= T && span < T && T <= ctx->max_span &&
                             bb.n_pieces <= ctx->wmax;
    for (uint64_t lo = 0, step = 0; lo < T; lo += step) {
        step = whole_batch ? T : span_now;
        WalkWindow w;
        KoTables kt;
        OvwTables ot;
        if ((rc = walk_window_begin(ctx, wb, lo, std::min<uint64_t>(T, lo + step), &w))) return rc;
        if ((rc = walk_register(ctx, kn, wb, w)) || (rc = walk_link(ctx, wb, w))) return rc;
        const LargeClusterRule rule = large_cluster_rule(ctx, kn);
        FGPU_LAUNCH("walk_cluster", k_walk_cluster, std::min(kn.cluster_grid, fgpu_blocks(w.max_pieces, 256)), 256, (const uint32_t*)w.uf_parent, w.cl_count, w.cl_offset,
                    ctx->cl_fill, ctx->cl_members, pl, lo, w.hi, (WinDesc*)ctx->wdesc, ctx->counters, w.cl_fail, rule.ko_heavy_w, w.root_list, w.roots_state);
        if ((rc = walk_large_tables(ctx, wb, rule, kt, ot)) || (rc = walk_large_first(ctx, kn, wb, w, rule, kt, ot)) || (rc = walk_clusters(ctx, kn, wb, w, rule, kt, ot)) ||
            (rc = walk_collect_and_reset(ctx, kn, wb, w)))
            return rc;
        ctx->scan_windows++;
        if ((rc = walk_span_look(ctx, kn, walk_stream, &span_now))) return rc;
    }
    if (ctx->delta_ready)
        FGPU_LAUNCH("walk_delta", k_delta_filter_add, 256, 256, (const uint32_t*)wb.created->list.p, (const unsigned long long*)wb.created->count.p,
                    (uint32_t*)ctx->delta_filter.p, ctx->delta_filter_bits - 1);
    ctx->delta_next++;
    ctx->window_span = span_now;
    ctx->prof_suppress = false;
    fgpu_prof_end(ctx, stage_tok);
    if (bb.walk_done) {
        FGPU_HIP(hipEventRecord(bb.walk_done, walk_stream));
        bb.walk_pending = true;
    }
    ctx->launch_stream = ctx->stream;
    ctx->scan_piece_base += n_pieces;
    return FGPU_OK;
}
```

Baseline: 5.942 billion.

## Split pure scan into position ranges so walk starts before whole batch finishes

The pure-scan need lookup, prewalk and flag kernels now run over word ranges, and an event is recorded after each range. The walk stream waits only on the event covering the window it is about to process, instead of waiting for the whole batch's pure_done. This lets the walk of early windows overlap with the scan of later ranges. In exchange there are more, smaller kernel launches and extra event bookkeeping, and a correctness risk if a range's reach does not cover piece extents.

```diff
diff --git a/faucet_amd/csrc/api.hip b/faucet_amd/csrc/api.hip
--- a/faucet_amd/csrc/api.hip
+++ b/faucet_amd/csrc/api.hip
@@ -404,6 +404,7 @@
     for (BatchBufs* b : ctx->all_batches) {
         if (b->pure_done) hipEventDestroy(b->pure_done);
         if (b->walk_done) hipEventDestroy(b->walk_done);
+        for (hipEvent_t e : b->range_ev) if (e) hipEventDestroy(e);
         delete b;
     }
     delete ctx;
@@ -636,6 +637,17 @@
     ctx->dbg_stall_us = getenv("FGPU_DEBUG_WALK_STALL_US") ? std::min(100000, std::max(0, atoi(getenv("FGPU_DEBUG_WALK_STALL_US")))) : 0;
     ctx->dbg_delta_check = getenv("FGPU_DEBUG_DELTA_CHECK") != nullptr;
     ctx->no_sparse_link = getenv("FGPU_NO_SPARSE_LINK") != nullptr;
+    ctx->scan_range_log2 = -1;
+    if (const char* e = getenv("FGPU_SCAN_RANGE_LOG2")) {
+        char* end = nullptr;
+        const long n = strtol(e, &end, 10);
+        if (end == e || *end || (n != 0 && (n < 8 || n > 40))) {
+            ctx->err = std::string("FGPU_SCAN_RANGE_LOG2=") + e + ": 0 (one range per batch) or 8..40 (ranges of 2^n positions)";
+            return FGPU_ERR_ARG;
+        }
+        ctx->scan_range_log2 = (int)n;
+    }
+    if (fgpu_walk_no_overlap()) ctx->scan_range_log2 = 0;
     const uint64_t start_span = std::max<uint64_t>(1ULL << 18, ctx->settled_span / 4);
     ctx->window_span = ctx->prm.walk_window_span ? std::min<uint64_t>(std::max<uint64_t>(ctx->prm.walk_window_span, 64), ctx->max_span)
                                                  : std::min<uint64_t>(start_span, ctx->max_span);
@@ -700,6 +712,20 @@
     ctx->adapt_overflows = ctx->counters_host->ko_overflows;
 }
 
+static BatchBufs* new_batch(fgpu_ctx* ctx) {
+    BatchBufs* b = new BatchBufs();
+    ctx->all_batches.push_back(b);
+    hipEventCreateWithFlags(&b->pure_done, hipEventDisableTiming);
+    hipEventCreateWithFlags(&b->walk_done, hipEventDisableTiming);
+    bool all = true;
+    for (hipEvent_t& e : b->range_ev) all = hipEventCreateWithFlags(&e, hipEventDisableTiming) == hipSuccess && all;
+    if (!all) {
+        for (hipEvent_t& e : b->range_ev) { if (e) hipEventDestroy(e); e = nullptr; }
+        (void)hipGetLastError();
+    }
+    return b;
+}
+
 static BatchBufs* acquire_batch(fgpu_ctx* ctx) {
     BatchBufs* b;
     static const size_t depth = getenv("FGPU_SCAN_BUFFERS") ? (size_t)std::min(FGPU_DELTA_RING, std::max(2, atoi(getenv("FGPU_SCAN_BUFFERS")))) : 2;
@@ -708,10 +734,7 @@
         b = ctx->pool[at];
         ctx->pool.erase(ctx->pool.begin() + at);
     } else {
-        b = new BatchBufs();
-        ctx->all_batches.push_back(b);
-        hipEventCreateWithFlags(&b->pure_done, hipEventDisableTiming);
-        hipEventCreateWithFlags(&b->walk_done, hipEventDisableTiming);
+        b = new_batch(ctx);
     }
     return b;
 }
@@ -722,7 +745,7 @@
     ctx->to_harvest.push_back(b);
 }
 
-static int scan_pure_into(fgpu_ctx* ctx, BatchBufs* b, const fgpu_reads* reads) {
+static int scan_pure_into(fgpu_ctx* ctx, BatchBufs* b, const fgpu_reads* reads, bool one_range = false) {
     if (b->stops_pending) {
         int hrc = fgpu_scan_harvest(ctx, b);
         if (hrc) return hrc;
@@ -740,7 +763,7 @@
     ctx->host_ms[1] += fgpu_host_now() - t_b;
     if (!rc) rc = journal_add(ctx, b, reads);
     uint64_t n_pieces = 0;
-    if (!rc) rc = fgpu_stage_scan_pure(ctx, &n_pieces);
+    if (!rc) rc = fgpu_stage_scan_pure(ctx, &n_pieces, one_range);
     if (!rc) ctx->journal_max_read_len = std::max<uint64_t>(ctx->journal_max_read_len, ctx->counters_host->max_read_len);
     if (!rc) rc = check_errors(ctx);
     if (!rc) ctx->scan_stats.reads_processed += reads->n_reads;
@@ -886,7 +909,7 @@
             FGPU_HIP(hipMemcpyAsync(b->bad.p, j->bad.p, bbytes, hipMemcpyDeviceToDevice, ctx->stream));
         }
         uint64_t n_pieces = 0;
-        rc = fgpu_stage_scan_pure(ctx, &n_pieces);
+        rc = fgpu_stage_scan_pure(ctx, &n_pieces, true);
         if (!rc) rc = check_errors(ctx);
         if (!rc && b->pure_done) FGPU_HIP(hipEventRecord(b->pure_done, ctx->stream));
         if (!rc) rc = fgpu_scan_reserve(ctx, ctx->counters_host->n_junctions + ctx->scan_imported);
@@ -950,13 +973,8 @@
     FGPU_HIP(hipSetDevice(ctx->prm.device));
     BatchBufs* b;
     if (!ctx->pool.empty()) { b = ctx->pool.front(); ctx->pool.erase(ctx->pool.begin()); }
-    else {
-        b = new BatchBufs();
-        ctx->all_batches.push_back(b);
-        hipEventCreateWithFlags(&b->pure_done, hipEventDisableTiming);
-        hipEventCreateWithFlags(&b->walk_done, hipEventDisableTiming);
-    }
-    rc = scan_pure_into(ctx, b, reads);
+    else b = new_batch(ctx);
+    rc = scan_pure_into(ctx, b, reads, true);
     ctx->cur = &ctx->bb_default;
     if (rc == FGPU_INTERNAL_REPLAY) {
         ctx->pool.insert(ctx->pool.begin(), b);
diff --git a/faucet_amd/csrc/fgpu_ctx.h b/faucet_amd/csrc/fgpu_ctx.h
--- a/faucet_amd/csrc/fgpu_ctx.h
+++ b/faucet_amd/csrc/fgpu_ctx.h
@@ -17,6 +17,9 @@
 #define FGPU_PADW 8
 #define FGPU_USUAL_SPAN (1ULL << 26)
 #define FGPU_MAX_SPAN (1ULL << 26)
+
+#define FGPU_RANGE_EVENTS 16
+#define FGPU_RANGE_MIN (1ULL << 20)
 
 struct DevBuf {
     void*    p = nullptr;
@@ -51,6 +54,11 @@
     uint64_t n_pieces = 0;
     uint64_t max_piece_span = 0;
     hipEvent_t pure_done = nullptr;
+    hipEvent_t range_ev[FGPU_RANGE_EVENTS] = {};
+    uint64_t range_first = 0;
+    uint64_t range_span = 0;
+    uint64_t n_ranges = 0;
+    uint64_t ranges_waited = 0;
     hipEvent_t walk_done = nullptr;
     bool walk_pending = false;
     uint32_t planes_gen = 0;
@@ -286,6 +294,7 @@
     int dbg_stall_us = 0;
     bool dbg_delta_check = false;
     bool no_sparse_link = false;
+    int scan_range_log2 = -1;
     DevBuf import_probe;
     uint64_t scan_grown = 0;
 
@@ -475,14 +484,17 @@
 int fgpu_load_pair_begin(fgpu_ctx* ctx);
 int fgpu_load_pair_end(fgpu_ctx* ctx);
 void fgpu_resident_reset(fgpu_ctx* ctx, bool keep_going);
-int fgpu_stage_scan_pure(fgpu_ctx* ctx, uint64_t* n_pieces);
+int fgpu_stage_scan_pure(fgpu_ctx* ctx, uint64_t* n_pieces, bool one_range);
+bool fgpu_walk_no_overlap();
 int fgpu_stage_scan_walk(fgpu_ctx* ctx, uint64_t n_pieces);
 int fgpu_stage_scan_need(fgpu_ctx* ctx);
+int fgpu_stage_scan_need_lookup(fgpu_ctx* ctx, uint64_t w_lo, uint64_t w_hi);
+int fgpu_stage_scan_need_prewalk(fgpu_ctx* ctx, uint64_t w_lo, uint64_t w_hi);
 int fgpu_scan_refresh_planes(fgpu_ctx* ctx, BatchBufs* b);
 int fgpu_scan_build_cand(fgpu_ctx* ctx, BatchBufs* b);
 int fgpu_scan_import_probe(fgpu_ctx* ctx, const void* dev_entries, uint64_t n, uint64_t after_seq, uint32_t* dfilter, uint64_t dfilter_bits,
                            uint64_t* max_seq, uint64_t* n_newer, uint64_t digest[2]);
-int fgpu_stage_scan_debug_drop(fgpu_ctx* ctx);
+int fgpu_stage_scan_debug_drop(fgpu_ctx* ctx, uint64_t w_lo, uint64_t w_hi);
 int fgpu_util_count_segments(fgpu_ctx* ctx, const void* bad, uint64_t n_words, int minlen);
 int fgpu_util_popcount(fgpu_ctx* ctx, const void* dev, uint64_t nbytes, unsigned long long* dev_out);
 int fgpu_util_or(fgpu_ctx* ctx, void* dst, const void* src, uint64_t nbytes);
diff --git a/faucet_amd/csrc/scan_pure.hip b/faucet_amd/csrc/scan_pure.hip
--- a/faucet_amd/csrc/scan_pure.hip
+++ b/faucet_amd/csrc/scan_pure.hip
@@ -176,19 +176,19 @@
 }
 
 __global__ void __launch_bounds__(256) k_scan_flags(const uint64_t* __restrict__ codes, const uint64_t* __restrict__ pm,
-                                                    const uint64_t* __restrict__ need, uint64_t T, uint64_t n_words, FdParams fp, const uint32_t* __restrict__ bloom,
+                                                    const uint64_t* __restrict__ need, uint64_t T, uint64_t w_lo, uint64_t w_hi, FdParams fp, const uint32_t* __restrict__ bloom,
                                                     unsigned long long* ff, unsigned long long* fb, unsigned long long* cf0,
                                                     unsigned long long* cf1, unsigned long long* cb0, unsigned long long* cb1,
                                                     DevCounters* cnt) {
     const int lane = fd_lane();
     const uint64_t n_waves = ((uint64_t)gridDim.x * blockDim.x) >> 6;
-    const uint64_t n_chunks = (n_words + 3) / 4;
+    const uint64_t n_chunks = (w_hi - w_lo + 3) / 4;
     unsigned long long n_eval = 0, n_piece = 0;
     for (uint64_t chunk = ((uint64_t)blockIdx.x * blockDim.x + threadIdx.x) >> 6; chunk < n_chunks; chunk += n_waves) {
         uint64_t mine = 0;
         if (lane < 8) {
-            const uint64_t w = chunk * 4 + (lane & 3);
-            if (w < n_words) {
+            const uint64_t w = w_lo + chunk * 4 + (lane & 3);
+            if (w < w_hi) {
                 const uint64_t tmask = (w + 1) * 64 <= T ? ~0ULL : (T > w * 64 ? (1ULL << (T - w * 64)) - 1 : 0ULL);
                 const uint64_t pmw = pm[w] & tmask, nd = need[w] & tmask;
                 if (lane < 4) {
@@ -216,7 +216,7 @@
             for (int c = 1; c < 8; c++)
                 if (t >= cum[c]) { q = c; mq = m[c]; before = cum[c]; }
             const int bit = select_bit(mq, t - before);
-            const uint64_t w = chunk * 4 + (q & 3);
+            const uint64_t w = w_lo + chunk * 4 + (q & 3);
             const uint64_t pos = w * 64 + bit;
             const uint64_t km = fd_kmer_at(codes, pos, fp.k);
             bool flag;
@@ -258,7 +258,7 @@
 
 template <int S>
 __global__ void __launch_bounds__(256) k_scan_flags_sm(const uint64_t* __restrict__ codes, const uint64_t* __restrict__ pm,
-                                                       const uint64_t* __restrict__ need, uint64_t T, uint64_t n_words, FdParams fp,
+                                                       const uint64_t* __restrict__ need, uint64_t T, uint64_t w_lo, uint64_t w_hi, FdParams fp,
                                                        const uint32_t* __restrict__ bloom, unsigned long long* ff, unsigned long long* fb,
                                                        unsigned long long* cf0, unsigned long long* cf1, unsigned long long* cb0,
                                                        unsigned long long* cb1, DevCounters* cnt) {
@@ -268,7 +268,7 @@
     const uint64_t lt_mask = (1ULL << lane) - 1;
     const uint64_t n_waves = ((uint64_t)gridDim.x * blockDim.x) >> 6;
     const uint64_t wv = ((uint64_t)blockIdx.x * blockDim.x + threadIdx.x) >> 6;
-    const uint64_t n_groups = (n_words + 63) / 64;
+    const uint64_t n_groups = (w_hi - w_lo + 63) / 64;
     uint64_t grp = wv * n_groups / n_waves;
     const uint64_t grp_end = (wv + 1) * n_groups / n_waves;
     unsigned long long n_eval = 0, n_piece = 0;
@@ -285,9 +285,9 @@
         for (int q = 0; q < S; q++) { idle[q] = __ballot(!(ch[q].st & FC_ACTIVE)); any_idle |= idle[q]; }
         while (any_idle && (next < total || grp < grp_end)) {
             if (next == total) {
-                const uint64_t w = grp * 64 + lane;
+                const uint64_t w = w_lo + grp * 64 + lane;
                 uint64_t f = 0, b = 0;
-                if (w < n_words) {
+                if (w < w_hi) {
                     const uint64_t tmask = (w + 1) * 64 <= T ? ~0ULL : (T > w * 64 ? (1ULL << (T - w * 64)) - 1 : 0ULL);
                     const uint64_t pmw = pm[w] & tmask, nd = need[w] & tmask;
                     f = nd & pmw & ((pmw >> 1) | (pm[w + 1] << 63));
@@ -307,7 +307,7 @@
                 pools[wid].excl[lane] = incl - c;
                 total = __builtin_amdgcn_readlane(incl, 63);
                 next = 0;
-                pool_word0 = grp * 64;
+                pool_word0 = w_lo + grp * 64;
                 grp++;
                 __builtin_amdgcn_fence(__ATOMIC_RELEASE, "wavefront");
                 __builtin_amdgcn_wave_barrier();
@@ -469,10 +469,78 @@
     return FGPU_OK;
 }
 
-int fgpu_stage_scan_pure(fgpu_ctx* ctx, uint64_t* n_pieces) {
+static int scan_pure_flags(fgpu_ctx* ctx, uint64_t w_lo, uint64_t w_hi) {
+    BatchBufs& bb = *ctx->cur;
+    const uint64_t nw = w_hi - w_lo;
+    const unsigned flags_grid = (unsigned)std::min<uint64_t>(std::max<uint64_t>(nw / 16, 1), 2 * FGPU_GRID_BLOCKS);
+    static const int sm_blocks = getenv("FGPU_FLAGS_SM_BLOCKS") ? atoi(getenv("FGPU_FLAGS_SM_BLOCKS")) : 4096;
+    if (ctx->fd.j <= 1 && sm_blocks > 0) {
+        const unsigned sm_grid = (unsigned)std::min<uint64_t>(std::max<uint64_t>((nw + 255) / 256, 1), (uint64_t)sm_blocks);
+        static const int sm_slots = getenv("FGPU_FLAGS_SM_SLOTS") ? atoi(getenv("FGPU_FLAGS_SM_SLOTS")) : 1;
+#define FGPU_FLAGS_SM(SLOTS)                                                                                                        \
+    FGPU_LAUNCH("scan_flags", k_scan_flags_sm<SLOTS>, sm_grid, 256, (const uint64_t*)bb.codes.p, (const uint64_t*)bb.pm.p,           \
+                (const uint64_t*)bb.need.p, bb.T, w_lo, w_hi, ctx->fd, (const uint32_t*)ctx->bloo2, (unsigned long long*)bb.ff.p,    \
+                (unsigned long long*)bb.fb.p, (unsigned long long*)bb.cf0.p, (unsigned long long*)bb.cf1.p,                         \
+                (unsigned long long*)bb.cb0.p, (unsigned long long*)bb.cb1.p, ctx->counters)
+        if (sm_slots <= 1) FGPU_FLAGS_SM(1);
+        else if (sm_slots == 2) FGPU_FLAGS_SM(2);
+        else if (sm_slots == 3) FGPU_FLAGS_SM(3);
+        else FGPU_FLAGS_SM(4);
+#undef FGPU_FLAGS_SM
+    } else
+        FGPU_LAUNCH("scan_flags", k_scan_flags, flags_grid, 256, (const uint64_t*)bb.codes.p, (const uint64_t*)bb.pm.p,
+                    (const uint64_t*)bb.need.p, bb.T, w_lo, w_hi, ctx->fd, (const uint32_t*)ctx->bloo2, (unsigned long long*)bb.ff.p,
+                    (unsigned long long*)bb.fb.p, (unsigned long long*)bb.cf0.p, (unsigned long long*)bb.cf1.p,
+                    (unsigned long long*)bb.cb0.p, (unsigned long long*)bb.cb1.p, ctx->counters);
+    return FGPU_OK;
+}
+
+static void scan_range_plan(const fgpu_ctx* ctx, const BatchBufs& bb, bool one_range, uint64_t* first, uint64_t* further) {
+    const uint64_t whole = bb.n_words * 64;
+    *first = *further = whole;
+    if (one_range || !bb.range_ev[0] || ctx->scan_range_log2 == 0) return;
+    if (ctx->scan_range_log2 > 0) { *first = *further = 1ULL << ctx->scan_range_log2; return; }
+    const uint64_t span = ctx->window_span;
+    if (span >= bb.T || bb.T < 2 * FGPU_RANGE_MIN) return;
+    const uint64_t n_windows = (bb.T + span - 1) / span;
+    uint64_t m = (uint64_t)(2.0 * (double)bb.T / (3.0 * (double)span) + 0.5);
+    m = std::min<uint64_t>(std::max<uint64_t>(m, 1), n_windows - 1);
+    const uint64_t cut = (m * span + bb.max_piece_span + 63) & ~63ULL;
+    if (cut + FGPU_RANGE_MIN > bb.T) return;
+    *first = cut;
+    *further = whole - cut;
+}
+
+static int scan_pure_back(fgpu_ctx* ctx, bool one_range) {
+    BatchBufs& bb = *ctx->cur;
+    int rc;
+    uint64_t first, further;
+    scan_range_plan(ctx, bb, one_range, &first, &further);
+    const uint64_t first_words = std::max<uint64_t>(first / 64, 1), further_words = std::max<uint64_t>(further / 64, 1);
+    const uint64_t reach_words = (bb.max_piece_span + 63) / 64 + 1;
+    bb.range_first = first_words * 64;
+    bb.range_span = further_words * 64;
+    bb.n_ranges = bb.n_words <= first_words ? 1 : 1 + (bb.n_words - first_words + further_words - 1) / further_words;
+    uint64_t looked = 0;
+    for (uint64_t r = 0, lo = 0; lo < bb.n_words; r++) {
+        const uint64_t hi = std::min(bb.n_words, lo + (r ? further_words : first_words));
+        const uint64_t look_to = std::min(bb.n_words, hi + reach_words);
+        if (looked < look_to) {
+            if ((rc = fgpu_stage_scan_need_lookup(ctx, looked, look_to))) return rc;
+            looked = look_to;
+        }
+        if ((rc = fgpu_stage_scan_need_prewalk(ctx, lo, hi)) || (rc = scan_pure_flags(ctx, lo, hi)) || (rc = fgpu_stage_scan_debug_drop(ctx, lo, hi))) return rc;
+        if (bb.n_ranges > 1) FGPU_HIP(hipEventRecord(bb.range_ev[r % FGPU_RANGE_EVENTS], ctx->stream));
+        lo = hi;
+    }
+    return FGPU_OK;
+}
+
+int fgpu_stage_scan_pure(fgpu_ctx* ctx, uint64_t* n_pieces, bool one_range) {
     BatchBufs& bb = *ctx->cur;
     *n_pieces = 0;
     bb.n_pieces = 0;
+    bb.n_ranges = 0;
     if (bb.T == 0) return FGPU_OK;
     const uint64_t wb = (bb.n_words + FGPU_PADW) * 8;
     int rc;
@@ -535,27 +603,7 @@
         if ((rc = fgpu_stage_scan_need(ctx))) return rc;
         DevBuf* outs[] = {&bb.ff, &bb.fb, &bb.cf0, &bb.cf1, &bb.cb0, &bb.cb1};
         for (DevBuf* o : outs) FGPU_HIP(hipMemsetAsync(o->p, 0, wb, ctx->stream));
-        const unsigned flags_grid = (unsigned)std::min<uint64_t>(std::max<uint64_t>(bb.n_words / 16, 1), 2 * FGPU_GRID_BLOCKS);
-        static const int sm_blocks = getenv("FGPU_FLAGS_SM_BLOCKS") ? atoi(getenv("FGPU_FLAGS_SM_BLOCKS")) : 4096;
-        if (ctx->fd.j <= 1 && sm_blocks > 0) {
-            const unsigned sm_grid = (unsigned)std::min<uint64_t>(std::max<uint64_t>((bb.n_words + 255) / 256, 1), (uint64_t)sm_blocks);
-            static const int sm_slots = getenv("FGPU_FLAGS_SM_SLOTS") ? atoi(getenv("FGPU_FLAGS_SM_SLOTS")) : 1;
-#define FGPU_FLAGS_SM(SLOTS)                                                                                                        \
-    FGPU_LAUNCH("scan_flags", k_scan_flags_sm<SLOTS>, sm_grid, 256, (const uint64_t*)bb.codes.p, (const uint64_t*)bb.pm.p,           \
-                (const uint64_t*)bb.need.p, bb.T, bb.n_words, ctx->fd, (const uint32_t*)ctx->bloo2, (unsigned long long*)bb.ff.p,    \
-                (unsigned long long*)bb.fb.p, (unsigned long long*)bb.cf0.p, (unsigned long long*)bb.cf1.p,                         \
-                (unsigned long long*)bb.cb0.p, (unsigned long long*)bb.cb1.p, ctx->counters)
-            if (sm_slots <= 1) FGPU_FLAGS_SM(1);
-            else if (sm_slots == 2) FGPU_FLAGS_SM(2);
-            else if (sm_slots == 3) FGPU_FLAGS_SM(3);
-            else FGPU_FLAGS_SM(4);
-#undef FGPU_FLAGS_SM
-        } else
-        FGPU_LAUNCH("scan_flags", k_scan_flags, flags_grid, 256, (const uint64_t*)bb.codes.p, (const uint64_t*)bb.pm.p,
-                    (const uint64_t*)bb.need.p, bb.T, bb.n_words, ctx->fd, (const uint32_t*)ctx->bloo2, (unsigned long long*)bb.ff.p,
-                    (unsigned long long*)bb.fb.p, (unsigned long long*)bb.cf0.p, (unsigned long long*)bb.cf1.p,
-                    (unsigned long long*)bb.cb0.p, (unsigned long long*)bb.cb1.p, ctx->counters);
-        if ((rc = fgpu_stage_scan_debug_drop(ctx))) return rc;
+        if ((rc = scan_pure_back(ctx, one_range))) return rc;
     }
     ctx->host_ms[4] += fgpu_host_now() - t_c;
     return FGPU_OK;
diff --git a/faucet_amd/csrc/scan_walk.hip b/faucet_amd/csrc/scan_walk.hip
--- a/faucet_amd/csrc/scan_walk.hip
+++ b/faucet_amd/csrc/scan_walk.hip
@@ -2057,10 +2057,10 @@
     while (wall_clock64() - t0 < ticks) __builtin_amdgcn_s_sleep(32);
 }
 
-__global__ void __launch_bounds__(256) k_debug_need_drop(uint64_t n_words, uint64_t* __restrict__ ff, uint64_t* __restrict__ fb,
+__global__ void __launch_bounds__(256) k_debug_need_drop(uint64_t w_lo, uint64_t w_hi, uint64_t* __restrict__ ff, uint64_t* __restrict__ fb,
                                                          uint64_t* need, uint64_t* cf0, uint64_t* cf1, uint64_t* cb0, uint64_t* cb1, int mode,
                                                          const uint64_t* __restrict__ pm, const uint32_t* __restrict__ kh) {
-    for (uint64_t w = (uint64_t)blockIdx.x * blockDim.x + threadIdx.x; w < n_words; w += (uint64_t)gridDim.x * blockDim.x) {
+    for (uint64_t w = w_lo + (uint64_t)blockIdx.x * blockDim.x + threadIdx.x; w < w_hi; w += (uint64_t)gridDim.x * blockDim.x) {
         uint64_t drop = need[w] & ~(ff[w] | fb[w]) & fd_mix(w * 0x9E3779B97F4A7C15ULL + 12345);
         if (mode == 2) {
             drop = 0;
@@ -2075,10 +2075,10 @@
     }
 }
 
-__global__ void __launch_bounds__(256) k_need_lookup(const uint64_t* __restrict__ codes, const uint64_t* __restrict__ pm, uint64_t n_words,
+__global__ void __launch_bounds__(256) k_need_lookup(const uint64_t* __restrict__ codes, const uint64_t* __restrict__ pm, uint64_t w_end,
                                                      FdParams fp, JTable jt, uint64_t* __restrict__ nF, uint64_t* __restrict__ nB,
                                                      uint32_t* __restrict__ kh, uint64_t w_first) {
-    const uint64_t total = n_words * 64;
+    const uint64_t total = w_end * 64;
     for (uint64_t p = w_first * 64 + (uint64_t)blockIdx.x * blockDim.x + threadIdx.x; p < total; p += (uint64_t)gridDim.x * blockDim.x) {
         bool inF = false, inB = false;
         if ((pm[p >> 6] >> (p & 63)) & 1ULL) {
@@ -2149,10 +2149,11 @@
     }
 }
 
-__global__ void __launch_bounds__(256) k_need_prewalk(const uint64_t* __restrict__ codes, const uint2* __restrict__ pieces, uint64_t n_pieces,
-                                                      FdParams fp, JTable jt, const uint64_t* __restrict__ nF, const uint64_t* __restrict__ nB,
-                                                      unsigned long long* need, int tight) {
-    for (uint64_t i = (uint64_t)blockIdx.x * blockDim.x + threadIdx.x; i < n_pieces; i += (uint64_t)gridDim.x * blockDim.x) {
+__global__ void __launch_bounds__(256) k_need_prewalk(const uint64_t* __restrict__ codes, const uint2* __restrict__ pieces, const uint32_t* __restrict__ prefix,
+                                                      uint64_t w_lo, uint64_t w_hi, FdParams fp, JTable jt, const uint64_t* __restrict__ nF,
+                                                      const uint64_t* __restrict__ nB, unsigned long long* need, int tight) {
+    const uint64_t i_first = prefix[w_lo], i_end = prefix[w_hi];
+    for (uint64_t i = i_first + (uint64_t)blockIdx.x * blockDim.x + threadIdx.x; i < i_end; i += (uint64_t)gridDim.x * blockDim.x) {
         const uint2 pc = pieces[i];
         const uint64_t p0 = pc.x;
         const uint32_t nwin = pc.y;
@@ -2298,15 +2299,26 @@
     const bool eager = (ctx->prm.flags & FGPU_FLAG_EAGER_FLAGS) || ctx->eager_runtime || ctx->eager_scan;
     FGPU_HIP(hipMemsetAsync(bb.need.p, eager ? 0xFF : 0, wb, ctx->stream));
     if (!bb.n_pieces) return FGPU_OK;
-    if (int rc = fgpu_ensure_b(ctx, &bb.kh, (bb.n_words + FGPU_PADW) * 64 * 4)) return rc;
-
+    return fgpu_ensure_b(ctx, &bb.kh, (bb.n_words + FGPU_PADW) * 64 * 4);
+}
+
+int fgpu_stage_scan_need_lookup(fgpu_ctx* ctx, uint64_t w_lo, uint64_t w_hi) {
+    BatchBufs& bb = *ctx->cur;
+    if (!bb.n_pieces || w_lo >= w_hi) return FGPU_OK;
+    FGPU_LAUNCH("need_lookup", k_need_lookup, fgpu_grid((w_hi - w_lo) * 64, 256), 256, (const uint64_t*)bb.codes.p, (const uint64_t*)bb.pm.p,
+                w_hi, ctx->fd, make_jt(ctx), (uint64_t*)bb.nF.p, (uint64_t*)bb.nB.p, (uint32_t*)bb.kh.p, w_lo);
+    return FGPU_OK;
+}
+
+int fgpu_stage_scan_need_prewalk(fgpu_ctx* ctx, uint64_t w_lo, uint64_t w_hi) {
+    BatchBufs& bb = *ctx->cur;
+    const bool eager = (ctx->prm.flags & FGPU_FLAG_EAGER_FLAGS) || ctx->eager_runtime || ctx->eager_scan;
+    if (eager || !bb.n_pieces || w_lo >= w_hi) return FGPU_OK;
     static const int need_tight = getenv("FGPU_NEED_TIGHT") ? atoi(getenv("FGPU_NEED_TIGHT")) : 2;
-    JTable jt = make_jt(ctx);
-    FGPU_LAUNCH("need_lookup", k_need_lookup, fgpu_grid(bb.n_words * 64, 256), 256, (const uint64_t*)bb.codes.p, (const uint64_t*)bb.pm.p,
-                bb.n_words, ctx->fd, jt, (uint64_t*)bb.nF.p, (uint64_t*)bb.nB.p, (uint32_t*)bb.kh.p, (uint64_t)0);
-    if (eager) return FGPU_OK;
-    FGPU_LAUNCH("need_prewalk", k_need_prewalk, fgpu_grid(bb.n_pieces, 256), 256, (const uint64_t*)bb.codes.p, (const uint2*)bb.pieces.p,
-                bb.n_pieces, ctx->fd, jt, (const uint64_t*)bb.nF.p, (const uint64_t*)bb.nB.p, (unsigned long long*)bb.need.p, need_tight);
+    const uint64_t most = std::min<uint64_t>(bb.n_pieces, (w_hi - w_lo) * 64 / (uint64_t)(ctx->fd.k + 1) + 2);
+    FGPU_LAUNCH("need_prewalk", k_need_prewalk, fgpu_grid(most, 256), 256, (const uint64_t*)bb.codes.p, (const uint2*)bb.pieces.p,
+                (const uint32_t*)bb.ps_prefix.p, w_lo, w_hi, ctx->fd, make_jt(ctx), (const uint64_t*)bb.nF.p, (const uint64_t*)bb.nB.p,
+                (unsigned long long*)bb.need.p, need_tight);
     return FGPU_OK;
 }
 
@@ -2340,12 +2352,12 @@
     return FGPU_OK;
 }
 
-int fgpu_stage_scan_debug_drop(fgpu_ctx* ctx) {
+int fgpu_stage_scan_debug_drop(fgpu_ctx* ctx, uint64_t w_lo, uint64_t w_hi) {
     static const int drop = getenv("FGPU_DEBUG_NEED_DROP") ? atoi(getenv("FGPU_DEBUG_NEED_DROP")) : 0;
     BatchBufs& bb = *ctx->cur;
-    if (!drop || !bb.n_pieces) return FGPU_OK;
+    if (!drop || !bb.n_pieces || w_lo >= w_hi) return FGPU_OK;
     if (drop == 2 && ((ctx->prm.flags & FGPU_FLAG_EAGER_FLAGS) || ctx->eager_runtime || ctx->eager_scan)) return FGPU_OK;
-    FGPU_LAUNCH("debug_need_drop", k_debug_need_drop, fgpu_grid(bb.n_words, 256), 256, bb.n_words, (uint64_t*)bb.ff.p, (uint64_t*)bb.fb.p,
+    FGPU_LAUNCH("debug_need_drop", k_debug_need_drop, fgpu_grid(w_hi - w_lo, 256), 256, w_lo, w_hi, (uint64_t*)bb.ff.p, (uint64_t*)bb.fb.p,
                 (uint64_t*)bb.need.p, (uint64_t*)bb.cf0.p, (uint64_t*)bb.cf1.p, (uint64_t*)bb.cb0.p, (uint64_t*)bb.cb1.p, drop,
                 (const uint64_t*)bb.pm.p, (const uint32_t*)bb.kh.p);
     return FGPU_OK;
@@ -2370,6 +2382,7 @@
     const bool dbg_span = getenv("FGPU_DEBUG_SPAN") != nullptr;
 };
 static const WalkKnobs& walk_knobs() { static const WalkKnobs knobs; return knobs; }
+bool fgpu_walk_no_overlap() { return walk_knobs().no_overlap; }
 
 struct WalkBatch {
     BatchBufs& bb;
@@ -2445,9 +2458,21 @@
                             bb.seq, 0);
 }
 
+static int walk_wait_range(fgpu_ctx* ctx, const WalkBatch& wb, uint64_t pos_end) {
+    BatchBufs& bb = wb.bb;
+    if (bb.n_ranges <= 1) return FGPU_OK;
+    const uint64_t last = pos_end - 1;
+    const uint64_t r = last < bb.range_first ? 0 : std::min<uint64_t>(1 + (last - bb.range_first) / bb.range_span, bb.n_ranges - 1);
+    if (r < bb.ranges_waited) return FGPU_OK;
+    FGPU_HIP(hipStreamWaitEvent(wb.walk_stream, bb.range_ev[r % FGPU_RANGE_EVENTS], 0));
+    bb.ranges_waited = r + 1;
+    return FGPU_OK;
+}
+
 static int walk_window_begin(fgpu_ctx* ctx, const WalkBatch& wb, uint64_t lo, uint64_t hi, WalkWindow* w) {
     const int parity = (int)(ctx->scan_windows & 1);
     const uint64_t set = parity * (uint64_t)ctx->wmax;
+    if (int rc = walk_wait_range(ctx, wb, std::min<uint64_t>(wb.T, hi + wb.ext))) return rc;
     FGPU_HIP(hipStreamWaitEvent(wb.walk_stream, ctx->ev_uf_reset[parity], 0));
     if (++ctx->wt_epoch > 255) {
         FGPU_HIP(hipMemsetAsync(ctx->wkeys, 0, ctx->wcap * 8, wb.walk_stream));
@@ -2758,7 +2783,8 @@
     WalkBatch wb{bb, pl, make_jt(ctx), bb.T, ext, ctx->scan_piece_base, walk_stream, ovw_stream, false, &ctx->delta_ring[ctx->delta_next % FGPU_DELTA_RING]};
     const uint64_t T = wb.T;
     ctx->launch_stream = walk_stream;
-    if (bb.pure_done) FGPU_HIP(hipStreamWaitEvent(walk_stream, bb.pure_done, 0));
+    bb.ranges_waited = 0;
+    if (bb.n_ranges <= 1 && bb.pure_done) FGPU_HIP(hipStreamWaitEvent(walk_stream, bb.pure_done, 0));
     if (ctx->dbg_stall_us) FGPU_LAUNCH("debug_stall", k_debug_stall, 1, 1, (unsigned long long)ctx->dbg_stall_us * 100ULL);
     if (ctx->refresh_snapshot && (rc = walk_refresh_prepared(ctx, bb, wb.jt, walk_stream, &wb.cand_ok))) return rc;
     if (ctx->record_stops) {
```

Measured after the change: 6.130 billion (median of 6 runs). +3.2%, better.
